# xandercai/JSPSR

Measured on AMD Instinct MI355X. Metric: Mpixels/sec fwd+bwd, JSPSR x8 on 512^2 DEM tiles, higher is better.
Workload: dtype bf16; 1 GPU; jspsr_r8_img_msk (image+mask guided, 43.87M params), 8 x 512x512 tiles per GPU, train step (fwd + L1/L2/Sobel loss + bwd + grad all-reduce + AdamW); storage policy: bf16 activations / gradients / MFMA operands, fp32 accumulation, BatchNorm statistics, master weights and optimizer, and the generator head (affinity logits + offsets) kept as fp32 planes; tiles_per_gpu=8, tile=512, global_tiles=8, parallelism=dp1, step_mode=eager

## Files before the change

### include/jspsr_hip.h

```cpp
#ifndef JSPSR_HIP_H
#define JSPSR_HIP_H

#include <stddef.h>
#include <stdint.h>

#ifdef __cplusplus
extern "C" {
#endif

#define JSPSR_OK 0
#define JSPSR_EINVAL (-1)
#define JSPSR_EALIGN (-2)

typedef void* jspsr_stream_t;

int jspsr_abi_version(void);
long long jspsr_launch_count(const char* what);
int jspsr_conv_dynamic_queue(int on);
const char* jspsr_last_error(void);

int jspsr_prop_forward_f32(const float* dem, const float* weight, const float* offset,
                           int offset_channels, const float* wk, const float* b0, float scale,
                           float* out, int B, int H, int W, jspsr_stream_t stream);

// ... 71 lines not shown
typedef struct jspsr_pack_desc {
  const float* w;
  void* out;
  long long start;
  long long total;
  int O, I, KH, KW;
  int mode;
  int c_pad;
  int dtype;
  int reserved;
} jspsr_pack_desc;
int jspsr_pack_chunk(void);
int jspsr_pack_weights_multi(const jspsr_pack_desc* descs, int n, long long total_blocks, jspsr_stream_t stream);

int jspsr_conv2d_stats_rows(int B, int OH, int OW);
int jspsr_conv2d_in_affine_ok(int dtype, int Cin, int KH, int KW, int stride);
int jspsr_conv2d_forward(int dtype, const void* in, const void* wpack, const float* bias, void* out,
                         int B, int IH, int IW, int Cin, int in_cstride, int in_coff, int Cout,
                         int out_cstride, int out_coff, int KH, int KW, int stride, int pad, int relu,
                         float* stats, const float* scale, const void* addend, int add_cstride,
                         const float* in_affine, int in_relu, jspsr_stream_t stream);
int jspsr_conv2d_forward_scaled(int dtype, const void* in, const void* wpack, const float* bias, void* out,
                                int B, int IH, int IW, int Cin, int in_cstride, int in_coff, int Cout,
                                int out_cstride, int out_coff, int KH, int KW, int stride, int pad, int relu,
                                float* stats, const float* scale, const void* addend, int add_cstride,
                                const float* in_scale, int in_scale_bstride, jspsr_stream_t stream);

int jspsr_conv2d_dgrad_reduce_ok(int dtype, int B, int IH, int IW, int Cg, int Cin, int KH, int KW, int stride, int pad);
int jspsr_conv2d_dgrad(int dtype, const void* gout, const void* wpack_t, const float* bias, void* gin,
                       int B, int OH, int OW, int Cg, int g_cstride, int g_coff, int IH, int IW,
                       int Cin, int in_cstride, int in_coff, int KH, int KW, int stride, int pad,
                       int relu, const void* addend, int add_cstride, const float* scale,
                       const void* red_x, int red_cstride, const float* red_par, float* red_out, jspsr_stream_t stream);

size_t jspsr_conv2d_wgrad_workspace_bytes(int dtype, int B, int OH, int OW, int Cg, int Cx, int KH, int KW);
int jspsr_conv2d_wgrad_x_affine_ok(int dtype, int B, int OH, int OW, int Cg, int Cx, int KH, int KW, int stride, int pad);
int jspsr_conv2d_wgrad(int dtype, const void* G, int Cg, int g_cstride, int g_coff, const void* X, int Cx,
                       int x_cstride, int x_coff, float* dW, int R, int C, int B, int OH, int OW,
                       int IH, int IW, int KH, int KW, int stride, int pad, int accumulate,
                       const float* x_affine, int x_relu, void* workspace, jspsr_stream_t stream);
int jspsr_conv2d_wgrad_scaled(int dtype, const void* G, int Cg, int g_cstride, int g_coff, const void* X, int Cx,
                              int x_cstride, int x_coff, float* dW, int R, int C, int B, int OH, int OW,
                              int IH, int IW, int KH, int KW, int stride, int pad, int accumulate,
                              const float* x_scale, int x_scale_bstride, void* workspace, jspsr_stream_t stream);

size_t jspsr_reduce_workspace_bytes(int dtype, int C, int nseg);

size_t jspsr_bn_mask_bytes(int dtype, long long npix, int C);
int jspsr_bn_forward(int dtype, const void* x, int x_cs, int x_coff, const void* res, int r_cs, int r_coff,
                     void* y, int y_cs, int y_coff, const float* gamma, const float* beta,
                     float* running_mean, float* running_var, float momentum, float eps, int training,
                     int relu, float res_scale, float* save_mean, float* save_invstd, long long npix, int C,
                     const float* ext_partial, int ext_rows, const float* res_affine, float* affine_out,
                     void* mask_out, void* workspace, jspsr_stream_t stream);

int jspsr_bn_fold(const float* gamma, const float* beta, const float* running_mean, const float* running_var,
                  float eps, float res_scale, int C, float* scale, float* shift, jspsr_stream_t stream);

int jspsr_bn_reduce_params(const float* gamma, const float* beta, const float* save_mean, const float* save_invstd, int C,
                           float* par, jspsr_stream_t stream);
int jspsr_bn_backward(int dtype, const void* dy, int dy_cs, int dy_coff, const void* y, int y_cs, int y_coff,
                      const void* x, int x_cs, int x_coff, const float* gamma, const float* beta, const float* save_mean,
                      const float* save_invstd, int training, int relu, float res_scale, void* dx, void* dres,
                      float* dgamma, float* dbeta, int accumulate, long long npix, int C, void* workspace,
                      const float* ext_partial, int ext_rows, const void* mask, jspsr_stream_t stream);

// ... 128 lines not shown
```

### jspsr_amd/JSPSR.py

```python
from __future__ import annotations

import contextlib
import math
import os

import torch
import torch.nn as nn

from . import engine as E
from . import ops
from .blocks import ConvUnit, HotPathModule, ResUnit, UpUnit
from .spn import Generator, PostProcessor

_AUX_KEYS = ("mask", "canopy", "coord")


class Model(HotPathModule):
    receptive_radius = 97
    plain_receptive_radius = 92
    size_multiple = 8

    def __init__(self, in_channels: dict, out_channels: int = 1, num_feature: int = 32,
                 layers: tuple = (2, 2, 2, 2), res_scale: tuple = (1, 1, 1, 1), spn: bool = True,
                 spn_scale: int = 1):
# ... 93 lines not shown
            elif flag_dem_coord:
                dem, coord = in_tensor
            else:
                raise NotImplementedError
        else:
            raise NotImplementedError
        return dem, img, msk, canopy, coord

    def forward(self, *in_tensor):
        dem, img, msk, canopy, coord = self.parse_input(
            self.flag_dem_img, self.flag_dem_msk, self.flag_dem_canopy, self.flag_dem_coord, *in_tensor)
        aux = msk if msk is not None else (canopy if canopy is not None else coord)
        with E.compute_dtype(self.compute_dtype), E.count_batches():
            return self._forward(dem, img, aux)

    branch_streams = True

    def _side_streams(self, device):
        if not self.branch_streams or os.environ.get("JSPSR_BRANCH_STREAMS", "1") == "0" or device.type != "cuda":
            return None
        cache = self.__dict__.setdefault("_branch_stream_cache", {})
        key = (device.index if device.index is not None else torch.cuda.current_device())
        if key not in cache:
            cache[key] = {br: torch.cuda.Stream(device=device) for br in ("img", "aux")}
        return {br: st for br, st in cache[key].items() if br in self._branches}

    def side_streams(self, device=None):
        device = device if device is not None else next(self.parameters()).device
        side = self._side_streams(torch.device(device))
        return list(side.values()) if side else []

    def _forward(self, dem, img, aux):
        dem_a = E.from_nchw(dem)
        feats = {"dem": self.conv_dem(dem_a)}
        if img is not None:
            feats["img"] = self.conv_img(E.from_nchw(img))
        if aux is not None:
            feats["aux"] = self.conv_aux(E.from_nchw(aux))
        order = [b for b in self._branches if b in feats]
        if len(order) < 2:
            raise NotImplementedError
        B, H, W = dem_a.shape[:3]
        nb, nf2 = len(order), self.conv0.conv[0].out_channels
        bufs, fused, joined = [], [], []
        defer_skip = all(getattr(self, f"layer{s}_dem")[0].fused for s in (2, 3, 4))
        deposit_ok = os.environ.get("JSPSR_GRAD_DEPOSIT", "1") != "0" and torch.is_grad_enabled() and order[0] == "dem"
        for s in range(1, 5):
            planes = nf2 * 2 ** (s - 1)
            if s > 1:
                H, W = (H + 1) // 2, (W + 1) // 2
            lead = planes if s < 4 else 0
            buf = E.SliceBuffer(B, H, W, lead + nb * planes, dem_a.dtype, dem_a.device)
            nxt = {}
            side = self._side_streams(dem_a.device) if len(order) > 1 else None
            if side is not None:
                main = torch.cuda.current_stream()
                forked = main.record_event()
            for i, br in enumerate(order):
                from_fused = br == "dem" and bool(fused)
                src = fused[-1] if from_fused else feats[br]
                units = list(getattr(self, f"layer{s}_{br}"))
                st = side.get(br) if side is not None else None
                if st is not None:
                    st.wait_event(forked)
                    buf.buf.record_stream(st)
                    if s == 1:
                        src.record_stream(st)
                with (torch.cuda.stream(st) if st is not None else contextlib.nullcontext()):
                    for k, u in enumerate(units):
                        kw = {}
                        if k == 0 and from_fused and defer_skip:
                            kw["grad_extra"] = bufs[-1][0]
                        elif k == 0 and s > 1 and defer_skip and br != "dem" and getattr(u, "fused", False) and deposit_ok:
                            holder, w_prev = bufs[-1][0], planes // 2
                            kw["grad_extra"] = (holder, i * w_prev, w_prev)
                            holder.expected_deposits += 1
                        if k == len(units) - 1:
                            kw["dest"] = (buf, lead + i * planes)
                        src = u(src, **kw)
                nxt[br] = src
            if side is not None:
                for st in side.values():
                    main.wait_stream(st)
            feats = nxt
            bufs.append((buf, lead))
            joined.append([feats[b] for b in order])
            fused.append(buf.join(joined[-1], lead))
        x = fused[3]
        for up, s in ((self.layer3d, 2), (self.layer2d, 1), (self.layer1d, 0)):
            buf, lead = bufs[s]
            x = buf.join([up(x, dest=(buf, 0))] + joined[s], 0, defer=nb if defer_skip else 0)
        c0 = self.conv0(x)
        if not self.spn:
            head = self.postprocessor.conv[0]
            return E.conv_head1(c0, head.weight, head.bias)
        dem = dem.detach()
        feature = self.generator.features(dem_a.detach(), c0)
        return self.postprocessor.from_feature(dem.float(), feature, self.generator)
```

### jspsr_amd/_lib.py

```python
from __future__ import annotations

import ctypes
import os
import subprocess
import threading

_HERE = os.path.dirname(os.path.abspath(__file__))
SO_PATH = os.environ.get("JSPSR_LAB_LIB") or os.path.join(_HERE, "lib", "libjspsr_hip.so")
CSRC = os.path.join(_HERE, "csrc")
ABI_VERSION = 25

_lock = threading.Lock()
_lib = None

c_p = ctypes.c_void_p
c_i = ctypes.c_int
c_f = ctypes.c_float
c_ll = ctypes.c_longlong

SIGNATURES = {
    "jspsr_abi_version": (c_i, []),
    "jspsr_launch_count": (c_ll, [ctypes.c_char_p]),
    "jspsr_conv_dynamic_queue": (c_i, [c_i]),
    "jspsr_last_error": (ctypes.c_char_p, []),
    "jspsr_prop_forward_f32": (c_i, [c_p, c_p, c_p, c_i, c_p, c_p, c_f, c_p, c_i, c_i, c_i, c_p]),
    "jspsr_prop_backward_workspace_bytes": (ctypes.c_size_t, [c_i, c_i, c_i]),
    "jspsr_prop_backward_f32": (c_i, [c_p] * 4 + [c_i] + [c_p] * 6 + [c_i, c_i, c_i, c_p]),
    "jspsr_prop_backward_fold_f32": (c_i, [c_p, c_i, c_i, c_i, c_p, c_p, c_p]),
    "jspsr_prop_step_forward_f32": (c_i, [c_p, c_p, c_p, c_i, c_p, c_p, c_f, c_i, c_p, c_i, c_i, c_i, c_p]),
    "jspsr_prop_step_backward_workspace_bytes": (ctypes.c_size_t, [c_i, c_i, c_i]),
    "jspsr_prop_step_backward_f32": (c_i, [c_p] * 4 + [c_i, c_p, c_f, c_i, c_i] + [c_p] * 6 + [c_i, c_i, c_i, c_p]),
    "jspsr_prop_head_forward": (c_i, [c_i, c_p, c_p, c_p, c_p, c_f, c_p, c_i, c_i, c_i, c_p]),
    "jspsr_prop_head_backward_workspace_bytes": (ctypes.c_size_t, [c_i, c_i, c_i]),
    "jspsr_prop_head_backward": (c_i, [c_i] + [c_p] * 8 + [c_i, c_i, c_i, c_p]),
    "jspsr_prop_logits_forward_f32": (c_i, [c_p, c_p, c_p, c_p, c_f, c_p, c_i, c_i, c_i, c_p]),
    "jspsr_prop_logits_backward_f32": (c_i, [c_p] * 8 + [c_i, c_i, c_i, c_p]),
    "jspsr_head_ok": (c_i, [c_i] * 5),
    "jspsr_head_forward": (c_i, [c_i, c_p, c_i, c_i, c_i, c_p, c_p, c_p, c_i, c_i, c_i, c_p]),
    "jspsr_head_backward_workspace_bytes": (ctypes.c_size_t, [c_i, c_i, c_i]),
    "jspsr_head_backward": (c_i, [c_i, c_p, c_p, c_i, c_p, c_i, c_i, c_p, c_p, c_p, c_i, c_i, c_i, c_p]),
    "jspsr_conv_head1_forward": (c_i, [c_i, c_p, c_i, c_i, c_i, c_p, c_p, c_p, c_i, c_i, c_i, c_p]),
    "jspsr_conv_head1_workspace_bytes": (ctypes.c_size_t, [c_i, c_i, c_i, c_i]),
    "jspsr_conv_head1_backward": (c_i, [c_i, c_p, c_p, c_i, c_i, c_i, c_p, c_p, c_i, c_i, c_p, c_p, c_p, c_i, c_i, c_i, c_p]),
    "jspsr_pack_weight": (c_i, [c_i, c_p, c_p] + [c_i] * 6 + [c_p]),
    "jspsr_pack_chunk": (c_i, []),
    "jspsr_pack_weights_multi": (c_i, [c_p, c_i, c_ll, c_p]),
    "jspsr_conv2d_stats_rows": (c_i, [c_i, c_i, c_i]),
    "jspsr_conv2d_in_affine_ok": (c_i, [c_i] * 5),
    "jspsr_conv2d_forward": (c_i, [c_i] + [c_p] * 4 + [c_i] * 14 + [c_p, c_p, c_p, c_i, c_p, c_i, c_p]),
    "jspsr_conv2d_forward_scaled": (c_i, [c_i] + [c_p] * 4 + [c_i] * 14 + [c_p, c_p, c_p, c_i, c_p, c_i, c_p]),
    "jspsr_bn_fold": (c_i, [c_p, c_p, c_p, c_p, c_f, c_f, c_i, c_p, c_p, c_p]),
    "jspsr_conv2d_dgrad_reduce_ok": (c_i, [c_i] * 10),
    "jspsr_conv2d_dgrad": (c_i, [c_i] + [c_p] * 4 + [c_i] * 16 + [c_p, c_i, c_p, c_p, c_i, c_p, c_p, c_p]),
    "jspsr_conv2d_wgrad_workspace_bytes": (ctypes.c_size_t, [c_i] * 8),
    "jspsr_conv2d_wgrad_x_affine_ok": (c_i, [c_i] * 10),
    "jspsr_conv2d_wgrad": (c_i, [c_i, c_p, c_i, c_i, c_i, c_p, c_i, c_i, c_i, c_p] + [c_i] * 12 + [c_p, c_i, c_p, c_p]),
    "jspsr_conv2d_wgrad_scaled": (c_i, [c_i, c_p, c_i, c_i, c_i, c_p, c_i, c_i, c_i, c_p] + [c_i] * 12 + [c_p, c_i, c_p, c_p]),
    "jspsr_reduce_workspace_bytes": (ctypes.c_size_t, [c_i, c_i, c_i]),
    "jspsr_bn_forward": (c_i, [c_i, c_p, c_i, c_i, c_p, c_i, c_i, c_p, c_i, c_i, c_p, c_p, c_p, c_p, c_f, c_f, c_i,
                               c_i, c_f, c_p, c_p, c_ll, c_i, c_p, c_i, c_p, c_p, c_p, c_p, c_p]),
    "jspsr_bn_mask_bytes": (ctypes.c_size_t, [c_i, c_ll, c_i]),
    "jspsr_bn_reduce_params": (c_i, [c_p, c_p, c_p, c_p, c_i, c_p, c_p]),
    "jspsr_bn_backward": (c_i, [c_i, c_p, c_i, c_i, c_p, c_i, c_i, c_p, c_i, c_i, c_p, c_p, c_p, c_p, c_i, c_i, c_f,
                                c_p, c_p, c_p, c_p, c_i, c_ll, c_i, c_p, c_p, c_i, c_p, c_p]),
    "jspsr_act_backward": (c_i, [c_i, c_p, c_i, c_i, c_p, c_i, c_i, c_p, c_i, c_p, c_ll, c_i, c_p, c_p]),
    "jspsr_gate_pool": (c_i, [c_i, c_p, c_i, c_ll, c_i, c_p, c_p, c_p, c_p, c_p]),
    "jspsr_gate_scale": (c_i, [c_i, c_p, c_p, c_p, c_i, c_ll, c_i, c_p]),
    "jspsr_gate_backward_reduce": (c_i, [c_i, c_p, c_p, c_p, c_i, c_ll, c_i, c_p, c_p]),
    "jspsr_gate_backward_apply": (c_i, [c_i, c_p, c_p, c_p, c_p, c_p, c_p, c_i, c_ll, c_i, c_p]),
    "jspsr_loss_workspace_bytes": (ctypes.c_size_t, [c_i, c_i, c_i]),
    "jspsr_loss_forward": (c_i, [c_p, c_p, c_f, c_f, c_f, c_p, c_p, c_i, c_i, c_i, c_p]),
    "jspsr_loss_backward": (c_i, [c_p, c_p, c_p, c_f, c_f, c_f, c_p, c_p, c_i, c_i, c_i, c_p]),
    "jspsr_loss_menu_workspace_bytes": (ctypes.c_size_t, [c_i, c_i, c_i, c_i]),
    "jspsr_loss_menu_forward": (c_i, [c_p, c_p, c_i, c_i, c_i, c_i, c_i, c_p, c_p, c_p, c_p, c_p, c_p]),
    "jspsr_loss_menu_backward": (c_i, [c_p, c_p, c_i, c_i, c_i, c_i, c_p, c_p, c_p, c_p, c_p]),
    "jspsr_ssim_workspace_bytes": (ctypes.c_size_t, [c_i, c_i, c_i, c_i]),
    "jspsr_ssim_forward": (c_i, [c_p, c_p, c_i, c_i, c_i, c_i, c_p, c_p, c_p, c_p]),
    "jspsr_metrics_workspace_bytes": (ctypes.c_size_t, [c_i, c_i]),
    "jspsr_metrics_forward": (c_i, [c_p, c_p, c_i, c_i, c_f, c_f, c_f, c_i, c_p, c_p, c_p]),
    "jspsr_scores_batch_workspace_bytes": (ctypes.c_size_t, [c_i, c_i, c_i]),
    "jspsr_scores_batch_forward": (c_i, [c_p, c_p, c_i, c_i, c_i, c_f, c_f, c_f, c_i, c_p, c_p, c_p]),
    "jspsr_scenes_assemble_f32": (c_i, [c_p] * 5 + [c_ll] + [c_i] * 6 + [ctypes.c_double, ctypes.c_double, c_p]),
    "jspsr_summary_workspace_bytes": (ctypes.c_size_t, [c_i, c_i, c_ll, c_ll]),
    "jspsr_summary_forward": (c_i, [c_p, c_p, c_i, c_p, c_ll, c_p, c_i, c_p, c_i, c_ll, c_ll, ctypes.c_double, c_p, c_p, c_p]),
    "jspsr_summary_valid_workspace_bytes": (ctypes.c_size_t, [c_i, c_i, c_ll, c_ll]),
    "jspsr_summary_valid_forward": (c_i, [c_p, c_p, c_i, c_p, c_ll, c_p, c_ll, c_p, c_i, c_p, c_i, c_ll, c_ll, ctypes.c_double,
# ... 82 lines not shown
```

### jspsr_amd/blocks.py

```python
from __future__ import annotations

import torch
import torch.nn as nn

from . import engine as E
from . import ops


class HotPathModule(nn.Module):

    def zero_grad(self, set_to_none: bool = True):
        red = self.__dict__.get("_grad_reducer")
        if red is not None:
            red.zero_grad()
        else:
            super().zero_grad(set_to_none)

    def train(self, mode: bool = True):
        ops.invalidate_packed_weights()
        return super().train(mode)

    def load_state_dict(self, *args, **kwargs):
        out = super().load_state_dict(*args, **kwargs)
        ops.invalidate_packed_weights()
        return out


class ChannelGate(nn.Module):

    def __init__(self, channels: int, ratio: int = 16):
        super().__init__()
        self.fc = nn.Sequential()
        self.fc.add_module("0", nn.Conv2d(channels, channels // ratio, 1, bias=False))
        self.fc.add_module("2", nn.Conv2d(channels // ratio, channels, 1, bias=False))

    def forward(self, x):
        return E.channel_gate(x, self.fc[0].weight, self.fc[1].weight)


class ConvUnit(nn.Module):

    def __init__(self, cin, cout, kernel_size=3, bn=True, relu=True, gate=False):
        super().__init__()
        if gate:
            self.camb = ChannelGate(cin)
        self.conv = nn.Sequential()
        self.conv.add_module("0", nn.Conv2d(cin, cout, kernel_size, 1, kernel_size // 2, bias=not bn))
        if bn:
            self.conv.add_module("bn", nn.BatchNorm2d(cout))
        self.k = kernel_size
        self.relu = relu

    def forward(self, x, dest=None):
        c = self.conv[0]
        if hasattr(self, "camb") and hasattr(self.conv, "bn"):
            fc = self.camb.fc
            return E.gated_conv_bn(x, fc[0].weight, fc[1].weight, c.weight, self.conv.bn, self.k // 2, relu=self.relu, dest=dest)
        if hasattr(self, "camb"):
            x = self.camb(x)
        if hasattr(self.conv, "bn"):
            return E.conv_bn(x, c.weight, self.conv.bn, 1, self.k // 2, relu=self.relu, dest=dest)
        return E.conv2d(x, c.weight, c.bias, 1, self.k // 2, relu=self.relu, dest=dest)


class UpUnit(nn.Module):

    def __init__(self, cin, cout):
        super().__init__()
        self.dconv = nn.Sequential()
        self.dconv.add_module("0", ConvUnit(cin, cout, 3, bn=True, relu=True, gate=True))
        self.dconv.add_module("1", nn.ConvTranspose2d(cout, cout, 3, 2, 1, 1, bias=False))
        self.dconv.add_module("bn", nn.BatchNorm2d(cout))

    def forward(self, x, dest=None):
        y = self.dconv[0](x)
        bn = self.dconv.bn
        if not torch.is_grad_enabled() and not (bn.training or bn.running_mean is None):
            return ops.conv_transpose_bn_infer(y, self.dconv[1].weight, bn.weight, bn.bias, E._bn_state(bn), True, dest)
        y = E.conv_transpose2d(y, self.dconv[1].weight)
        return E.batch_norm(y, bn, relu=True, dest=dest)


class ResUnit(nn.Module):

    def __init__(self, cin, cout, stride=1, project=False, act=True, scale=1.0):
        super().__init__()
        self.conv1 = nn.Conv2d(cin, cout, 3, stride, 1, bias=False)
        self.bn1 = nn.BatchNorm2d(cout)
        self.conv2 = nn.Conv2d(cout, cout, 3, 1, 1, bias=False)
        self.bn2 = nn.BatchNorm2d(cout)
        self.downsample = None
        if project:
            self.downsample = nn.Sequential(nn.Conv2d(cin, cout, 1, stride, bias=False), nn.BatchNorm2d(cout))
        self.stride, self.act, self.scale = stride, act, scale

    fused = True

    def forward(self, x, dest=None, grad_extra=None):
        if self.fused:
            return E.res_unit(x, self.conv1, self.bn1, self.conv2, self.bn2, self.downsample, self.stride, self.scale,
                              self.act, dest, grad_extra)
        if grad_extra is not None:
            raise RuntimeError("grad_extra needs the fused block")
        y = E.conv_bn(x, self.conv1.weight, self.bn1, self.stride, 1, relu=True)
        if self.downsample is not None:
            r = E.conv_bn(x, self.downsample[0].weight, self.downsample[1], self.stride, 0)
        else:
            r = x
        return E.conv_bn(y, self.conv2.weight, self.bn2, 1, 1, relu=self.act, residual=r, res_scale=self.scale,
                         dest=dest)
```

### jspsr_amd/csrc/conv.hip

```cpp
#include "conv_igemm.h"

#include <cstdlib>
#include <type_traits>

namespace {

using namespace jspsr;

constexpr int NT = 256;
constexpr int NCH = 8;
template <typename T> struct Elem;
template <> struct Elem<float> { static constexpr int EPC = 4; };
template <> struct Elem<__bf16> { static constexpr int EPC = 8; };

template <typename T> struct Mma;
template <> struct Mma<float> {
  static constexpr int BLK = 32, ROWP = 144, NE = 16, SUB = NCH / 2, SUBB = 32;
  using acc_t = f32x16;
  static __device__ __forceinline__ int frag_row(int lane) { return lane & 31; }
  static __device__ __forceinline__ int frag_chunk(int lane) { return lane >> 5; }
  static __device__ __forceinline__ int acc_row(int lane, int e) { return (e & 3) + 8 * (e >> 2) + 4 * (lane >> 5); }
  static __device__ __forceinline__ int acc_col(int lane) { return lane & 31; }
};
template <> struct Mma<__bf16> {
// ... 90 lines not shown
    for (int i = 0; i < 4; ++i) f[i] = __uint_as_float(w[i]);
  } else {
#pragma unroll
    for (int i = 0; i < 4; ++i) {
      f[2 * i] = __uint_as_float(w[i] << 16);
      f[2 * i + 1] = __uint_as_float(w[i] & 0xffff0000u);
    }
  }
}

template <typename T>
__device__ __forceinline__ uint4 add_packed(uint4 a, uint4 b) {
  if constexpr (sizeof(T) == 4) {
    float4 x = __builtin_bit_cast(float4, a), y = __builtin_bit_cast(float4, b);
    x.x += y.x; x.y += y.y; x.z += y.z; x.w += y.w;
    return __builtin_bit_cast(uint4, x);
  } else {
    const unsigned* pa = &a.x;
    const unsigned* pb = &b.x;
    uint4 r;
    unsigned* pr = &r.x;
#pragma unroll
    for (int i = 0; i < 4; ++i) {
      const float lo = __uint_as_float(pa[i] << 16) + __uint_as_float(pb[i] << 16);
      const float hi = __uint_as_float(pa[i] & 0xffff0000u) + __uint_as_float(pb[i] & 0xffff0000u);
      const __bf16 l = (__bf16)lo, h = (__bf16)hi;
      pr[i] = (unsigned)__builtin_bit_cast(unsigned short, l) | ((unsigned)__builtin_bit_cast(unsigned short, h) << 16);
    }
    return r;
  }
}

template <typename T>
__device__ __forceinline__ uint4 relu_packed(uint4 a) {
  if constexpr (sizeof(T) == 4) {
    float4 x = __builtin_bit_cast(float4, a);
    x.x = fmaxf(x.x, 0.f); x.y = fmaxf(x.y, 0.f); x.z = fmaxf(x.z, 0.f); x.w = fmaxf(x.w, 0.f);
    return __builtin_bit_cast(uint4, x);
  } else {
    unsigned* p = &a.x;
#pragma unroll
    for (int i = 0; i < 4; ++i) {
      if (p[i] & 0x00008000u) p[i] &= 0xffff0000u;
      if (p[i] & 0x80000000u) p[i] &= 0x0000ffffu;
    }
    return a;
  }
}

template <typename T, int BM, int BN, int WGM, int WGN, bool UNI, int NBUF>
__global__ __launch_bounds__(NT, NBUF == 1 ? 4 : 2) void conv_igemm_kernel(const T* __restrict__ in,
                                                          const T* __restrict__ wgt,
                                                          const float* __restrict__ bias,
                                                          T* __restrict__ out, float* __restrict__ stats, ConvGeom g) {
  static_assert(WGM * WGN == 4, "4 waves");
  constexpr int EPC = Elem<T>::EPC, BK = NCH * EPC;
  using M = IgemmMma<T, NBUF>;
  constexpr int ROWB = M::ROWP, BLK = M::BLK;
  constexpr int WTM = BM / WGM, WTN = BN / WGN, MI = WTM / BLK, NI = WTN / BLK;
  constexpr int A_IT = BM * NCH / NT, B_IT = (BN * NCH + NT - 1) / NT;
  static_assert(MI >= 1 && NI >= 1 && BM * NCH % NT == 0, "tile");
  using frag_t = typename Frag<T>::type;

  extern __shared__ __attribute__((aligned(16))) char smem[];
  constexpr int AS_BYTES = BM * ROWB, BS_BYTES = BN * ROWB;
  char* As = smem;
  char* Bs = smem + NBUF * AS_BYTES;

  constexpr int TLW = 16, TLH = BM / TLW;
  const int tid = threadIdx.x;
  const int ntn = (g.Cout + BN - 1) / BN;
  const int ttx = (g.MW + TLW - 1) / TLW, tty = (g.MH + TLH - 1) / TLH;
  const int t = g.accumulate ? (int)blockIdx.x : xcd_contiguous(blockIdx.x, gridDim.x);
  const int n0 = (t % ntn) * BN;
  const int mt = t / ntn;
  const int txi = mt % ttx, tyi = (mt / ttx) % tty, bimg = mt / (ttx * tty);
  const int ty0 = tyi * TLH, tx0 = txi * TLW;

  const int ch = tid & (NCH - 1);
  const int r0 = tid >> 3;
  constexpr unsigned OOB = 0xFFFFFFF0u;
  const int pix_bytes = g.in_cstride * (int)sizeof(T);
  const int iy_ref = ty0 * g.iy_mul + g.iy_add, ix_ref = tx0 * g.ix_mul + g.ix_add;
// ... 193 lines not shown
        areg[j] = make_uint4(0, 0, 0, 0);
        if (opix >= 0 && n0 + c16 * EPC < g.Cout)
          areg[j] = *reinterpret_cast<const uint4*>(static_cast<const char*>(g.addend) +
                                                    (opix * g.add_cstride + n0) * (long long)sizeof(T) + c16 * 16);
      }
    }
#pragma unroll
    for (int mi = 0; mi < MI; ++mi)
#pragma unroll
      for (int e = 0; e < M::NE; ++e) {
        const int row = wm * WTM + mi * BLK + M::acc_row(lane, e);
#pragma unroll
        for (int ni = 0; ni < NI; ++ni) {
          float v = acc[mi][ni][e] * sv[ni] + bv[ni];
          if (relu_first) v = fmaxf(v, 0.f);
          *reinterpret_cast<T*>(Os + row * OPITCH + (wn * WTN + ni * BLK + lc) * (int)sizeof(T)) = (T)v;
        }
      }
    __syncthreads();
    char* const obase = reinterpret_cast<char*>(out + g.out_coff + n0);
#pragma unroll
    for (int j = 0; j < O_IT; ++j) {
      const int i = tid + j * NT, row = i / CPRO, c16 = i % CPRO;
      const long long opix = out_pixel(row);
      if (opix < 0 || n0 + c16 * EPC >= g.Cout) continue;
      uint4 v = *reinterpret_cast<const uint4*>(Os + row * OPITCH + c16 * 16);
      if (CONV_ABLATE == 4 && v.x != 0x12345678u) continue;
      if (add_pre)
        v = add_packed<T>(v, areg[j < A_PRE ? j : 0]);
      else if (g.addend)
        v = add_packed<T>(v, *reinterpret_cast<const uint4*>(static_cast<const char*>(g.addend) +
                                                              (opix * g.add_cstride + n0) * (long long)sizeof(T) + c16 * 16));
      if (relu_last) v = relu_packed<T>(v);
      *reinterpret_cast<uint4*>(obase + opix * g.out_cstride * (long long)sizeof(T) + c16 * 16) = v;
    }
  } else {
#pragma unroll
    for (int mi = 0; mi < MI; ++mi) {
#pragma unroll
      for (int e = 0; e < M::NE; ++e) {
        const int row = wm * WTM + mi * BLK + M::acc_row(lane, e);
        const long long opix = out_pixel(row);
        if (opix < 0) continue;
        T* orow = out + opix * g.out_cstride + g.out_coff;
#pragma unroll
        for (int ni = 0; ni < NI; ++ni) {
          if (ncol[ni] >= g.Cout) continue;
          float v = acc[mi][ni][e] * sv[ni] + bv[ni];
          if (relu_first) v = fmaxf(v, 0.f);
          if (g.addend) v = (float)(T)v + (float)static_cast<const T*>(g.addend)[opix * g.add_cstride + ncol[ni]];
          if (relu_last) v = fmaxf(v, 0.f);
          orow[ncol[ni]] = (T)v;
        }
      }
    }
  }
}

#ifdef CONVLAB_STAMPS
constexpr int CONVLAB_SLOTS = 1 << 17;
__device__ unsigned long long convlab_stamp[CONVLAB_SLOTS * 16];
#define CL_NOW(t) do { __builtin_amdgcn_sched_barrier(0); asm volatile("s_memtime %0\n\ts_waitcnt lgkmcnt(0)" : "=s"(t) :: "memory"); \
    __builtin_amdgcn_sched_barrier(0); } while (0)
#if CONVLAB_STAMPS == 2
#define CL_STAMP(i) do { unsigned long long now_; CL_NOW(now_); cl_stamp[i] += now_ - cl_last; cl_last = now_; } while (0)
#else
#define CL_STAMP(i) do { } while (0)
#endif
#else
#define CL_STAMP(i) do { } while (0)
#endif
#if defined(CONVLAB_STAMPS) && CONVLAB_STAMPS == 3
#define CL_STAMP3(i) do { unsigned long long now_; CL_NOW(now_); cl_stamp[i] += now_ - cl_last; cl_last = now_; } while (0)
#else
#define CL_STAMP3(i) do { } while (0)
#endif

__host__ __device__ constexpr int patch_it(int BM, int NTH) { return ((BM / 16 + 2) * 18 * NCH + NTH - 1) / NTH; }

template <typename T, int BM, int BN, int WGM, int WGN>
__global__ __launch_bounds__(64 * WGM * WGN, WGM * WGN == 8 ? 1 : 2) void conv_patch_kernel(const T* __restrict__ in, const T* __restrict__ wgt,
                                                          const float* __restrict__ bias, T* __restrict__ out,
                                                          float* __restrict__ stats, ConvGeom g) {
  static_assert(WGM * WGN == 4 || WGM * WGN == 8, "4 or 8 waves");
  constexpr int NTH = 64 * WGM * WGN, RPI = NTH / NCH;
  constexpr int TLW = 16, TLH = BM / TLW;
  constexpr int EPC = Elem<T>::EPC, BK = NCH * EPC;
  using M = Mma<T>;
  constexpr int ROWB = M::ROWP, BLK = M::BLK;
  constexpr int WTM = BM / WGM, WTN = BN / WGN, MI = WTM / BLK, NI = WTN / BLK;
  constexpr int B_IT = (BN * NCH + NTH - 1) / NTH;
  constexpr int P_IT = patch_it(BM, NTH);
  constexpr int MAXPIX = P_IT * NTH / NCH;
  constexpr int BS_BYTES = BN * ROWB;
  constexpr unsigned OOB = 0xFFFFFFF0u;
  using frag_t = typename Frag<T>::type;

  extern __shared__ __attribute__((aligned(16))) char smem[];
  char* Ps = smem;
  char* Bs = smem + MAXPIX * ROWB;

#ifdef CONVLAB_STAMPS
  unsigned long long cl_entry, cl_stamp[8] = {0, 0, 0, 0, 0, 0, 0, 0}, cl_last = 0, cl_first = 0;
  CL_NOW(cl_entry);
  cl_last = cl_entry;
#endif
  const int tid = threadIdx.x;
  const int ntn = (g.Cout + BN - 1) / BN;
  const int ttx = (g.MW + TLW - 1) / TLW, tty = (g.MH + TLH - 1) / TLH;
  const int t = xcd_contiguous(blockIdx.x, gridDim.x);
  const int mt = (int)fastdiv((unsigned)t, g.fd_ntn);
  const int n0 = (t - mt * ntn) * BN;
  const int mrow = (int)fastdiv((unsigned)mt, g.fd_ttx), txi = mt - mrow * ttx;
// ... 253 lines not shown
  if (stats) {
    if constexpr (BM == 128) {
      stats_epilogue<M, MI, NI, WGM, WTM, WTN, BN>(acc, stats, smem, mt, g.Cout, n0, wm, wn, lane, out_pixel);
    } else {
      const int tty8 = (g.MH + 7) / 8;
      const int r1 = (bimg * tty8 + 2 * tyi) * ttx + txi;
      const int r2 = (2 * tyi + 1 < tty8) ? r1 + ttx : -1;
      stats_epilogue<M, MI, NI, WGM, WTM, WTN, BN>(acc, stats, smem, r1, g.Cout, n0, wm, wn, lane, out_pixel, r2);
    }
  }
  float bv[NI], sv[NI];
  int ncol[NI];
  const bool relu_first = g.relu && !g.addend, relu_last = g.relu && g.addend;
#pragma unroll
  for (int ni = 0; ni < NI; ++ni) {
    ncol[ni] = n0 + wn * WTN + ni * BLK + lc;
    bv[ni] = (bias && ncol[ni] < g.Cout) ? bias[ncol[ni]] : 0.f;
    sv[ni] = (g.scale && ncol[ni] < g.Cout) ? g.scale[ncol[ni]] : 1.f;
  }
  constexpr int OPITCH = BN * (int)sizeof(T) + 16;
  char* Os = smem;
  const bool vec_ok = (g.Cout % EPC == 0) && ((g.out_cstride * (int)sizeof(T)) % 16 == 0) &&
                      (((g.out_coff + n0) * (int)sizeof(T)) % 16 == 0) &&
                      ((reinterpret_cast<uintptr_t>(out) & 15u) == 0) &&
                      (!g.addend || (((reinterpret_cast<uintptr_t>(g.addend) & 15u) == 0) &&
                                     ((g.add_cstride * (int)sizeof(T)) % 16 == 0) && ((n0 * (int)sizeof(T)) % 16 == 0)));
  if (vec_ok) {
    constexpr int CPRO = BN * (int)sizeof(T) / 16;
    constexpr int O_IT = BM * CPRO / NTH, OB = O_IT <= 8 ? O_IT : 8;
    static_assert(BM * CPRO % NTH == 0 && O_IT % OB == 0, "epilogue rows");
    long long ooff[OB];
    uint4 areg[OB];
    uint4 zreg[OB];
    const int oy_t = ty0 * g.oy_mul + g.oy_add, ox_t = tx0 * g.ox_mul + g.ox_add, ystep = g.oy_mul * g.OW;
    const long long pix_t = ((long long)bimg * g.OH + oy_t) * g.OW + ox_t;
    const unsigned ocs = (unsigned)g.out_cstride * (unsigned)sizeof(T), acs = (unsigned)g.add_cstride * (unsigned)sizeof(T);
    const long long obase_t = pix_t * ocs, abase_t = pix_t * acs + n0 * (long long)sizeof(T);
    const unsigned zcs = (unsigned)g.red_cstride * (unsigned)sizeof(T);
    const long long zbase_t = pix_t * zcs + n0 * (long long)sizeof(T);
    const bool inside = ty0 + TLH <= g.MH && tx0 + TLW <= g.MW && oy_t + (TLH - 1) * g.oy_mul < g.OH &&
                        ox_t + (TLW - 1) * g.ox_mul < g.OW && n0 + BN <= g.Cout;
    auto plan_pieces = [&](int j0) __attribute__((always_inline)) {
#pragma unroll
      for (int j = 0; j < OB; ++j) {
        const int i = tid + (j0 + j) * NTH, row = i / CPRO, c16 = i % CPRO;
        const int dy = row >> 4, dx = (row + rot * dy) & (TLW - 1);
        const unsigned dpix = (unsigned)(dy * ystep + dx * g.ox_mul);
        bool ok = true;
        if (!inside)
          ok = ty0 + dy < g.MH && tx0 + dx < g.MW && oy_t + dy * g.oy_mul < g.OH && ox_t + dx * g.ox_mul < g.OW &&
               n0 + c16 * EPC < g.Cout;
        ooff[j] = ok ? obase_t + (long long)((unsigned long long)dpix * ocs) + c16 * 16 : -1;
        if (g.addend) {
          areg[j] = make_uint4(0, 0, 0, 0);
          if (ok)
            areg[j] = *reinterpret_cast<const uint4*>(static_cast<const char*>(g.addend) + abase_t +
                                                      (long long)((unsigned long long)dpix * acs) + c16 * 16);
        }
        if (g.red_out) {
          zreg[j] = make_uint4(0, 0, 0, 0);
          if (ok)
            zreg[j] = *reinterpret_cast<const uint4*>(static_cast<const char*>(g.red_x) + zbase_t +
                                                      (long long)((unsigned long long)dpix * zcs) + c16 * 16);
        }
      }
    };
    float rs1[EPC], rs2[EPC], rpa[EPC], rpb[EPC], rpi[EPC], rpm[EPC];
    if (g.red_out) {
      static_assert(NTH % CPRO == 0, "a thread's pieces share their channels");
      const int cc = n0 + (tid % CPRO) * EPC;
#pragma unroll
      for (int e2 = 0; e2 < EPC; ++e2) {
        const bool in_c = cc + e2 < g.Cout;
        rs1[e2] = rs2[e2] = 0.f;
        rpa[e2] = in_c ? g.red_par[cc + e2] : 0.f;
        rpb[e2] = in_c ? g.red_par[g.Cout + cc + e2] : 0.f;
        rpi[e2] = in_c ? g.red_par[2 * g.Cout + cc + e2] : 0.f;
        rpm[e2] = in_c ? g.red_par[3 * g.Cout + cc + e2] : 0.f;
      }
    }
    plan_pieces(0);
#pragma unroll
    for (int mi = 0; mi < MI; ++mi)
#pragma unroll
      for (int e = 0; e < M::NE; ++e) {
        const int row = wm * WTM + mi * BLK + M::acc_row(lane, e);
#pragma unroll
        for (int ni = 0; ni < NI; ++ni) {
          float v = acc[mi][ni][e] * sv[ni] + bv[ni];
          if (relu_first) v = fmaxf(v, 0.f);
          *reinterpret_cast<T*>(Os + row * OPITCH + (wn * WTN + ni * BLK + lc) * (int)sizeof(T)) = (T)v;
        }
      }
    CL_STAMP3(0);
    __syncthreads();
    CL_STAMP3(1);
    char* const obase = reinterpret_cast<char*>(out + g.out_coff + n0);
#pragma unroll
    for (int j0 = 0; j0 < O_IT; j0 += OB) {
      if (j0) plan_pieces(j0);
      uint4 ov[OB];
#pragma unroll
      for (int j = 0; j < OB; ++j) {
        const int i = tid + (j0 + j) * NTH, row = i / CPRO, c16 = i % CPRO;
        ov[j] = *reinterpret_cast<const uint4*>(Os + row * OPITCH + c16 * 16);
      }
      CL_STAMP3(2);
#pragma unroll
      for (int j = 0; j < OB; ++j) {
        if (ooff[j] < 0) continue;
        uint4 v = ov[j];
        if (g.addend) v = add_packed<T>(v, areg[j]);
        if (relu_last) v = relu_packed<T>(v);
        *reinterpret_cast<uint4*>(obase + ooff[j]) = v;
        if (g.red_out) {
          float dv[EPC], zv[EPC];
          unpack_chunk<T>(v, dv);
          unpack_chunk<T>(zreg[j], zv);
#pragma unroll
          for (int e2 = 0; e2 < EPC; ++e2) {
            const float dz = rpa[e2] * zv[e2] + rpb[e2] > 0.f ? dv[e2] : 0.f;
            rs1[e2] += dz;
            rs2[e2] += dz * (zv[e2] * rpi[e2] + rpm[e2]);
          }
        }
      }
    }
    if (g.red_out) {
      __syncthreads();
      float* red = reinterpret_cast<float*>(smem);
#pragma unroll
      for (int e2 = 0; e2 < EPC; ++e2) {
        red[tid * 2 * EPC + e2] = rs1[e2];
        red[tid * 2 * EPC + EPC + e2] = rs2[e2];
      }
      __syncthreads();
      int r1 = mt, r2 = -1;
      if constexpr (BM != 128) {
        const int tty8 = (g.MH + 7) / 8;
        r1 = (bimg * tty8 + 2 * tyi) * ttx + txi;
        r2 = (2 * tyi + 1 < tty8) ? r1 + ttx : -1;
      }
      for (int i = tid; i < 2 * BN; i += NTH) {
        const int which = i / BN, col = i % BN;
        if (n0 + col >= g.Cout) continue;
        const int cg_ = col / EPC, e2 = col % EPC;
        float tsum = 0.f;
        for (int k2 = 0; k2 < NTH / CPRO; ++k2) tsum += red[(cg_ + CPRO * k2) * 2 * EPC + which * EPC + e2];
        g.red_out[((size_t)r1 * 2 + which) * g.Cout + n0 + col] = tsum;
        if (r2 >= 0) g.red_out[((size_t)r2 * 2 + which) * g.Cout + n0 + col] = 0.f;
      }
    }
  } else {
#pragma unroll
    for (int mi = 0; mi < MI; ++mi)
#pragma unroll
      for (int e = 0; e < M::NE; ++e) {
        const int row = wm * WTM + mi * BLK + M::acc_row(lane, e);
        const long long opix = out_pixel(row);
        if (opix < 0) continue;
        T* orow = out + opix * g.out_cstride + g.out_coff;
#pragma unroll
        for (int ni = 0; ni < NI; ++ni) {
          if (ncol[ni] >= g.Cout) continue;
          float v = acc[mi][ni][e] * sv[ni] + bv[ni];
          if (relu_first) v = fmaxf(v, 0.f);
          if (g.addend) v = (float)(T)v + (float)static_cast<const T*>(g.addend)[opix * g.add_cstride + ncol[ni]];
          if (relu_last) v = fmaxf(v, 0.f);
          orow[ncol[ni]] = (T)v;
        }
      }
  }
#ifdef CONVLAB_STAMPS
  if ((tid & 63) == 0) {
    unsigned long long end_;
    CL_NOW(end_);
    unsigned long long* o = convlab_stamp + (size_t)((blockIdx.x * (NTH / 64) + (tid >> 6)) % CONVLAB_SLOTS) * 16;
    for (int i = 0; i < 4; ++i) o[i] = cl_stamp[i] + (i == 3 ? cl_stamp[4] : 0);
    o[4] = cl_first - cl_entry;
    o[5] = cl_loop - cl_first;
    o[6] = end_ - cl_loop;
    for (int i = 5; i < 8; ++i) o[3 + i] = cl_stamp[i];
    o[11] = cl_stamp[4];
    o[7] = (unsigned long long)KT;
  }
#endif
}

template <typename T, int BM, int BN, int WGM, int WGN>
int launch_patch(const void* in, const void* wgt, const float* bias, void* out, float* stats, const ConvGeom& g, hipStream_t s) {
  constexpr int NTH = 64 * WGM * WGN, TLW = 16, TLH = BM / TLW, MAXPIX = patch_it(BM, NTH) * NTH / NCH;
  const long long nblk = (long long)g.B * ((g.MH + TLH - 1) / TLH) * ((g.MW + TLW - 1) / TLW) * ((g.Cout + BN - 1) / BN);
  if (nblk > 0x7fffffffLL || (long long)TLH * g.oy_mul * g.OW + (long long)TLW * g.ox_mul > 0x7fffffffLL)
    return fail(JSPSR_EINVAL, "conv: grid too large");
  constexpr int ROWB = Mma<T>::ROWP;
  const size_t lds_stage = (size_t)MAXPIX * ROWB + 2 * BN * ROWB, lds_out = (size_t)BM * (BN * sizeof(T) + 16);
  const size_t lds = lds_stage > lds_out ? lds_stage : lds_out;
  ConvGeom gk = g;
  gk.fd_ntn = make_fastdiv((unsigned)((g.Cout + BN - 1) / BN));
  gk.fd_ttx = make_fastdiv((unsigned)((g.MW + TLW - 1) / TLW));
  gk.fd_tty = make_fastdiv((unsigned)((g.MH + TLH - 1) / TLH));
  auto kern = conv_patch_kernel<T, BM, BN, WGM, WGN>;
  static bool attr_set = false;
  if (!attr_set) {
    (void)hipFuncSetAttribute(reinterpret_cast<const void*>(kern), hipFuncAttributeMaxDynamicSharedMemorySize, (int)lds);
    attr_set = true;
  }
  hipLaunchKernelGGL(kern, dim3((unsigned)nblk), dim3(NTH), lds, s, static_cast<const T*>(in), static_cast<const T*>(wgt),
                     bias, static_cast<T*>(out), stats, gk);
  return check_launch(BM == 256 ? (BN == 64 ? "conv_patch_16x16" : "conv_patch_16x16x128") : "conv_patch");
}

template <typename T, int BM, int BN, int WGM, int WGN, int NBUF>
int launch_cfg(const void* in, const void* wgt, const float* bias, void* out, float* stats, const ConvGeom& g, hipStream_t s) {
  if ((long long)g.B * g.MH * g.MW <= 0) return JSPSR_OK;
  constexpr int TLW = 16, TLH = BM / TLW;
  const long long nblk = (long long)g.B * ((g.MH + TLH - 1) / TLH) * ((g.MW + TLW - 1) / TLW) * ((g.Cout + BN - 1) / BN);
  if (nblk > 0x7fffffffLL) return fail(JSPSR_EINVAL, "conv: grid too large");
  constexpr int ROWB = IgemmMma<T, NBUF>::ROWP;
  const size_t lds_stage = NBUF * (BM + BN) * ROWB, lds_out = (size_t)BM * (BN * sizeof(T) + 16);
  const size_t lds = lds_stage > lds_out ? lds_stage : lds_out;
  constexpr int BK = NCH * Elem<T>::EPC;
  static bool attr_set = false;
  if (!attr_set) {
    (void)hipFuncSetAttribute(reinterpret_cast<const void*>(conv_igemm_kernel<T, BM, BN, WGM, WGN, true, NBUF>),
                              hipFuncAttributeMaxDynamicSharedMemorySize, (int)lds);
    (void)hipFuncSetAttribute(reinterpret_cast<const void*>(conv_igemm_kernel<T, BM, BN, WGM, WGN, false, NBUF>),
                              hipFuncAttributeMaxDynamicSharedMemorySize, (int)lds);
    attr_set = true;
  }
  if (g.Cin % BK == 0)
    hipLaunchKernelGGL((conv_igemm_kernel<T, BM, BN, WGM, WGN, true, NBUF>), dim3((unsigned)nblk), dim3(NT), lds, s,
                       static_cast<const T*>(in), static_cast<const T*>(wgt), bias, static_cast<T*>(out), stats, g);
  else
    hipLaunchKernelGGL((conv_igemm_kernel<T, BM, BN, WGM, WGN, false, NBUF>), dim3((unsigned)nblk), dim3(NT), lds, s,
                       static_cast<const T*>(in), static_cast<const T*>(wgt), bias, static_cast<T*>(out), stats, g);
  return check_launch("conv_igemm");
}

template <typename T>
int launch(const void* in, const void* wgt, const float* bias, void* out, float* stats, const ConvGeom& g, hipStream_t s) {
  static const int no_patch = [] { const char* e = getenv("JSPSR_CONV_NOPATCH"); return e ? atoi(e) : 0; }();
  constexpr int BKT = NCH * Elem<T>::EPC;
  if constexpr (sizeof(T) == 2)
  {
    if (conv64_resident_ok(g, in, wgt, bias, out)) return launch_conv64_resident(in, wgt, bias, out, stats, g, s);
    if (conv128_resident_ok(g, in, wgt, bias, out)) return launch_conv128_resident(in, wgt, bias, out, stats, g, s);
  }
  if ((!no_patch || g.in_affine) && g.iy_mul == 1 && g.ix_mul == 1 && g.nty >= 1 && g.ntx >= 1 && g.nty <= 3 && g.ntx <= 3 &&
      g.nty * g.ntx > 1 && g.Cin % BKT == 0 && (long long)(g.IW + 20) * 12 * g.in_cstride * (long long)sizeof(T) < 0xE0000000LL) {
    static const int tall = [] { const char* e = getenv("JSPSR_CONV_TALL"); return e ? atoi(e) : 1; }();
    const long long tiles16 = (long long)g.B * ((g.MH + 15) / 16) * ((g.MW + 15) / 16);
    if (g.Cout > 64) {
      if (tall == 2 && tiles16 * ((g.Cout + 127) / 128) >= 512) return launch_patch<T, 256, 128, 4, 2>(in, wgt, bias, out, stats, g, s);
      if (tall && tall != 4 && tiles16 * ((g.Cout + 63) / 64) >= 1024) return launch_patch<T, 256, 64, 4, 1>(in, wgt, bias, out, stats, g, s);
      return launch_patch<T, 128, 128, 2, 2>(in, wgt, bias, out, stats, g, s);
    }
    if (g.Cout > 32) {
      if (tall && tiles16 >= 1024) return launch_patch<T, 256, 64, 4, 1>(in, wgt, bias, out, stats, g, s);
      return launch_patch<T, 128, 64, 2, 2>(in, wgt, bias, out, stats, g, s);
    }
    return launch_patch<T, 128, 32, 4, 1>(in, wgt, bias, out, stats, g, s);
  }
  if (g.red_out) return fail(JSPSR_EINVAL, "conv2d_dgrad: the fused BatchNorm-backward reduce needs the patch kernel (jspsr_conv2d_dgrad_reduce_ok)");
  if (g.in_affine) return fail(JSPSR_EINVAL, "conv2d_forward: in_affine needs the patch kernel (stride 1, 2..9 taps, Cin a multiple of %d): ask jspsr_conv2d_in_affine_ok first", BKT);
  static const int nbuf_env = [] { const char* e = getenv("JSPSR_CONV_NBUF"); return e ? atoi(e) : 0; }();
  const int nbuf_narrow = nbuf_env ? nbuf_env : ((long long)g.nty * g.ntx * g.Cin <= 1152 ? 1 : 2);
  if (g.Cout > 64) return launch_cfg<T, 128, 128, 2, 2, 2>(in, wgt, bias, out, stats, g, s);
// ... 136 lines not shown
extern "C" int jspsr_conv2d_forward_scaled(int dtype, const void* in, const void* wpack, const float* bias, void* out,
                                           int B, int IH, int IW, int Cin, int in_cstride, int in_coff, int Cout,
                                           int out_cstride, int out_coff, int KH, int KW, int stride, int pad, int relu,
                                           float* stats, const float* scale, const void* addend, int add_cstride,
                                           const float* in_scale, int in_scale_bstride, jspsr_stream_t stream) {
  if (!in_scale || in_scale_bstride < Cin || in_scale_bstride % 4)
    return fail(JSPSR_EINVAL, "conv2d_forward_scaled: in_scale must be [B][in_scale_bstride >= Cin] floats, the stride a multiple of 4");
  return conv2d_forward_impl(dtype, in, wpack, bias, out, B, IH, IW, Cin, in_cstride, in_coff, Cout, out_cstride, out_coff, KH, KW,
                             stride, pad, relu, stats, scale, addend, add_cstride, in_scale, 0, in_scale_bstride, 1, stream);
}

extern "C" int jspsr_conv2d_in_affine_ok(int dtype, int Cin, int KH, int KW, int stride) {
  const int bk = NCH * (dtype == JSPSR_F32 ? 4 : 8);
  return (dtype == JSPSR_F32 || dtype == JSPSR_BF16) && stride == 1 && KH >= 1 && KW >= 1 && KH <= 3 && KW <= 3 && KH * KW > 1 &&
         Cin > 0 && Cin % bk == 0;
}

extern "C" int jspsr_conv2d_dgrad_reduce_ok(int dtype, int B, int IH, int IW, int Cg, int Cin, int KH, int KW, int stride, int pad) {
  if (dtype != JSPSR_F32 && dtype != JSPSR_BF16) return 0;
  static const int off = [] { const char* e = getenv("JSPSR_BN_REDUCE_FUSE"); return e && atoi(e) == 0; }();
  if (off) return 0;
  const int epc = dtype == JSPSR_F32 ? 4 : 8, bkt = NCH * epc;
  if (KH != 3 || KW != 3 || stride != 1 || pad != 1 || Cg <= 0 || Cg % bkt || Cin <= 0 || Cin % epc || B <= 0 || IH <= 0 || IW <= 0) return 0;
  static const int no_patch = [] { const char* e = getenv("JSPSR_CONV_NOPATCH"); return e ? atoi(e) : 0; }();
  if (no_patch) return 0;
  if (dtype == JSPSR_BF16 && Cg == 64 && Cin == 64) {
    static const int resident = [] { const char* e = getenv("JSPSR_CONV_RESIDENT"); return e ? atoi(e) : 1; }();
    static const int min_tiles = [] { const char* e = getenv("JSPSR_CONV_RESIDENT_MIN"); return e ? atoi(e) : 512; }();
    if (resident && (long long)B * ((IH + 15) / 16) * ((IW + 15) / 16) >= min_tiles) return 0;
  }
  return 1;
}

extern "C" int jspsr_conv2d_dgrad(int dtype, const void* gout, const void* wpack_t, const float* bias, void* gin,
                                  int B, int OH, int OW, int Cg, int g_cstride, int g_coff, int IH, int IW,
                                  int Cin, int in_cstride, int in_coff, int KH, int KW, int stride, int pad,
                                  int relu, const void* addend, int add_cstride, const float* scale,
                                  const void* red_x, int red_cstride, const float* red_par, float* red_out,
                                  jspsr_stream_t stream) {
  if (int e = check_common(dtype, gout, wpack_t, gin, Cg, g_cstride, g_coff, in_cstride, in_coff, Cin, "conv2d_dgrad")) return e;
  if (addend && add_cstride < Cin) return fail(JSPSR_EINVAL, "conv2d_dgrad: addend pitch %d < %d channels", add_cstride, Cin);
  if (red_out) {
    if (!red_x || !red_par || !jspsr_conv2d_dgrad_reduce_ok(dtype, B, IH, IW, Cg, Cin, KH, KW, stride, pad))
      return fail(JSPSR_EINVAL, "conv2d_dgrad: the fused BatchNorm-backward reduce needs jspsr_conv2d_dgrad_reduce_ok(...) != 0");
    const int epc = dtype == JSPSR_F32 ? 4 : 8;
    if (red_cstride < Cin || red_cstride % epc || in_cstride % epc || in_coff % epc || !aligned16(red_x) || !aligned16(gin) ||
        (addend && (!aligned16(addend) || add_cstride % epc)))
      return fail(JSPSR_EALIGN, "conv2d_dgrad: fused reduce needs 16-byte pieces (pitches / offsets multiples of %d, aligned tensors)", epc);
  }
  if (B <= 0 || OH <= 0 || OW <= 0 || IH <= 0 || IW <= 0 || KH <= 0 || KW <= 0 || stride <= 0 || pad < 0)
    return fail(JSPSR_EINVAL, "conv2d_dgrad: bad geometry");
  hipStream_t s = static_cast<hipStream_t>(stream);
  for (int py = 0; py < stride; ++py)
    for (int px = 0; px < stride; ++px) {
      ConvGeom g{};
      g.B = B; g.IH = OH; g.IW = OW; g.Cin = Cg;
      g.OH = IH; g.OW = IW; g.Cout = Cin;
      g.in_cstride = g_cstride; g.in_coff = g_coff; g.out_cstride = in_cstride; g.out_coff = in_coff;
      g.MH = (IH - py + stride - 1) / stride;
      g.MW = (IW - px + stride - 1) / stride;
      if (g.MH <= 0 || g.MW <= 0) continue;
      g.ky0 = (py + pad) % stride; g.kx0 = (px + pad) % stride; g.kstep = stride;
      g.nty = g.ky0 < KH ? (KH - g.ky0 + stride - 1) / stride : 0;
      g.ntx = g.kx0 < KW ? (KW - g.kx0 + stride - 1) / stride : 0;
      if (g.nty == 0 || g.ntx == 0) g.nty = g.ntx = 0;
      g.iy_mul = 1; g.iy_add = (py + pad - g.ky0) / stride; g.ix_mul = 1; g.ix_add = (px + pad - g.kx0) / stride;
      g.sign = -1; g.KH = KH; g.KW = KW;
      g.oy_mul = stride; g.oy_add = py; g.ox_mul = stride; g.ox_add = px; g.relu = relu;
      g.addend = addend; g.add_cstride = add_cstride; g.scale = scale;
      g.red_x = red_x; g.red_cstride = red_cstride; g.red_par = red_par; g.red_out = red_out;
      const int e = dtype == JSPSR_F32 ? launch<float>(gout, wpack_t, bias, gin, nullptr, g, s)
                                       : launch<__bf16>(gout, wpack_t, bias, gin, nullptr, g, s);
      if (e) return e;
    }
  return JSPSR_OK;
}

#ifdef CONVLAB_STAMPS
extern "C" int jspsr_lab_conv_stamps(unsigned long long* out16, int reset) {
  static unsigned long long host[CONVLAB_SLOTS * 16];
  if (hipMemcpyFromSymbol(host, HIP_SYMBOL(convlab_stamp), sizeof(host)) != hipSuccess) return 1;
  for (int i = 0; i < 16; ++i) out16[i] = 0;
  for (int r = 0; r < CONVLAB_SLOTS; ++r)
    if (host[r * 16 + 7]) { for (int i = 0; i < 16; ++i) out16[i] += host[r * 16 + i]; }
  if (reset) { for (size_t i = 0; i < sizeof(host) / 8; ++i) host[i] = 0; if (hipMemcpyToSymbol(HIP_SYMBOL(convlab_stamp), host, sizeof(host)) != hipSuccess) return 1; }
  return 0;
}
#endif
```

### jspsr_amd/csrc/conv128.hip

```cpp
#include "conv_igemm.h"

#include <atomic>

#include <cstdlib>
#include <type_traits>

namespace {

using namespace jspsr;

constexpr int Q_NTH = 256;
constexpr int Q_TH = 8, Q_TW = 16;
constexpr int Q_PH = Q_TH + 2, Q_PW = Q_TW + 2, Q_NPIX = Q_PH * Q_PW;
constexpr int Q_PIXB = 256;
constexpr int Q_PATCHB = Q_NPIX * Q_PIXB;
constexpr int Q_PIECES = Q_PATCHB / 1024;
static_assert(Q_PIECES * 1024 == Q_PATCHB, "whole pieces");
constexpr int Q_NP = (Q_PIECES + 3) / 4;
constexpr int Q_BUF1 = 65536;
constexpr int Q_XCHB = 16384;
constexpr int Q_OFF_RED = Q_PATCHB + Q_XCHB;
static_assert(Q_OFF_RED + 2048 <= Q_BUF1, "the first 64 KiB hold patch 0, inbox 0 and the fold");
constexpr int Q_OFF_RUN = Q_OFF_RED + 2048;
static_assert(Q_OFF_RUN + 16 <= Q_BUF1, "run starts inside the first 64 KiB");
// ... 38 lines not shown
}

template <bool FIRST, bool WA>
__device__ __forceinline__ void mfma4(f32x4& c0, f32x4& c1, f32x4& c2, f32x4& c3, const i32x4& w0, const i32x4& w1, const i32x4& w2,
                                      const i32x4& w3, const i32x4& b) {
#define K2Q_MFMA4(OUT, CC, WC)                                                                                           \
  asm volatile("v_mfma_f32_16x16x32_bf16 %0, %4, %8, " CC "0\n\tv_mfma_f32_16x16x32_bf16 %1, %5, %8, " CC "1\n\t"        \
               "v_mfma_f32_16x16x32_bf16 %2, %6, %8, " CC "2\n\tv_mfma_f32_16x16x32_bf16 %3, %7, %8, " CC "3"             \
               : OUT(c0), OUT(c1), OUT(c2), OUT(c3) : WC(w0), WC(w1), WC(w2), WC(w3), "v"(b))
  if constexpr (FIRST) {
    if constexpr (WA)
      asm volatile("v_mfma_f32_16x16x32_bf16 %0, %4, %8, 0\n\tv_mfma_f32_16x16x32_bf16 %1, %5, %8, 0\n\t"
                   "v_mfma_f32_16x16x32_bf16 %2, %6, %8, 0\n\tv_mfma_f32_16x16x32_bf16 %3, %7, %8, 0"
                   : "=&v"(c0), "=&v"(c1), "=&v"(c2), "=&v"(c3) : "a"(w0), "a"(w1), "a"(w2), "a"(w3), "v"(b));
    else
      asm volatile("v_mfma_f32_16x16x32_bf16 %0, %4, %8, 0\n\tv_mfma_f32_16x16x32_bf16 %1, %5, %8, 0\n\t"
                   "v_mfma_f32_16x16x32_bf16 %2, %6, %8, 0\n\tv_mfma_f32_16x16x32_bf16 %3, %7, %8, 0"
                   : "=&v"(c0), "=&v"(c1), "=&v"(c2), "=&v"(c3) : "v"(w0), "v"(w1), "v"(w2), "v"(w3), "v"(b));
  } else {
    if constexpr (WA) K2Q_MFMA4("+v", "%", "a");
    else K2Q_MFMA4("+v", "%", "v");
  }
#undef K2Q_MFMA4
}

typedef const i32x4 __attribute__((address_space(3)))* lds_frag_t;

struct QTile { int bimg, tyi, txi; };
struct QSrc { i32x4 desc; __amdgpu_buffer_rsrc_t rsrc; int oy0, ox0; bool interior; };

template <int SIGN, int MODE, int KH>
__device__ __forceinline__ void conv128_body(const __bf16* __restrict__ in, const __bf16* __restrict__ wgt, const float* __restrict__ bias,
                                             __bf16* __restrict__ out, float* __restrict__ stats, const ConvGeom& g, int ntiles, unsigned* __restrict__ ticket, char* smem) {
  constexpr bool STATS = MODE == 1, AFFINE = MODE == 2;
  const int tid = threadIdx.x, wave = __builtin_amdgcn_readfirstlane(tid >> 6), lane = tid & 63;
  const int cg = wave & 1;
  const int n = lane & 15, q = lane >> 4;
  const int ttx = (g.MW + Q_TW - 1) / Q_TW, tty = (g.MH + Q_TH - 1) / Q_TH;
  const int G = gridDim.x;
  const unsigned lds0 = (unsigned)(size_t)(lptr_t)smem;
  if (lds0 != 0) __builtin_trap();
  const int v = xcd_contiguous(blockIdx.x, G);

  i32x4 breg[9][2][4];
#pragma unroll
  for (int cb = 0; cb < 4; ++cb) {
    const int ch = 64 * cg + 32 * (cb >> 1) + 8 * (n >> 2) + 4 * (cb & 1) + (n & 3);
    const char* wrow = reinterpret_cast<const char*>(wgt) + (size_t)ch * (9 * 128 * 2) + (64 * KH + 8 * q) * 2;
#pragma unroll
    for (int t = 0; t < 9; ++t)
#pragma unroll
      for (int s = 0; s < 2; ++s) breg[t][s][cb] = *reinterpret_cast<const i32x4*>(wrow + t * 256 + s * 64);
  }

  const int dGx = G % ttx, dGy = (G / ttx) % tty, dGb = G / (ttx * tty);
  auto advance = [&](QTile c) {
    c.txi += dGx;
    int carry = c.txi >= ttx;
    c.txi -= carry ? ttx : 0;
    c.tyi += dGy + carry;
    carry = c.tyi >= tty;
    c.tyi -= carry ? tty : 0;
    c.bimg += dGb + carry;
    return c;
  };

  const int pix_bytes = g.in_cstride * 2;
// ... 42 lines not shown
  };
  auto piece_dst = [&](unsigned bufoff, int i) __attribute__((always_inline)) {
#ifdef K2Q_LAB_TODUMP
    return (unsigned)Q_OFF_DUMP;
#endif
    return (wave + 4 * i < Q_PIECES) ? bufoff + (unsigned)(wave + 4 * i) * 1024u : (unsigned)Q_OFF_DUMP;
  };
  auto issue_piece = [&](const QSrc& p, unsigned bufoff, int i) __attribute__((always_inline)) {
    unsigned src = dsrc[i];
    if (!p.interior) src = piece_src(p, piece_xy(i));
    const unsigned dst = lds0 + piece_dst(bufoff, i);
#if defined(K2Q_LAB_NOISSUE)
    asm volatile("" : : "s"(dst), "v"(src), "s"(p.desc));
#elif defined(K2Q_LAB_OOB)
    asm volatile("s_mov_b32 m0, %0\n\ts_nop 4\n\tbuffer_load_dwordx4 %1, %2, 0 offen lds" : : "s"(dst), "v"(src | 0xF0000000u), "s"(p.desc));
#else
    asm volatile("s_mov_b32 m0, %0\n\ts_nop 4\n\tbuffer_load_dwordx4 %1, %2, 0 offen lds" : : "s"(dst), "v"(src), "s"(p.desc));
#endif
  };

  unsigned abase[4][3];
#pragma unroll
  for (int b = 0; b < 4; ++b)
#pragma unroll
    for (int tx = 0; tx < 3; ++tx)
      abase[b][tx] = (unsigned)((Q_PW * b + tx + n) * Q_PIXB + (((8 * KH + q) ^ (2 * ((2 * b + tx + n) & 7))) << 4));

  auto prefetch_addend = [&](QTile tc) __attribute__((always_inline)) {
    const int y = tc.tyi * Q_TH + 4 * KH + q, x = tc.txi * Q_TW + n;
    const unsigned off = (y < g.MH && x < g.MW) ? (unsigned)(y * g.OW + x) * (unsigned)(g.add_cstride * 2) : 0xFFFFFFF0u;
    const unsigned long long b64 = reinterpret_cast<unsigned long long>(g.addend) + ((long long)tc.bimg * g.OH * g.OW * g.add_cstride + 64 * cg) * 2;
    const i32x4 d = {(int)(unsigned)b64, (int)((unsigned)(b64 >> 32) & 0xffffu), g.addend ? (int)0xFFFFFF00u : 0, 0x00020000};
    asm volatile("s_mov_b32 m0, %0\n\ts_nop 4\n\tbuffer_load_dwordx4 %1, %2, 0 offen lds" : : "s"(lds0 + (unsigned)Q_OFF_DUMP), "v"(off), "s"(d));
  };

  char* const give = smem + inbox_off(wave ^ 2) + lane * 16;
  const char* const take = smem + inbox_off(wave) + lane * 16;
  f32x4 acc[8][4];
  auto meet = [&]() __attribute__((always_inline)) {
    asm volatile("s_nop 15\n\ts_nop 15" ::: "memory");
#pragma unroll
    for (int i = 0; i < 4; ++i)
#pragma unroll
      for (int cb = 0; cb < 4; ++cb) *reinterpret_cast<f32x4*>(give + (i * 4 + cb) * 1024) = acc[4 * (1 - KH) + i][cb];
    asm volatile("s_waitcnt lgkmcnt(0)" ::: "memory");
    __builtin_amdgcn_s_barrier();
    asm volatile("" ::: "memory");
#pragma unroll
    for (int i = 0; i < 4; ++i)
#pragma unroll
      for (int cb = 0; cb < 4; ++cb) acc[4 * KH + i][cb] = *reinterpret_cast<const f32x4*>(take + (i * 4 + cb) * 1024);
  };

  auto mfma_tile = [&](const QSrc& nxt, unsigned nbufoff, QTile tc) __attribute__((always_inline)) {
    i32x4 a[Q_LAH];
    constexpr int NSTG = (K2Q_LD_DIST + K2Q_LD_EVERY - 1) / K2Q_LD_EVERY;
    u32x4 stg[NSTG];
    static_for<0, Q_NK + Q_LAH>([&](auto K) __attribute__((always_inline)) {
      constexpr int k = decltype(K)::value;
      if constexpr (k >= Q_LAH) {
        constexpr int kk = k - Q_LAH, half = kk / 72, st = (kk % 72) >> 2, tap = st >> 1, s = st & 1;
        constexpr int r = (half == 0 ? 4 * (1 - KH) : 4 * KH) + (kk & 3);
        if constexpr (kk == 72) meet();
        mfma4<(half == 0 && st == 0), (tap < 8)>(acc[r][0], acc[r][1], acc[r][2], acc[r][3], breg[tap][s][0], breg[tap][s][1], breg[tap][s][2],
                                                 breg[tap][s][3], a[kk % Q_LAH]);
      }
      if constexpr (k < Q_NK) {
        constexpr int half = k / 72, st = (k % 72) >> 2, tap = st >> 1, s = st & 1;
        constexpr int r = (half == 0 ? 4 * (1 - KH) : 4 * KH) + (k & 3);
        constexpr int ty = SIGN > 0 ? tap / 3 : 2 - tap / 3, tx = SIGN > 0 ? tap % 3 : 2 - tap % 3;
        constexpr int R = r + ty;
        a[k % Q_LAH] = *reinterpret_cast<lds_frag_t>((abase[R & 3][tx] ^ (unsigned)(s * 64)) + (unsigned)((R >> 2) * Q_ROWS4));
        if constexpr (K2Q_DMA_MODE == 1 && k % K2Q_DMA_EVERY == 2 && k / K2Q_DMA_EVERY < Q_NP) issue_piece(nxt, nbufoff, k / K2Q_DMA_EVERY);
        if constexpr (!STATS && k == 1) prefetch_addend(tc);
        if constexpr (K2Q_DMA_MODE == 3) {
          constexpr int LD = K2Q_LD_EVERY, WD = K2Q_LD_DIST;
          static_assert(2 + LD * (Q_NP - 1) + WD < Q_NK, "the last piece is written inside the loop");
          if constexpr (k >= 2 + WD && (k - 2 - WD) % LD == 0 && (k - 2 - WD) / LD < Q_NP) {
            constexpr int j = (k - 2 - WD) / LD;
            *reinterpret_cast<u32x4*>(smem + piece_dst(nbufoff, j) + lane * 16) = stg[j % NSTG];
          }
          if constexpr (k >= 2 && (k - 2) % LD == 0 && (k - 2) / LD < Q_NP) {
            constexpr int j = (k - 2) / LD;
            stg[j % NSTG] = __builtin_amdgcn_raw_buffer_load_b128(nxt.rsrc, piece_src(nxt, piece_xy(j)), 0, 0);
          }
        }
      }
    });
    asm volatile("s_nop 15\n\ts_nop 15" ::: "memory");
  };

  const bool relu_first = g.relu && !g.addend, relu_last = g.relu && g.addend;
  float* const red = reinterpret_cast<float*>(smem + Q_OFF_RED);
  auto out_desc = [&](int bimg) {
    const unsigned long long b64 = reinterpret_cast<unsigned long long>(out) + ((long long)bimg * g.OH * g.OW * g.out_cstride + g.out_coff + 64 * cg) * 2;
    return __builtin_amdgcn_make_buffer_rsrc(reinterpret_cast<char*>(b64), 0, 0xFFFFFF00u, 0x00020000);
  };
  auto add_desc = [&](int bimg) {
    const unsigned long long b64 = reinterpret_cast<unsigned long long>(g.addend) + ((long long)bimg * g.OH * g.OW * g.add_cstride + 64 * cg) * 2;
    return __builtin_amdgcn_make_buffer_rsrc(reinterpret_cast<char*>(b64), 0, g.addend ? 0xFFFFFF00u : 0u, 0x00020000);
  };

  auto epilogue = [&](QTile tc) __attribute__((always_inline)) {
    const int ty0 = tc.tyi * Q_TH + 4 * KH, x = tc.txi * Q_TW + n;
    const __amdgpu_buffer_rsrc_t orsrc = out_desc(tc.bimg), adrsrc = add_desc(tc.bimg);
    unsigned ooff[4], aoff[4];
    bool inside[4];
// ... 33 lines not shown
                s2[c] = __builtin_fmaf(a0, a0, s2[c]);
              }
            }
          }
          row_sum<8>(s1); row_sum<8>(s2);
          row_sum<4>(s1); row_sum<4>(s2);
          row_sum<2>(s1); row_sum<2>(s2);
          row_sum<1>(s1); row_sum<1>(s2);
          if (n == 0) {
            float* r1 = red + (KH * 2 + 0) * 128 + 64 * cg + 32 * h + 8 * q;
            float* r2 = red + (KH * 2 + 1) * 128 + 64 * cg + 32 * h + 8 * q;
            *reinterpret_cast<f32x4*>(r1) = f32x4{s1[0], s1[1], s1[2], s1[3]};
            *reinterpret_cast<f32x4*>(r1 + 4) = f32x4{s1[4], s1[5], s1[6], s1[7]};
            *reinterpret_cast<f32x4*>(r2) = f32x4{s2[0], s2[1], s2[2], s2[3]};
            *reinterpret_cast<f32x4*>(r2 + 4) = f32x4{s2[4], s2[5], s2[6], s2[7]};
          }
        }
      }
    }
    if constexpr (AFFINE) {
#pragma unroll
      for (int h = 0; h < 2; ++h) {
        const float* tab = reinterpret_cast<const float*>(smem + Q_OFF_PAR) + 64 * cg + 32 * h + 8 * q;
#pragma unroll
        for (int u = 0; u < 2; ++u) {
          const f32x4 s4 = *reinterpret_cast<const f32x4*>(tab + 4 * u), b4 = *reinterpret_cast<const f32x4*>(tab + 128 + 4 * u);
#pragma unroll
          for (int i = 0; i < 4; ++i)
#pragma unroll
            for (int j = 0; j < 4; ++j) acc[4 * KH + i][2 * h + u][j] = acc[4 * KH + i][2 * h + u][j] * s4[j] + b4[j];
        }
      }
    }
    if (!STATS && g.addend) {
      u32x4 av[4][2];
#pragma unroll
      for (int i = 0; i < 4; ++i)
#pragma unroll
        for (int h = 0; h < 2; ++h) av[i][h] = __builtin_amdgcn_raw_buffer_load_b128(adrsrc, aoff[i], h * 64, 0);
#pragma unroll
      for (int i = 0; i < 4; ++i)
#pragma unroll
        for (int h = 0; h < 2; ++h) {
          const f32x4 lo = acc[4 * KH + i][2 * h], hi = acc[4 * KH + i][2 * h + 1];
          const u32x4 o = {pack_bf16(lo[0], lo[1]), pack_bf16(lo[2], lo[3]), pack_bf16(hi[0], hi[1]), pack_bf16(hi[2], hi[3])};
          __builtin_amdgcn_raw_buffer_store_b128(add_bf16x8(o, av[i][h], relu_last), orsrc, ooff[i], h * 64, 0);
        }
    } else {
      if (!STATS && relu_first) {
#pragma unroll
        for (int i = 0; i < 4; ++i)
#pragma unroll
          for (int cb = 0; cb < 4; ++cb)
#pragma unroll
            for (int j = 0; j < 4; ++j) acc[4 * KH + i][cb][j] = relu_bits(acc[4 * KH + i][cb][j]);
      }
#pragma unroll
      for (int i = 0; i < 4; ++i)
#pragma unroll
        for (int h = 0; h < 2; ++h) {
          const f32x4 lo = acc[4 * KH + i][2 * h], hi = acc[4 * KH + i][2 * h + 1];
          const u32x4 o = {pack_bf16(lo[0], lo[1]), pack_bf16(lo[2], lo[3]), pack_bf16(hi[0], hi[1]), pack_bf16(hi[2], hi[3])};
          __builtin_amdgcn_raw_buffer_store_b128(o, orsrc, ooff[i], h * 64, 0);
        }
    }
  };
  auto flush_stats = [&](QTile tc) __attribute__((always_inline)) {
// ... 124 lines not shown
  static std::atomic<unsigned> n{0};
  return base ? base + 2 * (n.fetch_add(1, std::memory_order_relaxed) % 1024u) : nullptr;
}

template <int SIGN, int MODE>
void launch_k2q(const void* in, const void* wgt, const float* bias, void* out, float* stats, const ConvGeom& g, int ntiles, int grid, hipStream_t s) {
  static bool attr_set = false;
  if (!attr_set) {
    (void)hipFuncSetAttribute(reinterpret_cast<const void*>(conv128_resident_kernel<SIGN, MODE>), hipFuncAttributeMaxDynamicSharedMemorySize, Q_LDS);
    attr_set = true;
  }
  static const int dynq = [] { const char* e = getenv("JSPSR_CONV_DYNQ128"); return e ? atoi(e) : 0; }();
  const int forced = conv_dynq_override();
  unsigned* ticket = ((forced >= 0 ? forced : dynq) && (long long)ntiles >= 4LL * Q_RUN * grid) ? next_ticket() : nullptr;
  hipLaunchKernelGGL((conv128_resident_kernel<SIGN, MODE>), dim3(grid), dim3(Q_NTH), Q_LDS, s, static_cast<const __bf16*>(in),
                     static_cast<const __bf16*>(wgt), bias, static_cast<__bf16*>(out), stats, g, ntiles, ticket);
}

}

namespace jspsr {

bool conv128_resident_ok(const ConvGeom& g, const void* in, const void* wgt, const float* bias, const void* out) {
  static const int enabled = [] { const char* e = getenv("JSPSR_CONV_RESIDENT128"); return e ? atoi(e) : 1; }();
  if (!enabled) return false;
  if (g.Cin != 128 || g.Cout != 128 || g.nty != 3 || g.ntx != 3 || g.KH != 3 || g.KW != 3) return false;
  if (g.iy_mul != 1 || g.ix_mul != 1 || g.oy_mul != 1 || g.ox_mul != 1 || g.oy_add != 0 || g.ox_add != 0) return false;
  if (g.ky0 != 0 || g.kx0 != 0 || g.kstep != 1 || g.in_affine || g.red_out) return false;
  if (bias && !aligned4(bias)) return false;
  if (g.sign < 0 && (bias || g.scale)) return false;
  if (g.in_cstride % 8 || g.in_coff % 8 || g.out_cstride % 8 || g.out_coff % 8) return false;
  if (!aligned16(in) || !aligned16(wgt) || !aligned16(out)) return false;
  if (g.addend && (!aligned16(g.addend) || g.add_cstride % 8)) return false;
  if ((long long)(g.IW + 20) * 12 * g.in_cstride * 2 >= 0x7fffffffLL || g.IW >= (1 << 20) || g.in_cstride >= (1 << 20)) return false;
  if ((long long)g.OH * g.OW * g.out_cstride * 2 >= 0xF0000000LL || (long long)g.OH * g.OW * g.add_cstride * 2 >= 0xF0000000LL)
    return false;
  const long long tiles = (long long)g.B * ((g.MH + Q_TH - 1) / Q_TH) * ((g.MW + Q_TW - 1) / Q_TW);
  static const int min_tiles = [] { const char* e = getenv("JSPSR_CONV_RESIDENT128_MIN"); return e ? atoi(e) : 2048; }();
  return tiles >= min_tiles && tiles < 0x7fffffffLL;
}

int launch_conv128_resident(const void* in, const void* wgt, const float* bias, void* out, float* stats, const ConvGeom& g, hipStream_t s) {
  const int ntiles = g.B * ((g.MH + Q_TH - 1) / Q_TH) * ((g.MW + Q_TW - 1) / Q_TW);
  static int ncu = 0;
  if (!ncu) {
    int dev = 0;
    hipDeviceProp_t p;
    if (hipGetDevice(&dev) != hipSuccess || hipGetDeviceProperties(&p, dev) != hipSuccess) return fail((int)hipErrorInvalidDevice, "conv: device query failed");
    ncu = p.multiProcessorCount > 0 ? p.multiProcessorCount : 256;
  }
  const int grid = ntiles < ncu ? ntiles : ncu;
  static const int trace = [] { const char* e = getenv("JSPSR_CONV_TRACE128"); return e ? atoi(e) : 0; }();
  if (trace)
    fprintf(stderr, "K2q sign %d B %d %dx%d in pitch %d off %d out pitch %d off %d addend %d (pitch %d) relu %d stats %d in %p out %p\n", g.sign, g.B,
            g.MH, g.MW, g.in_cstride, g.in_coff, g.out_cstride, g.out_coff, g.addend != nullptr, g.add_cstride, g.relu, stats != nullptr, in, out);
  const int mode = stats ? 1 : ((bias || g.scale) ? 2 : 0);
  if (g.sign > 0) {
    if (mode == 0) launch_k2q<1, 0>(in, wgt, bias, out, stats, g, ntiles, grid, s);
    else if (mode == 1) launch_k2q<1, 1>(in, wgt, bias, out, stats, g, ntiles, grid, s);
    else launch_k2q<1, 2>(in, wgt, bias, out, stats, g, ntiles, grid, s);
  } else {
    if (mode != 0) return fail(JSPSR_EINVAL, "conv128_resident: the reversed walk has no statistics / affine form");
    launch_k2q<-1, 0>(in, wgt, bias, out, stats, g, ntiles, grid, s);
  }
  return check_launch("conv128_resident");
}

}
```

### jspsr_amd/csrc/conv64.hip

```cpp
#include "conv_igemm.h"

#include <atomic>

#include <cstdlib>
#include <type_traits>

namespace {

using namespace jspsr;

constexpr int R_NTH = 512;
constexpr int R_PW = 18, R_NPIX = R_PW * R_PW;
constexpr int R_PITCH = 144;
constexpr int R_PPP = 7;
constexpr int R_PIECEB = R_PPP * R_PITCH;
constexpr int R_PIECES = (R_NPIX + R_PPP - 1) / R_PPP;
#ifdef K2R_ORDER
constexpr int order_of(bool) { return K2R_ORDER; }
#else
constexpr int order_of(bool stats) { return stats ? 0 : 2; }
#endif
#ifdef K2R_EARLY
constexpr int early_pieces(bool) { return K2R_EARLY; }
#else
constexpr int early_pieces(bool stats) { return stats ? 8 : 6; }
#endif
constexpr int R_PATCHB = R_PIECES * R_PIECEB + 16;
constexpr int R_SCRP = 80;
constexpr int R_SCRB = 64 * R_SCRP;
constexpr int R_OFF_SCR = 2 * R_PATCHB;
constexpr int R_OFF_RED = R_OFF_SCR + 8 * R_SCRB;
constexpr int R_RUNB = 16;
constexpr int R_LDS_STATS = R_OFF_RED + 3 * 4 * 2 * 64 * 4 + R_RUNB;
constexpr int R_LDS_PLAIN = 2 * R_PATCHB + R_RUNB;
constexpr int R_OFF_PAR = 2 * R_PATCHB;
constexpr int R_LDS_AFFINE = R_OFF_PAR + 2 * 64 * 4 + R_RUNB;
constexpr int R_RUN = 4;
#ifndef K2R_LA
#define K2R_LA 4
#endif
constexpr int R_ROT = 14;
constexpr int NK = 72, LA = K2R_LA;

struct Tile { int bimg, tyi, txi; };
struct PatchSrc { i32x4 desc; int oy0, ox0; bool interior; };

template <int SIGN, int MODE>
__global__ __launch_bounds__(R_NTH) void conv64_resident_kernel(const __bf16* __restrict__ in, const __bf16* __restrict__ wgt,
                                                                  const float* __restrict__ bias, __bf16* __restrict__ out,
                                                                  float* __restrict__ stats, ConvGeom g, int ntiles,
                                                                  unsigned* __restrict__ ticket) {
  constexpr bool STATS = MODE == 1, AFFINE = MODE == 2;
  constexpr int LDSB = MODE == 1 ? R_LDS_STATS : (MODE == 2 ? R_LDS_AFFINE : R_LDS_PLAIN);
  extern __shared__ __attribute__((aligned(128))) char smem[];
  const int tid = threadIdx.x, wave = __builtin_amdgcn_readfirstlane(tid >> 6), lane = tid & 63;
  const int wm = (wave >> 1) & 3, wn = wave & 1;
  const int lr = lane & 31, lh = lane >> 5;
  const int ttx = (g.MW + 15) >> 4, tty = (g.MH + 15) >> 4;
  const int G = gridDim.x;
  const unsigned lds0 = (unsigned)(size_t)(lptr_t)smem;
  const int v = xcd_contiguous(blockIdx.x, G);
  const bool late = wave >= 4;
  constexpr int ORDER = order_of(STATS), R_PE = early_pieces(STATS), R_PL = (R_PIECES - 4 * R_PE + 3) / 4;
  constexpr int R_PIT = R_PE > R_PL ? R_PE : R_PL;

  bf16x8 breg[9][4];
  {
    const char* wrow = reinterpret_cast<const char*>(wgt) + (size_t)(wn * 32 + lr) * (9 * 64 * 2) + lh * 16;
#pragma unroll
    for (int t = 0; t < 9; ++t)
#pragma unroll
      for (int s = 0; s < 4; ++s) breg[t][s] = *reinterpret_cast<const bf16x8*>(wrow + t * 128 + s * 32);
  }

  const int dGx = G % ttx, dGy = (G / ttx) % tty, dGb = G / (ttx * tty);
  auto advance = [&](Tile c) {
    c.txi += dGx;
    int carry = c.txi >= ttx;
    c.txi -= carry ? ttx : 0;
    c.tyi += dGy + carry;
    carry = c.tyi >= tty;
    c.tyi -= carry ? tty : 0;
    c.bimg += dGb + carry;
    return c;
  };
// ... 70 lines not shown
    __builtin_amdgcn_sched_group_barrier(0x100, LA, 0);
#pragma unroll
    for (int k = 0; k < NK; ++k) {
      __builtin_amdgcn_sched_group_barrier(0x008, 1, 0);
      if (k + LA < NK) __builtin_amdgcn_sched_group_barrier(0x100, 1, 0);
    }
  };

  const bool relu_first = g.relu && !g.addend, relu_last = g.relu && g.addend;
  char* const scr = smem + R_OFF_SCR + wave * R_SCRB;
  float* const red = reinterpret_cast<float*>(smem + R_OFF_RED);
  const int ncol = wn * 32 + lr;
  const int tty8 = (g.MH + 7) >> 3;

  auto flush_stats = [&](Tile tc, int par) __attribute__((always_inline)) {
    if (tid < 256) {
      const int half = tid >> 7, which = (tid >> 6) & 1, col = tid & 63;
      const int row = 2 * tc.tyi + half;
      if (row < tty8) {
        const float* r0 = red + ((par * 4 + 2 * half) * 2 + which) * 64 + col;
        stats[((size_t)((tc.bimg * tty8 + row) * ttx + tc.txi) * 2 + which) * 64 + col] = r0[0] + r0[2 * 64];
      }
    }
  };

  auto out_desc = [&](int bimg) {
    const unsigned long long b64 = reinterpret_cast<unsigned long long>(out) + ((long long)bimg * g.OH * g.OW * g.out_cstride + g.out_coff + wn * 32) * 2;
    return __builtin_amdgcn_make_buffer_rsrc(reinterpret_cast<char*>(b64), 0, 0xFFFFFF00u, 0x00020000);
  };
  auto add_desc = [&](int bimg) {
    const unsigned long long b64 = reinterpret_cast<unsigned long long>(g.addend) + ((long long)bimg * g.OH * g.OW * g.add_cstride + wn * 32) * 2;
    return __builtin_amdgcn_make_buffer_rsrc(reinterpret_cast<char*>(b64), 0, g.addend ? 0xFFFFFF00u : 0u, 0x00020000);
  };

  auto epilogue_stats = [&](Tile tc, int par) __attribute__((always_inline)) {
    const int ty0 = tc.tyi * 16, tx0 = tc.txi * 16;
    const bool whole = ty0 + 16 <= g.MH && tx0 + 16 <= g.MW;
    if (stats) {
      float s = 0.f, q = 0.f;
      if (whole) {
        f32x2 s2 = {0.f, 0.f}, q2 = {0.f, 0.f};
#pragma unroll
        for (int mi = 0; mi < 2; ++mi)
#pragma unroll
          for (int e = 0; e < 16; e += 2) {
            const f32x2 a2 = {acc[mi][e], acc[mi][e + 1]};
            s2 += a2;
            q2 = __builtin_elementwise_fma(a2, a2, q2);
          }
        s = s2[0] + s2[1];
        q = q2[0] + q2[1];
      } else {
        int lh4 = 4 * lh;
        asm volatile("" : "+v"(lh4));
#pragma unroll
        for (int mi = 0; mi < 2; ++mi)
#pragma unroll
          for (int e = 0; e < 16; ++e) {
            const int R = wm * 64 + mi * 32 + (e & 3) + 8 * (e >> 2) + lh4, dy = R >> 4;
            const int y = ty0 + dy, x = tx0 + ((R + R_ROT * dy) & 15);
            if (y < g.MH && x < g.MW) {
              const float a0 = acc[mi][e];
              s += a0;
              q += a0 * a0;
            }
          }
// ... 18 lines not shown
    const __amdgpu_buffer_rsrc_t orsrc = out_desc(tc.bimg), adrsrc = add_desc(tc.bimg);
    unsigned ooff[4], aoff[4];
#pragma unroll
    for (int j = 0; j < 4; ++j) {
      const int dy = wm * 4 + j;
      const int y = ty0 + dy, x = tx0 + ((prow + R_ROT * dy) & 15);
      const bool inside = whole || (y < g.MH && x < g.MW);
      const unsigned pix = (unsigned)(y * g.OW + x);
      ooff[j] = inside ? pix * (unsigned)(g.out_cstride * 2) + c16 * 16u : 0xFFFFFFF0u;
      aoff[j] = inside ? pix * (unsigned)(g.add_cstride * 2) + c16 * 16u : 0xFFFFFFF0u;
    }
    if (g.addend) {
      u32x4 av[4];
#pragma unroll
      for (int j = 0; j < 4; ++j) av[j] = __builtin_amdgcn_raw_buffer_load_b128(adrsrc, aoff[j], 0, 0);
#pragma unroll
      for (int j = 0; j < 4; ++j) {
        const u32x4 o = *reinterpret_cast<const u32x4*>(scr + (j * 16 + prow) * R_SCRP + c16 * 16);
        __builtin_amdgcn_raw_buffer_store_b128(add_bf16x8(o, av[j], relu_last), orsrc, ooff[j], 0, 0);
      }
    } else {
#pragma unroll
      for (int j = 0; j < 4; ++j) {
        const u32x4 o = *reinterpret_cast<const u32x4*>(scr + (j * 16 + prow) * R_SCRP + c16 * 16);
        __builtin_amdgcn_raw_buffer_store_b128(o, orsrc, ooff[j], 0, 0);
      }
    }
  };

  auto epilogue_regs = [&](Tile tc) __attribute__((always_inline)) {
    const int ty0 = tc.tyi * 16, tx0 = tc.txi * 16;
    const bool whole = ty0 + 16 <= g.MH && tx0 + 16 <= g.MW;
    const __amdgpu_buffer_rsrc_t orsrc = out_desc(tc.bimg), adrsrc = add_desc(tc.bimg);
    unsigned ooff[2], aoff[2];
#pragma unroll
    for (int mi = 0; mi < 2; ++mi) {
      const int R = wm * 64 + mi * 32 + lr, dy = R >> 4;
      const int y = ty0 + dy, x = tx0 + ((R + R_ROT * dy) & 15);
      const bool inside = whole || (y < g.MH && x < g.MW);
      const unsigned pix = (unsigned)(y * g.OW + x);
      ooff[mi] = inside ? pix * (unsigned)(g.out_cstride * 2) + lh * 16u : 0xFFFFFFF0u;
      aoff[mi] = inside ? pix * (unsigned)(g.add_cstride * 2) + lh * 16u : 0xFFFFFFF0u;
    }
    u32x4 av[2][2];
    if (g.addend) {
#pragma unroll
      for (int mi = 0; mi < 2; ++mi)
#pragma unroll
        for (int h = 0; h < 2; ++h) av[mi][h] = __builtin_amdgcn_raw_buffer_load_b128(adrsrc, aoff[mi], h * 32, 0);
    }
    if constexpr (AFFINE) {
      const float* tab = reinterpret_cast<const float*>(smem + R_OFF_PAR) + wn * 32 + 4 * lh;
#pragma unroll
      for (int q = 0; q < 4; ++q) {
        const f32x4v s4 = *reinterpret_cast<const f32x4v*>(tab + 8 * q), b4 = *reinterpret_cast<const f32x4v*>(tab + 64 + 8 * q);
#pragma unroll
        for (int mi = 0; mi < 2; ++mi)
#pragma unroll
          for (int i = 0; i < 4; ++i) acc[mi][4 * q + i] = acc[mi][4 * q + i] * s4[i] + b4[i];
      }
    }
    if (relu_first) {
#pragma unroll
      for (int mi = 0; mi < 2; ++mi)
#pragma unroll
        for (int e = 0; e < 16; ++e) acc[mi][e] = relu_bits(acc[mi][e]);
    }
    unsigned d[2][8];
#pragma unroll
    for (int mi = 0; mi < 2; ++mi)
#pragma unroll
      for (int e = 0; e < 16; e += 2) d[mi][e >> 1] = pack_bf16(acc[mi][e], acc[mi][e + 1]);
#pragma unroll
    for (int mi = 0; mi < 2; ++mi) {
#pragma unroll
      for (int q = 0; q < 4; q += 2)
#pragma unroll
        for (int w = 0; w < 2; ++w) {
          const auto r = __builtin_amdgcn_permlane32_swap(d[mi][2 * q + w], d[mi][2 * q + 2 + w], false, false);
          d[mi][2 * q + w] = r[0];
          d[mi][2 * q + 2 + w] = r[1];
        }
#pragma unroll
      for (int h = 0; h < 2; ++h) {
        u32x4 o = {d[mi][4 * h], d[mi][4 * h + 1], d[mi][4 * h + 2], d[mi][4 * h + 3]};
        if (g.addend) o = add_bf16x8(o, av[mi][h], relu_last);
        __builtin_amdgcn_raw_buffer_store_b128(o, orsrc, ooff[mi], h * 32, 0);
      }
    }
  };
  auto epilogue = [&](Tile tc, int par) __attribute__((always_inline)) {
    if constexpr (STATS) epilogue_stats(tc, par); else epilogue_regs(tc);
  };

  if constexpr (AFFINE) {
    if (tid < 128) reinterpret_cast<float*>(smem + R_OFF_PAR)[tid] = tid < 64 ? (g.scale ? g.scale[tid] : 1.f) : (bias ? bias[tid - 64] : 0.f);
  }
  const bool dyn = ticket != nullptr;
  int* const s_run = reinterpret_cast<int*>(smem + LDSB - R_RUNB);
  if (dyn) {
    if (tid == 0) {
      s_run[0] = (int)__hip_atomic_fetch_add(ticket, (unsigned)R_RUN, __ATOMIC_RELAXED, __HIP_MEMORY_SCOPE_AGENT);
      s_run[1] = (int)__hip_atomic_fetch_add(ticket, (unsigned)R_RUN, __ATOMIC_RELAXED, __HIP_MEMORY_SCOPE_AGENT);
    }
    __syncthreads();
  }
  auto tile_of = [&](int t_) { return Tile{(t_ / ttx) / tty, (t_ / ttx) % tty, t_ % ttx}; };
  int t = dyn ? s_run[0] : v, it = 0;
  int krun = 0, nrun = 0;
  int tn, kn, nn;
  unsigned pend = 0;
  int pend_slot = -1;
  auto step_walk = [&](int t_, int k_, int n_, Tile c_, int& t2, int& k2, int& n2, Tile& c2) {
    if (!dyn) {
      t2 = t_ + G; k2 = 0; n2 = 0; c2 = advance(c_);
    } else if (k_ + 1 < R_RUN && t_ + 1 < ntiles) {
      t2 = t_ + 1; k2 = k_ + 1; n2 = n_;
      c2 = c_;
      if (++c2.txi == ttx) { c2.txi = 0; if (++c2.tyi == tty) { c2.tyi = 0; ++c2.bimg; } }
// ... 98 lines not shown
  static std::atomic<unsigned> n{0};
  return base ? base + 2 * (n.fetch_add(1, std::memory_order_relaxed) % 1024u) : nullptr;
}

template <int SIGN, int MODE>
void launch_k2r(const void* in, const void* wgt, const float* bias, void* out, float* stats, const ConvGeom& g, int ntiles, int grid,
                hipStream_t s) {
  static const int dynq = [] { const char* e = getenv("JSPSR_CONV_DYNQ"); return e ? atoi(e) : 0; }();
  const int forced = conv_dynq_override();
  unsigned* ticket = ((forced >= 0 ? forced : dynq) && (long long)ntiles >= 4LL * R_RUN * grid) ? next_ticket() : nullptr;
  constexpr int lds = MODE == 1 ? R_LDS_STATS : (MODE == 2 ? R_LDS_AFFINE : R_LDS_PLAIN);
  static bool attr_set = false;
  if (!attr_set) {
    (void)hipFuncSetAttribute(reinterpret_cast<const void*>(conv64_resident_kernel<SIGN, MODE>), hipFuncAttributeMaxDynamicSharedMemorySize, lds);
    attr_set = true;
  }
  hipLaunchKernelGGL((conv64_resident_kernel<SIGN, MODE>), dim3(grid), dim3(R_NTH), lds, s, static_cast<const __bf16*>(in),
                     static_cast<const __bf16*>(wgt), bias, static_cast<__bf16*>(out), stats, g, ntiles, ticket);
}

}

namespace jspsr {

bool conv64_resident_ok(const ConvGeom& g, const void* in, const void* wgt, const float* bias, const void* out) {
  static const int enabled = [] { const char* e = getenv("JSPSR_CONV_RESIDENT"); return e ? atoi(e) : 1; }();
  if (!enabled) return false;
  if (g.Cin != 64 || g.Cout != 64 || g.nty != 3 || g.ntx != 3 || g.KH != 3 || g.KW != 3) return false;
  if (g.iy_mul != 1 || g.ix_mul != 1 || g.oy_mul != 1 || g.ox_mul != 1 || g.oy_add != 0 || g.ox_add != 0) return false;
  if (g.ky0 != 0 || g.kx0 != 0 || g.kstep != 1 || g.in_affine || g.red_out) return false;
  if (g.in_cstride % 8 || g.in_coff % 8 || g.out_cstride % 8 || g.out_coff % 8) return false;
  if (!aligned16(in) || !aligned16(wgt) || !aligned16(out)) return false;
  if (g.addend && (!aligned16(g.addend) || g.add_cstride % 8)) return false;
  if ((long long)(g.IW + 20) * 20 * g.in_cstride * 2 >= 0x7fffffffLL) return false;
  if ((long long)g.OH * g.OW * g.out_cstride * 2 >= 0xF0000000LL || (long long)g.OH * g.OW * g.add_cstride * 2 >= 0xF0000000LL)
    return false;
  const long long tiles = (long long)g.B * ((g.MH + 15) / 16) * ((g.MW + 15) / 16);
  static const int min_tiles = [] { const char* e = getenv("JSPSR_CONV_RESIDENT_MIN"); return e ? atoi(e) : 512; }();
  return tiles >= min_tiles && tiles < 0x7fffffffLL;
}

int launch_conv64_resident(const void* in, const void* wgt, const float* bias, void* out, float* stats, const ConvGeom& g,
                           hipStream_t s) {
  const int ntiles = g.B * ((g.MH + 15) / 16) * ((g.MW + 15) / 16);
  static int ncu = 0;
  if (!ncu) {
    int dev = 0;
    hipDeviceProp_t p;
    if (hipGetDevice(&dev) != hipSuccess || hipGetDeviceProperties(&p, dev) != hipSuccess) return fail((int)hipErrorInvalidDevice, "conv: device query failed");
    ncu = p.multiProcessorCount > 0 ? p.multiProcessorCount : 256;
  }
  const int grid = ntiles < ncu ? ntiles : ncu;
  const int mode = stats ? 1 : ((bias || g.scale) ? 2 : 0);
  if (g.sign > 0) {
    if (mode == 0) launch_k2r<1, 0>(in, wgt, bias, out, stats, g, ntiles, grid, s);
    else if (mode == 1) launch_k2r<1, 1>(in, wgt, bias, out, stats, g, ntiles, grid, s);
    else launch_k2r<1, 2>(in, wgt, bias, out, stats, g, ntiles, grid, s);
  } else {
    if (mode == 0) launch_k2r<-1, 0>(in, wgt, bias, out, stats, g, ntiles, grid, s);
    else if (mode == 1) launch_k2r<-1, 1>(in, wgt, bias, out, stats, g, ntiles, grid, s);
    else launch_k2r<-1, 2>(in, wgt, bias, out, stats, g, ntiles, grid, s);
  }
  return check_launch("conv64_resident");
}

}
```

### jspsr_amd/csrc/conv_igemm.h

```cpp
#pragma once
#include "common.h"

namespace jspsr {

using f32x16 = __attribute__((ext_vector_type(16))) float;
using f32x4 = __attribute__((ext_vector_type(4))) float;
using bf16x8 = __attribute__((ext_vector_type(8))) __bf16;
using u16 = unsigned short;

struct ConvGeom {
  int B, IH, IW, Cin;
  int OH, OW, Cout;
  int in_cstride;
  int in_coff;
  int out_cstride;
  int out_coff;
  int MH, MW;
  int iy_mul, iy_add, ix_mul, ix_add, sign;
  int nty, ntx;
  int ky0, kx0, kstep;
  int KH, KW;
  int oy_mul, oy_add, ox_mul, ox_add;
  int relu;
  int accumulate;
  const void* addend;
  int add_cstride;
  const float* scale;
  const float* in_affine;
  int in_relu;
  int in_bstride;
  int in_scale_only;
  FastDiv fd_ntn, fd_ttx, fd_tty;
  const void* red_x;
  int red_cstride;
  const float* red_par;
  float* red_out;
};

typedef __attribute__((address_space(3))) void* lptr_t;
typedef int i32x4 __attribute__((ext_vector_type(4)));
typedef unsigned u32x4 __attribute__((ext_vector_type(4)));
typedef float f32x2 __attribute__((ext_vector_type(2)));
typedef float f32x4v __attribute__((ext_vector_type(4)));

typedef __bf16 bf16x2 __attribute__((ext_vector_type(2)));
__device__ __forceinline__ unsigned pack_bf16(float lo, float hi) {
  const f32x2 v = {lo, hi};
  return __builtin_bit_cast(unsigned, __builtin_convertvector(v, bf16x2));
}
__device__ __forceinline__ float relu_bits(float x) { return __int_as_float(max(__float_as_int(x), 0)); }
__device__ __forceinline__ u32x4 add_bf16x8(u32x4 a, u32x4 b, bool relu) {
  u32x4 r;
#pragma unroll
  for (int i = 0; i < 4; ++i) {
    float lo = __uint_as_float(a[i] << 16) + __uint_as_float(b[i] << 16);
    float hi = __uint_as_float(a[i] & 0xffff0000u) + __uint_as_float(b[i] & 0xffff0000u);
    if (relu) { lo = relu_bits(lo); hi = relu_bits(hi); }
    r[i] = pack_bf16(lo, hi);
  }
  return r;
}


bool conv64_resident_ok(const ConvGeom& g, const void* in, const void* wgt, const float* bias, const void* out);
int launch_conv64_resident(const void* in, const void* wgt, const float* bias, void* out, float* stats, const ConvGeom& g,
                           hipStream_t s);

bool conv128_resident_ok(const ConvGeom& g, const void* in, const void* wgt, const float* bias, const void* out);
int launch_conv128_resident(const void* in, const void* wgt, const float* bias, void* out, float* stats, const ConvGeom& g, hipStream_t s);

}

template <typename T, int N>
__device__ __forceinline__ uint4 affine_relu16(const uint4& v, const float (&sc)[N], const float (&sh)[N], bool relu) {
  static_assert(N * sizeof(T) == 16, "one 16-byte chunk of channels");
  uint4 r;
  if constexpr (sizeof(T) == 4) {
    float f[4] = {__uint_as_float(v.x), __uint_as_float(v.y), __uint_as_float(v.z), __uint_as_float(v.w)};
#pragma unroll
    for (int i = 0; i < 4; ++i) {
      f[i] = __builtin_fmaf(f[i], sc[i], sh[i]);
      if (relu) f[i] = fmaxf(f[i], 0.f);
    }
    r = make_uint4(__float_as_uint(f[0]), __float_as_uint(f[1]), __float_as_uint(f[2]), __float_as_uint(f[3]));
  } else {
    const unsigned w[4] = {v.x, v.y, v.z, v.w};
    unsigned o[4];
#pragma unroll
    for (int i = 0; i < 4; ++i) {
      float lo = __builtin_fmaf(__uint_as_float(w[i] << 16), sc[2 * i], sh[2 * i]);
      float hi = __builtin_fmaf(__uint_as_float(w[i] & 0xffff0000u), sc[2 * i + 1], sh[2 * i + 1]);
      if (relu) { lo = fmaxf(lo, 0.f); hi = fmaxf(hi, 0.f); }
      const __bf16 bl = (__bf16)lo, bh = (__bf16)hi;
      o[i] = (unsigned)__builtin_bit_cast(unsigned short, bl) | ((unsigned)__builtin_bit_cast(unsigned short, bh) << 16);
    }
// ... 28 lines not shown
```

### jspsr_amd/csrc/elementwise.hip

```cpp
#include "common.h"

#include <atomic>
#include <cstdlib>

namespace {

using namespace jspsr;

constexpr int TX = 64, TY = 4;

template <typename T> struct V;
template <> struct V<float> { static constexpr int N = 4; };
template <> struct V<__bf16> { static constexpr int N = 8; };

template <typename T, int N>
struct Pack { T v[N]; };

template <typename T>
__device__ __forceinline__ uint4 load_raw(const T* p) { return *reinterpret_cast<const uint4*>(p); }
template <typename T>
__device__ __forceinline__ void unpack(const uint4& raw, float (&f)[V<T>::N]) {
  if constexpr (sizeof(T) == 4) {
    f[0] = __uint_as_float(raw.x); f[1] = __uint_as_float(raw.y); f[2] = __uint_as_float(raw.z); f[3] = __uint_as_float(raw.w);
  } else {
// ... 807 lines not shown
  else if (mode == 0) { BN_BWD_APPLY(0, dy, dy_cs, dy_coff, dres); }
  else if (mode == 1) { BN_BWD_APPLY(1, dy, dy_cs, dy_coff, dres); }
  else if (mode == 2) { BN_BWD_APPLY(2, dy, dy_cs, dy_coff, dres); }
  else { BN_BWD_APPLY(3, dy, dy_cs, dy_coff, dres); }
#undef BN_BWD_APPLY
  return check_launch("bn_bwd_apply");
}

extern "C" int jspsr_bn_fold(const float* gamma, const float* beta, const float* running_mean, const float* running_var,
                             float eps, float res_scale, int C, float* scale, float* shift, jspsr_stream_t stream) {
  if (!gamma || !beta || !running_mean || !running_var || !scale || !shift || C <= 0)
    return fail(JSPSR_EINVAL, "bn_fold: bad arguments");
  hipLaunchKernelGGL(bn_fold_kernel, dim3((C + 255) / 256), dim3(256), 0, static_cast<hipStream_t>(stream), gamma, beta,
                     running_mean, running_var, eps, res_scale, C, scale, shift);
  return check_launch("bn_fold");
}

extern "C" int jspsr_act_backward(int dtype, const void* dy, int dy_cs, int dy_coff, const void* y, int y_cs, int relu,
                                  void* dz, int dz_cs, float* dbias, long long npix, int C, void* workspace,
                                  jspsr_stream_t stream) {
  if (int e = check_c(dtype, C, "act_backward")) return e;
  if (!dy || (relu && !y) || !workspace || npix <= 0) return fail(JSPSR_EINVAL, "act_backward: null pointer or empty tensor");
  const int vec = dtype == JSPSR_F32 ? 4 : 8;
  if (dy_cs % vec || dy_coff % vec || (dz && dz_cs % vec) || (relu && (y_cs % vec || y_cs < C)))
    return fail(JSPSR_EINVAL, "act_backward: bad pitch");
  hipStream_t s = static_cast<hipStream_t>(stream);
  float* partial = static_cast<float*>(workspace);
  const RedGeom g = make_red(npix, 1, C, vec);
#define ACT_BWD(R) DISPATCH(dtype, hipLaunchKernelGGL((act_bwd_kernel<T, R>), red_grid(g, vec), dim3(TX, TY), 0, s, static_cast<const T*>(dy), \
                                     dy_cs, dy_coff, static_cast<const T*>(y), y_cs, relu, static_cast<T*>(dz), dz_cs, g, partial))
  if (relu) { ACT_BWD(true); } else { ACT_BWD(false); }
#undef ACT_BWD
  if (int e = check_launch("act_backward")) return e;
  if (dbias) {
    hipLaunchKernelGGL(sum_rows_kernel, dim3((C + 3) / 4), dim3(256), 0, s, partial, g.chunks, 1, 0, C, dbias);
    return check_launch("act_backward_bias");
  }
  return JSPSR_OK;
}

extern "C" int jspsr_gate_pool(int dtype, const void* x, int B, long long npix, int C, float* avg, float* mx, int* amax,
                               void* workspace, jspsr_stream_t stream) {
  if (int e = check_c(dtype, C, "gate_pool")) return e;
  if (!x || !avg || !mx || !amax || !workspace || B <= 0 || npix <= 0 || npix > 0x7fffffffLL)
    return fail(JSPSR_EINVAL, "gate_pool: bad arguments");
  const int vec = dtype == JSPSR_F32 ? 4 : 8;
  hipStream_t s = static_cast<hipStream_t>(stream);
  const RedGeom g = make_red(npix, B, C, vec);
  const size_t rows = (size_t)B * g.chunks;
  float* psum = static_cast<float*>(workspace);
  float* pmax = psum + rows * C;
  int* pidx = reinterpret_cast<int*>(pmax + rows * C);
  DISPATCH(dtype, hipLaunchKernelGGL(gate_pool_kernel<T>, red_grid(g, vec), dim3(TX, TY), 0, s, static_cast<const T*>(x), g,
                                     psum, pmax, pidx));
  if (int e = check_launch("gate_pool")) return e;
  hipLaunchKernelGGL(gate_pool_finalize_kernel, dim3((C + 255) / 256, B), dim3(256), 0, s, psum, pmax, pidx, g.chunks, C,
                     npix, avg, mx, amax);
  return check_launch("gate_pool_finalize");
}

extern "C" int jspsr_gate_scale(int dtype, const void* x, const float* s_, void* y, int B, long long npix, int C,
                                jspsr_stream_t stream) {
  if (int e = check_c(dtype, C, "gate_scale")) return e;
  if (!x || !s_ || !y || B <= 0 || npix <= 0) return fail(JSPSR_EINVAL, "gate_scale: bad arguments");
  const int vec = dtype == JSPSR_F32 ? 4 : 8;
  hipStream_t s = static_cast<hipStream_t>(stream);
// ... 370 lines not shown
```

### jspsr_amd/engine.py

```python
from __future__ import annotations

import os

import torch

from . import kernels as K
from . import ops

_compute_dtype = torch.float32
_gate_sync = None
_offset_probe = None


class compute_dtype:

    def __init__(self, dtype):
        if dtype not in (torch.float32, torch.bfloat16):
            raise ValueError("compute dtype must be torch.float32 or torch.bfloat16")
        self.dtype = dtype

    def __enter__(self):
        global _compute_dtype
        self.prev, _compute_dtype = _compute_dtype, self.dtype

    def __exit__(self, *a):
        global _compute_dtype
        _compute_dtype = self.prev


def _gpu(x: torch.Tensor) -> torch.Tensor:
    if not x.is_cuda:
        raise RuntimeError("jspsr_amd runs on the GPU only: move the module and its inputs to cuda "
                           "(there is no CPU fallback; the CPU restatement lives in oracle/ for tests)")
    return x


def from_nchw(x: torch.Tensor) -> torch.Tensor:
    _gpu(x)
    B, C, H, W = x.shape
    e = K.epc(_compute_dtype)
    if x.dtype == torch.float32 and x.is_contiguous() and not (x.requires_grad and torch.is_grad_enabled()):
        return K.nchw_to_nhwc(x, _compute_dtype, (C + e - 1) // e * e)
    x = x.reshape(B, H, W, 1) if C == 1 else x.permute(0, 2, 3, 1)
    return ops.pad_channels(x.to(_compute_dtype), e).contiguous()


def to_nchw_f32(x: torch.Tensor) -> torch.Tensor:
    B, H, W, C = x.shape
    if C == 1:
        return x.float().reshape(B, 1, H, W)
    return x.permute(0, 3, 1, 2).float().contiguous()


SliceBuffer = ops.SliceBuffer


def conv2d(x, weight, bias=None, stride=1, padding=0, relu=False, dest=None):
    return ops.conv2d(x, weight, bias, stride, padding, relu, dest)


def conv_transpose2d(x, weight):
    return ops.conv_transpose2d(x, weight)


_nbt_pending = None


class count_batches:

    def __enter__(self):
        global _nbt_pending
        self.prev, _nbt_pending = _nbt_pending, []
        return self

    def __exit__(self, *a):
        global _nbt_pending
        todo, _nbt_pending = _nbt_pending, self.prev
        if todo and a[0] is None:
            seen = {}
            for t in todo:
                seen[id(t)] = (t, seen.get(id(t), (t, 0))[1] + 1)
            once = [t for t, k in seen.values() if k == 1]
            if once:
                torch._foreach_add_(once, 1)
            for t, k in seen.values():
                if k > 1:
                    t += k
        return False


def _count_batch(bn):
    if bn.training and bn.track_running_stats and bn.num_batches_tracked is not None:
        if _nbt_pending is not None:
            _nbt_pending.append(bn.num_batches_tracked)
        else:
            bn.num_batches_tracked += 1


def batch_norm(x, bn: torch.nn.BatchNorm2d, relu=False, residual=None, res_scale=1.0, partial=None, dest=None):
    training = bn.training or bn.running_mean is None
    _count_batch(bn)
    return ops.batch_norm(x, bn.weight, bn.bias, bn.running_mean, bn.running_var, bn.momentum, bn.eps, training,
                          relu, residual, res_scale, partial, dest)


def conv_bn(x, weight, bn: torch.nn.BatchNorm2d, stride=1, padding=0, relu=False, residual=None, res_scale=1.0, dest=None):
    if bn.training or bn.running_mean is None:
        y, st = ops.conv2d_with_stats(x, weight, stride, padding)
        return batch_norm(y, bn, relu, residual, res_scale, partial=st, dest=dest)
    if not torch.is_grad_enabled():
        return ops.conv_bn_infer(x, weight, bn.weight, bn.bias, _bn_state(bn), stride, padding, relu, residual,
                                 res_scale, dest)
    return batch_norm(ops.conv2d(x, weight, None, stride, padding), bn, relu, residual, res_scale, dest=dest)


def _bn_state(bn: torch.nn.BatchNorm2d):
    training = bn.training or bn.running_mean is None
    _count_batch(bn)
    return (bn.running_mean, bn.running_var, bn.momentum, bn.eps, training)


def res_unit(x, conv1, bn1, conv2, bn2, downsample, stride, scale, act, dest=None, grad_extra=None):
    bns = [_bn_state(bn1), _bn_state(bn2)]
    wd = gd = bd = None
    if downsample is not None:
        wd, gd, bd = downsample[0].weight, downsample[1].weight, downsample[1].bias
        bns.append(_bn_state(downsample[1]))
    return ops.res_unit(x, conv1.weight, bn1.weight, bn1.bias, conv2.weight, bn2.weight, bn2.bias, wd, gd, bd,
                        stride, scale, act, tuple(bns), dest, grad_extra)


def channel_gate(x, w1, w2):
    if _gate_sync is not None:
        avg, mx = _gate_sync.pool(x.contiguous())
        s = ops._gate_mlp(avg, mx, w1.detach().float(), w2.detach().float()).contiguous()
        return K.gate_scale(x.contiguous(), s)
    return ops.channel_gate(x, w1, w2)


def gated_conv_bn(x, gw1, gw2, weight, bn: torch.nn.BatchNorm2d, padding=1, relu=False, dest=None):
    training = bn.training or bn.running_mean is None
    if _gate_sync is None and training and torch.is_grad_enabled() and ops.gated_conv_ok(x, weight, padding):
        return ops.gated_conv_bn(x, gw1, gw2, weight, bn.weight, bn.bias, _bn_state(bn), padding, relu, dest)
    return conv_bn(channel_gate(x, gw1, gw2), weight, bn, 1, padding, relu=relu, dest=dest)


def propagate_head(dem, head, w, b, scale=1.0):
    return ops.propagate_head(dem.contiguous(), head, w, b, scale)


planar_heads = os.environ.get("JSPSR_HEAD_PLANES", "1") != "0"


def heads_propagate(dem, feature, conv_weight, conv_offset, w, b, scale=1.0):
    dem = dem.contiguous()
    if planar_heads and ops.head_planes_ok(feature):
        planes = ops.head_planes(feature, conv_weight.weight, conv_weight.bias, conv_offset.weight, conv_offset.bias)
        if _offset_probe is not None:
            _offset_probe.append(planes[:, 9:].permute(0, 2, 3, 1))
        return ops.propagate_logits(dem, planes, w, b, scale)
    w_all, b_all = ops.merge_heads(conv_weight.weight, conv_weight.bias, conv_offset.weight, conv_offset.bias)
    head = conv2d(feature, w_all, b_all)
# ... 20 lines not shown
```

### jspsr_amd/kernels.py

```python
from __future__ import annotations

import torch

from . import _lib

F32, BF16 = 0, 1


def _dt(t: torch.Tensor) -> int:
    if t.dtype == torch.float32:
        return F32
    if t.dtype == torch.bfloat16:
        return BF16
    raise TypeError(f"unsupported dtype {t.dtype}")


def epc(dtype: torch.dtype) -> int:
    return 4 if dtype == torch.float32 else 8


def _stream() -> int:
    return torch.cuda.current_stream().cuda_stream


# ... 80 lines not shown
    if addend is not None:
        _chk_s(addend, "conv2d_forward addend")
        if tuple(addend.shape) != (B, OH, OW, Cout) or addend.dtype != x.dtype:
            raise ValueError(f"conv2d_forward: addend {tuple(addend.shape)} {addend.dtype} does not match the result")
    head = (_dt(x), x.data_ptr(), wpack.data_ptr(), bias.data_ptr() if bias is not None else None, out.data_ptr(),
            B, IH, IW, Cin, Cs, in_coff, Cout, pitch(out), out_coff, KH, KW, stride, pad, int(relu),
            st.data_ptr() if st is not None else None, scale.data_ptr() if scale is not None else None,
            addend.data_ptr() if addend is not None else None, pitch(addend) if addend is not None else 0)
    if in_scale is not None:
        if in_affine is not None:
            raise ValueError("conv2d_forward: in_scale and in_affine exclude each other")
        _chk_scale(in_scale, B, Cin, "conv2d_forward in_scale")
        _lib.check(lib.jspsr_conv2d_forward_scaled(*head, in_scale.data_ptr(), in_scale.shape[1], _stream()),
                   "jspsr_conv2d_forward_scaled")
    else:
        _lib.check(lib.jspsr_conv2d_forward(*head, in_affine.data_ptr() if in_affine is not None else None, int(in_relu),
                                            _stream()), "jspsr_conv2d_forward")
    return (out, st) if stats else out


def dgrad_reduce_ok(dtype, B, IH, IW, Cg, Cin, KH, KW, stride, pad) -> bool:
    dt = F32 if dtype == torch.float32 else BF16
    return bool(_lib.load().jspsr_conv2d_dgrad_reduce_ok(dt, B, IH, IW, Cg, Cin, KH, KW, stride, pad))


def bn_reduce_params(gamma, beta, mean, invstd):
    C = gamma.numel()
    par = torch.empty((4, C), dtype=torch.float32, device=gamma.device)
    _lib.check(_lib.load().jspsr_bn_reduce_params(gamma.data_ptr(), beta.data_ptr(), mean.data_ptr(), invstd.data_ptr(), C,
                                                  par.data_ptr(), _stream()), "jspsr_bn_reduce_params")
    return par


def conv2d_dgrad(g, wpack_t, in_hw, stride, pad, bias=None, relu=False, out=None, out_coff=0, g_coff=0, addend=None,
                 scale=None, red=None):
    _chk_s(g, "conv2d_dgrad")
    B, OH, OW, _ = g.shape
    Cgs = pitch(g)
    Cin, KH, KW, Cg = wpack_t.shape
    IH, IW = in_hw
    if out is None:
        out = torch.empty((B, IH, IW, Cin), dtype=g.dtype, device=g.device)
    else:
        _chk_s(out, "conv2d_dgrad out")
        if tuple(out.shape[:3]) != (B, IH, IW) or out.shape[3] < out_coff + Cin or out.dtype != g.dtype:
            raise ValueError(f"conv2d_dgrad: out {tuple(out.shape)} {out.dtype} cannot take a ({B},{IH},{IW},{Cin}) {g.dtype} result at channel {out_coff}")
    if addend is not None:
        _chk_s(addend, "conv2d_dgrad addend")
        if tuple(addend.shape) != (B, IH, IW, Cin) or addend.dtype != g.dtype:
            raise ValueError(f"conv2d_dgrad: addend {tuple(addend.shape)} {addend.dtype} does not match the result")
    lib = _lib.load()
    red_x = red_par = red_out = None
    if red is not None:
        red_x, red_par = red
        _chk_s(red_x, "conv2d_dgrad red_x")
        if tuple(red_x.shape) != (B, IH, IW, Cin) or red_x.dtype != g.dtype:
            raise ValueError(f"conv2d_dgrad: red_x {tuple(red_x.shape)} {red_x.dtype} does not match the result")
        rows = lib.jspsr_conv2d_stats_rows(B, IH, IW)
        red_out = torch.empty((rows, 2, Cin), dtype=torch.float32, device=g.device)
    _lib.check(lib.jspsr_conv2d_dgrad(_dt(g), g.data_ptr(), wpack_t.data_ptr(),
                                      bias.data_ptr() if bias is not None else None, out.data_ptr(),
                                      B, OH, OW, Cg, Cgs, g_coff, IH, IW, Cin, pitch(out), out_coff,
                                      KH, KW, stride, pad, int(relu),
                                      addend.data_ptr() if addend is not None else None,
                                      pitch(addend) if addend is not None else 0,
                                      scale.data_ptr() if scale is not None else None,
                                      red_x.data_ptr() if red is not None else None, pitch(red_x) if red is not None else 0,
                                      red_par.data_ptr() if red is not None else None,
                                      red_out.data_ptr() if red is not None else None, _stream()), "jspsr_conv2d_dgrad")
    return (out, red_out) if red is not None else out


def conv2d_wgrad(G, X, R, C, KH, KW, stride, pad, out=None, accumulate=False, g_coff=0, cg=None, x_coff=0, cx=None,
                 x_affine=None, x_relu=False, x_scale=None):
    _chk_s(G, "conv2d_wgrad")
    _chk_s(X, "conv2d_wgrad")
    B, OH, OW, Cg_ = G.shape
    _, IH, IW, Cx_ = X.shape
    Cgs, Cxs = pitch(G), pitch(X)
    cg = Cg_ if cg is None else cg
    cx = Cx_ if cx is None else cx
    if out is None:
        out = torch.empty((R, C, KH, KW), dtype=torch.float32, device=G.device)
    lib = _lib.load()
    dt = _dt(G)
    nbytes = lib.jspsr_conv2d_wgrad_workspace_bytes(dt, B, OH, OW, cg, cx, KH, KW)
    ws = torch.empty(max(nbytes, 16), dtype=torch.uint8, device=G.device)
    head = (dt, G.data_ptr(), cg, Cgs, g_coff, X.data_ptr(), cx, Cxs, x_coff, out.data_ptr(), R, C, B, OH, OW, IH, IW, KH, KW,
            stride, pad, int(accumulate))
    if x_scale is not None:
        if x_affine is not None:
            raise ValueError("conv2d_wgrad: x_scale and x_affine exclude each other")
        _chk_scale(x_scale, B, cx, "conv2d_wgrad x_scale")
        _lib.check(lib.jspsr_conv2d_wgrad_scaled(*head, x_scale.data_ptr(), x_scale.shape[1], ws.data_ptr(), _stream()),
                   "jspsr_conv2d_wgrad_scaled")
    else:
        _lib.check(lib.jspsr_conv2d_wgrad(*head, x_affine.data_ptr() if x_affine is not None else None, int(x_relu),
                                          ws.data_ptr(), _stream()), "jspsr_conv2d_wgrad")
    return out



# ... 194 lines not shown
```

### jspsr_amd/ops.py

```python
from __future__ import annotations

import collections
import os
import weakref

import torch

from . import _lib
from . import kernels as K


def _stream() -> int:
    return torch.cuda.current_stream().cuda_stream


def _need_gpu(*ts):
    for t in ts:
        if not t.is_cuda:
            raise RuntimeError("jspsr_amd ops run on the GPU only (got a CPU tensor); there is no CPU fallback")
        if t.dtype != torch.float32:
            raise TypeError(f"expected float32, got {t.dtype}")


def prop_forward_raw(dem, weight, offset, w, b, scale, out):
# ... 577 lines not shown
            raise ValueError("SliceBuffer: slice start / buffer width must be a multiple of 16 bytes")
        return v

    def join(self, parts, lo=0, defer=0):
        return _Join.apply(self, lo, defer, *parts)


class _Join(torch.autograd.Function):
    @staticmethod
    def forward(ctx, holder, lo, defer, *parts):
        ctx.holder, ctx.defer = holder, int(defer)
        ctx.widths = [p.shape[3] for p in parts]
        n = sum(ctx.widths)
        for p, w in zip(parts, ctx.widths):
            if p.untyped_storage().data_ptr() != holder.buf.untyped_storage().data_ptr():
                raise RuntimeError("SliceBuffer.join: a part does not live in this buffer")
        return holder.buf.narrow(3, lo, n).detach()

    @staticmethod
    def backward(ctx, g):
        outs, off = [], 0
        keep = len(ctx.widths) - ctx.defer
        for i, w in enumerate(ctx.widths):
            outs.append(g.narrow(3, off, w) if i < keep else None)
            if i == keep:
                ctx.holder.deferred = g.narrow(3, off, sum(ctx.widths[keep:]))
                ctx.holder.deferred_event = torch.cuda.current_stream().record_event()
                ctx.holder.deposit_events = []
                ctx.holder.pending_deposits = ctx.holder.expected_deposits
            off += w
        return (None, None, None) + tuple(outs)


class _Conv(torch.autograd.Function):

    @staticmethod
    def forward(ctx, x, weight, bias, stride, pad, relu, transposed, want_stats=False, dest=None):
        x = K.nhwc(x)
        cdt = x.dtype
        e = K.epc(cdt)
        B, H, W, Cp = x.shape
        if Cp % e:
            raise ValueError(f"conv: input channels {Cp} must be padded to a multiple of {e} (ops.pad_channels)")
        w = weight.detach().contiguous()
        ctx.wparam = weight if isinstance(weight, torch.nn.Parameter) else None
        bias_d = bias.detach().contiguous() if bias is not None else None
        if not transposed:
            O, I, KH, KW = w.shape
            if Cp < I:
                raise ValueError("conv: input has fewer channels than the weight")
            out = None
            if dest is not None:
                out = dest[0].slice(dest[1], O, (B, (H + 2 * pad - KH) // stride + 1, (W + 2 * pad - KW) // stride + 1))
            y = K.conv2d_forward(x, _packed(weight, w, 0, Cp, cdt), bias_d, stride, pad, relu, stats=want_stats, out=out)
            if want_stats:
                y, st = y
                ctx.cfg = (stride, pad, relu, transposed, bias is not None)
                ctx.save_for_backward(x, w, None)
                ctx.mark_non_differentiable(st)
                return y, st
        else:
            I, O, KH, KW = w.shape
            if Cp != I or stride != 2 or pad != 1 or KH != 3:
                raise ValueError("conv_transpose: only k3 s2 p1 op1 without channel padding is built")
            if dest is not None:
                raise ValueError("conv_transpose: dest is not supported")
            y = K.conv2d_dgrad(x, _packed(weight, w, 1, Cp, cdt), (2 * H, 2 * W), 2, 1, bias=bias_d, relu=relu)
        ctx.cfg = (stride, pad, relu, transposed, bias is not None)
        ctx.save_for_backward(x, w, y if relu else None)
        return y

    @staticmethod
    def backward(ctx, dy, *unused):
        stride, pad, relu, transposed, has_bias = ctx.cfg
        x, w, y = ctx.saved_tensors
        cdt = x.dtype
        e = K.epc(cdt)
        dy = K.nhwc(dy)
        Co = dy.shape[3]
        Cg = (Co + e - 1) // e * e
        dbias = None
        if Co % e == 0 and (relu or has_bias):
            dz, dbias = K.act_backward(dy, y, relu, want_dz=relu, want_dbias=has_bias)
            if dz is None:
                dz = dy
        else:
            dz = pad_channels(dy * (y > 0) if relu else dy, e).contiguous()
            if has_bias:
                dbias = K.act_backward(dz, None, False, want_dz=False, want_dbias=True)[1][:Co]
        B, H, W, Cp = x.shape
        dx = dW = None
        if not transposed:
            O, I, KH, KW = w.shape
            if ctx.needs_input_grad[0]:
                if Cp != I:
                    raise RuntimeError("conv backward: gradient w.r.t. a channel-padded input is not supported")
                dx = K.conv2d_dgrad(dz, _packed(ctx.wparam, w, 1, Cg, cdt), (H, W), stride, pad)
            if ctx.needs_input_grad[1]:
                dW = _wgrad_async(ctx.wparam, dz, x, O, I, KH, KW, stride, pad)
        else:
            I, O, KH, KW = w.shape
            if ctx.needs_input_grad[0]:
                dx = K.conv2d_forward(dz, _packed(ctx.wparam, w, 0, Cg, cdt), None, 2, 1, False)
            if ctx.needs_input_grad[1]:
                dW = _wgrad_async(ctx.wparam, x, dz, I, O, KH, KW, 2, 1)
        return dx, dW, dbias, None, None, None, None, None, None


def conv2d(x, weight, bias=None, stride=1, pad=0, relu=False, dest=None):
    return _Conv.apply(x, weight, bias, stride, pad, relu, False, False, dest)


def conv2d_with_stats(x, weight, stride=1, pad=0):
    return _Conv.apply(x, weight, None, stride, pad, False, False, True)


def conv_transpose2d(x, weight):
    return _Conv.apply(x, weight, None, 2, 1, False, True)


class _BatchNorm(torch.autograd.Function):

    @staticmethod
    def forward(ctx, x, gamma, beta, running_mean, running_var, momentum, eps, training, relu, res, res_scale,
                partial=None, dest=None):
        x = K.nhwc(x)
        res_c = K.nhwc(res) if res is not None else None
        rs = float(res_scale) if res is not None else 1.0
        out = dest[0].slice(dest[1], x.shape[3], x.shape[:3]) if dest is not None else None
        mode = 0 if not relu else (1 if res is not None else 2)
        masked = mode == 1 and bn_relu_mask
        y, mean, invstd, *mk = K.bn_forward(x, gamma.detach(), beta.detach(), running_mean, running_var, momentum, eps,
                                            training, relu, res_c, rs, partial=partial if training else None, out=out,
                                            want_mask=masked)
        ctx.gb = tuple(p if isinstance(p, torch.nn.Parameter) else None for p in (gamma, beta))
        ctx.cfg = (training, mode, rs, res is not None)
        ctx.save_for_backward(x, y if mode == 1 and not masked else None, gamma.detach(), beta.detach(), mean, invstd,
                              mk[0] if masked else None)
        return y

    @staticmethod
    def backward(ctx, dy):
        training, relu, rs, has_res = ctx.cfg
        x, y, gamma, beta, mean, invstd, mask = ctx.saved_tensors
        sink = _bn_sink(*ctx.gb)
        dx, dres, dgamma, dbeta = K.bn_backward(K.nhwc(dy), y, x, gamma, mean, invstd, training, relu, rs,
                                                want_dres=has_res and ctx.needs_input_grad[9], beta=beta, grads_into=sink,
                                                mask=mask)
        if sink is not None:
            _bn_ready(*ctx.gb)
        if has_res and ctx.needs_input_grad[9] and dres is None:
            dres = dy
        return dx, dgamma, dbeta, None, None, None, None, None, None, dres, None, None, None


def batch_norm(x, gamma, beta, running_mean, running_var, momentum, eps, training, relu=False, res=None, res_scale=1.0,
               partial=None, dest=None):
    return _BatchNorm.apply(x, gamma, beta, running_mean, running_var, momentum, eps, training, relu, res, res_scale,
                            partial, dest)


fold_shortcut_bn = os.environ.get("JSPSR_BN_FOLD_SHORTCUT", "1") != "0"
fuse_bn1_input = os.environ.get("JSPSR_FUSE_BN1", "1") != "0"


class _ResUnit(torch.autograd.Function):

    @staticmethod
    def forward(ctx, x, w1, g1, b1, w2, g2, b2, wd, gd, bd, stride, scale, act, bns, dest, grad_extra=None):
        ctx.grad_extra = grad_extra
        x = K.nhwc(x)
        cdt, e = x.dtype, K.epc(x.dtype)
        B, H, W, Cp = x.shape
        O, I = w1.shape[:2]
        if Cp != I or Cp % e or O % e:
            raise ValueError(f"res_unit: {Cp} input channels against weight {tuple(w1.shape)} (multiples of {e} needed)")
        has_d = wd is not None
        (rm1, rv1, mom1, eps1, tr1), (rm2, rv2, mom2, eps2, tr2) = bns[0], bns[1]
        w1d, w2d = w1.detach().contiguous(), w2.detach().contiguous()
        g1d, b1d, g2d, b2d = g1.detach(), b1.detach(), g2.detach(), b2.detach()

        def conv_bn(inp, wt, k, st, pad, gam, bet, rm, rv, mom, eps, tr, relu, res=None, rs=1.0, out=None, par=None,
                    res_affine=None, stats_only=False, in_affine=None, want_mask=False):
            z = K.conv2d_forward(inp, _packed(par, wt, 0, inp.shape[3], cdt), None, st, pad, False, stats=tr,
                                 in_affine=in_affine, in_relu=in_affine is not None)
            z, part = z if tr else (z, None)
            y, mean, invstd, *mk = K.bn_forward(z, gam, bet, rm, rv, mom, eps, tr, relu, res, rs, partial=part, out=out,
                                                res_affine=res_affine, stats_only=stats_only, want_mask=want_mask)
            return (z, y, mean, invstd, mk[0]) if want_mask else (z, y, mean, invstd)

        OH1, OW1 = (H + 2 - 3) // stride + 1, (W + 2 - 3) // stride + 1
        fuse1 = fuse_bn1_input and K.fused_input_ok(cdt, B, OH1, OW1, O, O, 3, 3, 1, 1)
        if fuse1:
            z1, aff1, m1, i1 = conv_bn(x, w1d, 3, stride, 1, g1d, b1d, rm1, rv1, mom1, eps1, tr1, True, par=w1, stats_only=True)
            y1 = None
        else:
            z1, y1, m1, i1 = conv_bn(x, w1d, 3, stride, 1, g1d, b1d, rm1, rv1, mom1, eps1, tr1, True, par=w1)
            aff1 = None
        if has_d:
            rmd, rvd, momd, epsd, trd = bns[2]
            wdd, gdd, bdd = wd.detach().contiguous(), gd.detach(), bd.detach()
            if fold_shortcut_bn:
                zd, r_aff, md, idd = conv_bn(x, wdd, 1, stride, 0, gdd, bdd, rmd, rvd, momd, epsd, trd, False, par=wd, stats_only=True)
# ... 63 lines not shown
        dWd = dgd = dbd = None
        side = dres
        deposit = None
        if isinstance(ctx.grad_extra, tuple):
            holder, off, n = ctx.grad_extra
            if holder.deferred is not None and has_d and need_x:
                cur = torch.cuda.current_stream()
                cur.wait_event(holder.deferred_event)
                deposit = holder.deferred.narrow(3, off, n)
                if tuple(deposit.shape) != tuple(x.shape):
                    raise RuntimeError(f"res_unit: parked gradient slice {tuple(deposit.shape)} does not match the input {tuple(x.shape)}")
                if deposit.dtype != x.dtype or not (deposit.is_contiguous() or K.is_slice(deposit)):
                    holder.pending_deposits -= 1
                    deposit = None
                else:
                    deposit.record_stream(cur)
            elif holder.deferred is not None:
                holder.pending_deposits -= 1
        extra = ctx.grad_extra.take_deferred() if (ctx.grad_extra is not None and not isinstance(ctx.grad_extra, tuple)) else deposit
        if extra is not None:
            extra = K.nhwc(extra)
            if tuple(extra.shape) != tuple(x.shape):
                raise RuntimeError(f"res_unit: deferred gradient {tuple(extra.shape)} does not match the input {tuple(x.shape)}")
            if not (has_d and need_x):
                side, extra = side + extra, None
        if has_d:
            sinkd = _bn_sink(pgd, pbd)
            dzd, _, dgd, dbd = K.bn_backward(dres, None, zd, gd, md, idd, trd, 0, 1.0, beta=bd, grads_into=sinkd)
            if sinkd is not None:
                _bn_ready(pgd, pbd)
            dWd = _wgrad_async(pd, dzd, x, O, Cin, 1, 1, stride, 0)
            side = K.conv2d_dgrad(dzd, _packed(pd, wd, 1, O, cdt), (H, W), stride, 0, addend=extra) if need_x else None
        dx = None
        if need_x and deposit is not None:
            K.conv2d_dgrad(dz1, _packed(p1, w1, 1, O, cdt), (H, W), stride, 1, addend=K.nhwc(side), out=deposit)
            ctx.grad_extra[0].deposit_events.append(torch.cuda.current_stream().record_event())
        elif need_x:
            dx = K.conv2d_dgrad(dz1, _packed(p1, w1, 1, O, cdt), (H, W), stride, 1, addend=K.nhwc(side))
        if wgrad_after_dgrad:
            dW1 = _wgrad_async(p1, dz1, x, O, Cin, 3, 3, stride, 1)
        return (dx, dW1, dg1, db1, dW2, dg2, db2, dWd, dgd, dbd, None, None, None, None, None, None)


def conv_bn_infer(x, weight, gamma, beta, bn, stride, pad, relu=False, res=None, res_scale=1.0, dest=None):
    x = K.nhwc(x)
    rm, rv, _, eps, training = bn
    if training or rm is None:
        raise RuntimeError("conv_bn_infer: BatchNorm must be in eval mode with running statistics")
    sc, sh = K.bn_fold(gamma.detach(), beta.detach(), rm, rv, eps, res_scale if res is not None else 1.0)
    O, I, KH, KW = weight.shape
    B, H, W, Cp = x.shape
    out = None
    if dest is not None:
        out = dest[0].slice(dest[1], O, (B, (H + 2 * pad - KH) // stride + 1, (W + 2 * pad - KW) // stride + 1))
    return K.conv2d_forward(x, _packed(weight, weight.detach().contiguous(), 0, Cp, x.dtype), sh, stride, pad, relu, out=out,
                            scale=sc, addend=K.nhwc(res) if res is not None else None)


def conv_transpose_bn_infer(x, weight, gamma, beta, bn, relu=True, dest=None):
    x = K.nhwc(x)
    rm, rv, _, eps, training = bn
    if training or rm is None:
        raise RuntimeError("conv_transpose_bn_infer: BatchNorm must be in eval mode with running statistics")
    I, O, KH, KW = weight.shape
    B, H, W, Cp = x.shape
    if Cp != I or KH != 3:
        raise ValueError("conv_transpose: only k3 s2 p1 op1 without channel padding is built")
    sc, sh = K.bn_fold(gamma.detach(), beta.detach(), rm, rv, eps, 1.0)
    out = dest[0].slice(dest[1], O, (B, 2 * H, 2 * W)) if dest is not None else None
    return K.conv2d_dgrad(x, _packed(weight, weight.detach().contiguous(), 1, Cp, x.dtype), (2 * H, 2 * W), 2, 1, bias=sh,
                          relu=relu, out=out, scale=sc)


def res_unit_infer(x, w1, g1, b1, w2, g2, b2, wd, gd, bd, stride, scale, act, bns, dest=None):
    y1 = conv_bn_infer(x, w1, g1, b1, bns[0], stride, 1, relu=True)
    r = conv_bn_infer(x, wd, gd, bd, bns[2], stride, 0) if wd is not None else x
    return conv_bn_infer(y1, w2, g2, b2, bns[1], 1, 1, relu=bool(act), res=r, res_scale=scale, dest=dest)


def res_unit(x, w1, g1, b1, w2, g2, b2, wd, gd, bd, stride, scale, act, bns, dest=None, grad_extra=None):
    if not torch.is_grad_enabled() and not any(b[4] for b in bns):
        return res_unit_infer(x, w1, g1, b1, w2, g2, b2, wd, gd, bd, stride, scale, act, bns, dest)
    return _ResUnit.apply(x, w1, g1, b1, w2, g2, b2, wd, gd, bd, stride, scale, act, bns, dest, grad_extra)


def _gate_mlp(avg, mx, w1, w2):
    f = torch.nn.functional
    h = lambda v: f.linear(f.relu(f.linear(v, w1.flatten(1))), w2.flatten(1))
    return torch.sigmoid(h(avg) + h(mx))


class _ChannelGate(torch.autograd.Function):

    @staticmethod
    def forward(ctx, x, w1, w2):
        x = x.contiguous()
        avg, mx, amax = K.gate_pool(x)
        w1f, w2f = w1.detach().float().flatten(1).contiguous(), w2.detach().float().flatten(1).contiguous()
        s, hid = K.gate_mlp_forward(avg, mx, w1f, w2f)
        y = K.gate_scale(x, s)
        ctx.save_for_backward(x, avg, mx, amax, s, hid, w1f, w2f)
        ctx.wshapes = (w1.shape, w2.shape, w1.dtype, w2.dtype)
        return y

    @staticmethod
    def backward(ctx, dy):
        x, avg, mx, amax, s, hid, w1f, w2f = ctx.saved_tensors
        dy = dy.contiguous()
        ds = K.gate_backward_reduce(dy, x)
        davg, dmax, dw1, dw2 = K.gate_mlp_backward(ds, s, hid, avg, mx, w1f, w2f)
        dx = K.gate_backward_apply(dy, s, davg, dmax, amax)
        s1, s2, t1, t2 = ctx.wshapes
        return dx, dw1.reshape(s1).to(t1), dw2.reshape(s2).to(t2)


def channel_gate(x, w1, w2):
# ... 72 lines not shown
```

### jspsr_amd/spn.py

```python
from __future__ import annotations

import torch
import torch.nn as nn

from . import engine as E
from . import ops
from .blocks import ConvUnit, ResUnit


class Generator(nn.Module):

    def __init__(self, in_channels, kernel_size, block=None, bc=16, leaky=False):
        super().__init__()
        if kernel_size != 3 or leaky:
            raise NotImplementedError("only the 3x3, ReLU generator the reference instantiates is built")
        self.kernel_size = kernel_size
        self.num = kernel_size * kernel_size - 1
        self.idx_ref = self.num // 2
        self.convd1 = ConvUnit(1, bc * 2, 3, bn=False)
        self.convd2 = ConvUnit(bc * 2, bc * 2, 3, bn=False)
        self.convf1 = ConvUnit(in_channels, bc * 2, 3, bn=False)
        self.convf2 = ConvUnit(bc * 2, bc * 2, 3, bn=False)
        self.conv = ConvUnit(bc * 4, bc * 4, 3, bn=False)
        self.block = ResUnit(bc * 4, bc * 4)
        self.conv_weight = nn.Sequential(nn.Conv2d(bc * 4, kernel_size**2, 1))
        self.conv_offset = ConvUnit(bc * 4, 2 * self.num, 1, bn=False, relu=False)

    def features(self, dem, context):
        B, H, W = context.shape[:3]
        nd, nc = self.convd2.conv[0].out_channels, self.convf2.conv[0].out_channels
        buf = E.SliceBuffer(B, H, W, nd + nc, context.dtype, context.device)
        d = self.convd2(self.convd1(dem), dest=(buf, 0))
        f = self.convf2(self.convf1(context), dest=(buf, nd))
        return self.block(self.conv(buf.join((d, f))))

    def heads(self, feature):
        cw, co = self.conv_weight[0], self.conv_offset.conv[0]
        nw, no = cw.weight.shape[0], co.weight.shape[0]
        pad = (-(nw + no)) % 8
        w_all = torch.cat((cw.weight, co.weight, cw.weight.new_zeros((pad,) + tuple(cw.weight.shape[1:]))), 0)
        b_all = torch.cat((cw.bias, co.bias, cw.bias.new_zeros(pad)))
        y = E.conv2d(feature, w_all, b_all)
        return E.sigmoid(y[..., :nw]), y[..., nw:nw + no]

    def head(self, feature):
        cw, co = self.conv_weight[0], self.conv_offset.conv[0]
        w_all, b_all = ops.merge_heads(cw.weight, cw.bias, co.weight, co.bias)
        return E.conv2d(feature, w_all, b_all)

    def forward(self, dem, context):
        weight, off16 = self.heads(self.features(E.from_nchw(dem), E.from_nchw(context)))
        weight, off16 = E.to_nchw_f32(weight), E.to_nchw_f32(off16)
        B, _, H, W = off16.shape
        zero = torch.zeros(B, 2, H, W, dtype=off16.dtype, device=off16.device)
        i = 2 * self.idx_ref
        offset = torch.cat((off16[:, :i], zero, off16[:, i:]), 1)
        return weight.contiguous(), offset.contiguous()


class PostProcessor(nn.Module):

    def __init__(self, kernel_size=3, residual=True, scale=1.0):
        super().__init__()
        if kernel_size != 3 or not residual:
            raise NotImplementedError("only kernel_size=3, residual=True (what JSPSR/LRRU/EDSR use) is built")
        self.residual = residual
        self.w = nn.Parameter(torch.ones((1, 1, kernel_size, kernel_size)))
# ... 14 lines not shown
```

Baseline: 35.93 Mpixel/s.

## Fuse ReLU backward mask into consumer conv dgrad epilogue via gated outputs

Adds a GATE template variant to the implicit-GEMM and patch conv kernels that zeroes dgrad outputs where the forward input activation (the producer's ReLU output) is non-positive. A ReluLink object lets the consuming conv or ResUnit tell the producing bias+ReLU conv that its incoming gradient is already masked, so the producer skips its separate act_backward ReLU pass and only reduces dbias. This removes a full read/write of gradient tensors for the stem and generator convs, at the cost of an extra gate read in the dgrad epilogue and more kernel instantiations.

```diff
diff --git a/include/jspsr_hip.h b/include/jspsr_hip.h
--- a/include/jspsr_hip.h
+++ b/include/jspsr_hip.h
@@ -127,6 +127,12 @@
                        int Cin, int in_cstride, int in_coff, int KH, int KW, int stride, int pad,
                        int relu, const void* addend, int add_cstride, const float* scale,
                        const void* red_x, int red_cstride, const float* red_par, float* red_out, jspsr_stream_t stream);
+int jspsr_conv2d_dgrad_gated(int dtype, const void* gout, const void* wpack_t, const float* bias, void* gin,
+                             int B, int OH, int OW, int Cg, int g_cstride, int g_coff, int IH, int IW,
+                             int Cin, int in_cstride, int in_coff, int KH, int KW, int stride, int pad,
+                             int relu, const void* addend, int add_cstride, const float* scale,
+                             const void* red_x, int red_cstride, const float* red_par, float* red_out,
+                             const void* gate, int gate_cstride, jspsr_stream_t stream);
 
 size_t jspsr_conv2d_wgrad_workspace_bytes(int dtype, int B, int OH, int OW, int Cg, int Cx, int KH, int KW);
 int jspsr_conv2d_wgrad_x_affine_ok(int dtype, int B, int OH, int OW, int Cg, int Cx, int KH, int KW, int stride, int pad);
diff --git a/jspsr_amd/JSPSR.py b/jspsr_amd/JSPSR.py
--- a/jspsr_amd/JSPSR.py
+++ b/jspsr_amd/JSPSR.py
@@ -149,11 +149,12 @@
 
     def _forward(self, dem, img, aux):
         dem_a = E.from_nchw(dem)
-        feats = {"dem": self.conv_dem(dem_a)}
+        stem_links = {"dem": ops.ReluLink(), "aux": ops.ReluLink()}
+        feats = {"dem": self.conv_dem(dem_a, relu_link=stem_links["dem"])}
         if img is not None:
             feats["img"] = self.conv_img(E.from_nchw(img))
         if aux is not None:
-            feats["aux"] = self.conv_aux(E.from_nchw(aux))
+            feats["aux"] = self.conv_aux(E.from_nchw(aux), relu_link=stem_links["aux"])
         order = [b for b in self._branches if b in feats]
         if len(order) < 2:
             raise NotImplementedError
@@ -192,6 +193,8 @@
                             holder, w_prev = bufs[-1][0], planes // 2
                             kw["grad_extra"] = (holder, i * w_prev, w_prev)
                             holder.expected_deposits += 1
+                        if k == 0 and s == 1 and br in stem_links:
+                            kw["gate_links"] = (stem_links[br],)
                         if k == len(units) - 1:
                             kw["dest"] = (buf, lead + i * planes)
                         src = u(src, **kw)
diff --git a/jspsr_amd/_lib.py b/jspsr_amd/_lib.py
--- a/jspsr_amd/_lib.py
+++ b/jspsr_amd/_lib.py
@@ -52,6 +52,7 @@
     "jspsr_bn_fold": (c_i, [c_p, c_p, c_p, c_p, c_f, c_f, c_i, c_p, c_p, c_p]),
     "jspsr_conv2d_dgrad_reduce_ok": (c_i, [c_i] * 10),
     "jspsr_conv2d_dgrad": (c_i, [c_i] + [c_p] * 4 + [c_i] * 16 + [c_p, c_i, c_p, c_p, c_i, c_p, c_p, c_p]),
+    "jspsr_conv2d_dgrad_gated": (c_i, [c_i] + [c_p] * 4 + [c_i] * 16 + [c_p, c_i, c_p, c_p, c_i, c_p, c_p, c_p, c_i, c_p]),
     "jspsr_conv2d_wgrad_workspace_bytes": (ctypes.c_size_t, [c_i] * 8),
     "jspsr_conv2d_wgrad_x_affine_ok": (c_i, [c_i] * 10),
     "jspsr_conv2d_wgrad": (c_i, [c_i, c_p, c_i, c_i, c_i, c_p, c_i, c_i, c_i, c_p] + [c_i] * 12 + [c_p, c_i, c_p, c_p]),
diff --git a/jspsr_amd/blocks.py b/jspsr_amd/blocks.py
--- a/jspsr_amd/blocks.py
+++ b/jspsr_amd/blocks.py
@@ -51,8 +51,10 @@
         self.k = kernel_size
         self.relu = relu
 
-    def forward(self, x, dest=None):
+    def forward(self, x, dest=None, relu_link=None, gate_links=None):
         c = self.conv[0]
+        if (relu_link is not None or gate_links) and (hasattr(self, "camb") or hasattr(self.conv, "bn") or not self.relu):
+            raise ValueError("ConvUnit: ReLU links need the bias + ReLU form (bn=False, relu=True, no gate)")
         if hasattr(self, "camb") and hasattr(self.conv, "bn"):
             fc = self.camb.fc
             return E.gated_conv_bn(x, fc[0].weight, fc[1].weight, c.weight, self.conv.bn, self.k // 2, relu=self.relu, dest=dest)
@@ -60,7 +62,8 @@
             x = self.camb(x)
         if hasattr(self.conv, "bn"):
             return E.conv_bn(x, c.weight, self.conv.bn, 1, self.k // 2, relu=self.relu, dest=dest)
-        return E.conv2d(x, c.weight, c.bias, 1, self.k // 2, relu=self.relu, dest=dest)
+        return E.conv2d(x, c.weight, c.bias, 1, self.k // 2, relu=self.relu, dest=dest,
+                        relu_link=relu_link, gate_links=gate_links)
 
 
 class UpUnit(nn.Module):
@@ -96,10 +99,10 @@
 
     fused = True
 
-    def forward(self, x, dest=None, grad_extra=None):
+    def forward(self, x, dest=None, grad_extra=None, gate_links=None):
         if self.fused:
             return E.res_unit(x, self.conv1, self.bn1, self.conv2, self.bn2, self.downsample, self.stride, self.scale,
-                              self.act, dest, grad_extra)
+                              self.act, dest, grad_extra, gate_links)
         if grad_extra is not None:
             raise RuntimeError("grad_extra needs the fused block")
         y = E.conv_bn(x, self.conv1.weight, self.bn1, self.stride, 1, relu=True)
diff --git a/jspsr_amd/csrc/conv.hip b/jspsr_amd/csrc/conv.hip
--- a/jspsr_amd/csrc/conv.hip
+++ b/jspsr_amd/csrc/conv.hip
@@ -146,6 +146,27 @@
 }
 
 template <typename T>
+__device__ __forceinline__ uint4 gate_packed(uint4 v, uint4 gt) {
+  if constexpr (sizeof(T) == 4) {
+    v.x = __uint_as_float(gt.x) > 0.f ? v.x : 0u;
+    v.y = __uint_as_float(gt.y) > 0.f ? v.y : 0u;
+    v.z = __uint_as_float(gt.z) > 0.f ? v.z : 0u;
+    v.w = __uint_as_float(gt.w) > 0.f ? v.w : 0u;
+    return v;
+  } else {
+    unsigned* p = &v.x;
+    const unsigned* pg = &gt.x;
+#pragma unroll
+    for (int i = 0; i < 4; ++i) {
+      const unsigned lo = __uint_as_float(pg[i] << 16) > 0.f ? (p[i] & 0x0000ffffu) : 0u;
+      const unsigned hi = __uint_as_float(pg[i] & 0xffff0000u) > 0.f ? (p[i] & 0xffff0000u) : 0u;
+      p[i] = lo | hi;
+    }
+    return v;
+  }
+}
+
+template <typename T>
 __device__ __forceinline__ uint4 relu_packed(uint4 a) {
   if constexpr (sizeof(T) == 4) {
     float4 x = __builtin_bit_cast(float4, a);
@@ -162,7 +183,7 @@
   }
 }
 
-template <typename T, int BM, int BN, int WGM, int WGN, bool UNI, int NBUF>
+template <typename T, int BM, int BN, int WGM, int WGN, bool UNI, int NBUF, bool GATE = false>
 __global__ __launch_bounds__(NT, NBUF == 1 ? 4 : 2) void conv_igemm_kernel(const T* __restrict__ in,
                                                           const T* __restrict__ wgt,
                                                           const float* __restrict__ bias,
@@ -422,6 +443,9 @@
         v = add_packed<T>(v, *reinterpret_cast<const uint4*>(static_cast<const char*>(g.addend) +
                                                               (opix * g.add_cstride + n0) * (long long)sizeof(T) + c16 * 16));
       if (relu_last) v = relu_packed<T>(v);
+      if constexpr (GATE)
+        v = gate_packed<T>(v, *reinterpret_cast<const uint4*>(static_cast<const char*>(g.gate) +
+                                                               (opix * g.gate_cstride + n0) * (long long)sizeof(T) + c16 * 16));
       *reinterpret_cast<uint4*>(obase + opix * g.out_cstride * (long long)sizeof(T) + c16 * 16) = v;
     }
   } else {
@@ -440,6 +464,9 @@
           if (relu_first) v = fmaxf(v, 0.f);
           if (g.addend) v = (float)(T)v + (float)static_cast<const T*>(g.addend)[opix * g.add_cstride + ncol[ni]];
           if (relu_last) v = fmaxf(v, 0.f);
+          if constexpr (GATE) {
+            if (!((float)static_cast<const T*>(g.gate)[opix * g.gate_cstride + ncol[ni]] > 0.f)) v = 0.f;
+          }
           orow[ncol[ni]] = (T)v;
         }
       }
@@ -468,7 +495,7 @@
 
 __host__ __device__ constexpr int patch_it(int BM, int NTH) { return ((BM / 16 + 2) * 18 * NCH + NTH - 1) / NTH; }
 
-template <typename T, int BM, int BN, int WGM, int WGN>
+template <typename T, int BM, int BN, int WGM, int WGN, bool GATE = false>
 __global__ __launch_bounds__(64 * WGM * WGN, WGM * WGN == 8 ? 1 : 2) void conv_patch_kernel(const T* __restrict__ in, const T* __restrict__ wgt,
                                                           const float* __restrict__ bias, T* __restrict__ out,
                                                           float* __restrict__ stats, ConvGeom g) {
@@ -788,12 +815,15 @@
     long long ooff[OB];
     uint4 areg[OB];
     uint4 zreg[OB];
+    uint4 greg[GATE ? OB : 1];
     const int oy_t = ty0 * g.oy_mul + g.oy_add, ox_t = tx0 * g.ox_mul + g.ox_add, ystep = g.oy_mul * g.OW;
     const long long pix_t = ((long long)bimg * g.OH + oy_t) * g.OW + ox_t;
     const unsigned ocs = (unsigned)g.out_cstride * (unsigned)sizeof(T), acs = (unsigned)g.add_cstride * (unsigned)sizeof(T);
     const long long obase_t = pix_t * ocs, abase_t = pix_t * acs + n0 * (long long)sizeof(T);
     const unsigned zcs = (unsigned)g.red_cstride * (unsigned)sizeof(T);
     const long long zbase_t = pix_t * zcs + n0 * (long long)sizeof(T);
+    const unsigned gcs = (unsigned)g.gate_cstride * (unsigned)sizeof(T);
+    const long long gbase_t = pix_t * gcs + n0 * (long long)sizeof(T);
     const bool inside = ty0 + TLH <= g.MH && tx0 + TLW <= g.MW && oy_t + (TLH - 1) * g.oy_mul < g.OH &&
                         ox_t + (TLW - 1) * g.ox_mul < g.OW && n0 + BN <= g.Cout;
     auto plan_pieces = [&](int j0) __attribute__((always_inline)) {
@@ -813,6 +843,12 @@
             areg[j] = *reinterpret_cast<const uint4*>(static_cast<const char*>(g.addend) + abase_t +
                                                       (long long)((unsigned long long)dpix * acs) + c16 * 16);
         }
+        if constexpr (GATE) {
+          greg[j] = make_uint4(0, 0, 0, 0);
+          if (ok)
+            greg[j] = *reinterpret_cast<const uint4*>(static_cast<const char*>(g.gate) + gbase_t +
+                                                      (long long)((unsigned long long)dpix * gcs) + c16 * 16);
+        }
         if (g.red_out) {
           zreg[j] = make_uint4(0, 0, 0, 0);
           if (ok)
@@ -868,6 +904,7 @@
         uint4 v = ov[j];
         if (g.addend) v = add_packed<T>(v, areg[j]);
         if (relu_last) v = relu_packed<T>(v);
+        if constexpr (GATE) v = gate_packed<T>(v, greg[j]);
         *reinterpret_cast<uint4*>(obase + ooff[j]) = v;
         if (g.red_out) {
           float dv[EPC], zv[EPC];
@@ -923,6 +960,9 @@
           if (relu_first) v = fmaxf(v, 0.f);
           if (g.addend) v = (float)(T)v + (float)static_cast<const T*>(g.addend)[opix * g.add_cstride + ncol[ni]];
           if (relu_last) v = fmaxf(v, 0.f);
+          if constexpr (GATE) {
+            if (!((float)static_cast<const T*>(g.gate)[opix * g.gate_cstride + ncol[ni]] > 0.f)) v = 0.f;
+          }
           orow[ncol[ni]] = (T)v;
         }
       }
@@ -943,12 +983,15 @@
 #endif
 }
 
-template <typename T, int BM, int BN, int WGM, int WGN>
+template <typename T, int BM, int BN, int WGM, int WGN, bool GATE = false>
 int launch_patch(const void* in, const void* wgt, const float* bias, void* out, float* stats, const ConvGeom& g, hipStream_t s) {
   constexpr int NTH = 64 * WGM * WGN, TLW = 16, TLH = BM / TLW, MAXPIX = patch_it(BM, NTH) * NTH / NCH;
   const long long nblk = (long long)g.B * ((g.MH + TLH - 1) / TLH) * ((g.MW + TLW - 1) / TLW) * ((g.Cout + BN - 1) / BN);
   if (nblk > 0x7fffffffLL || (long long)TLH * g.oy_mul * g.OW + (long long)TLW * g.ox_mul > 0x7fffffffLL)
     return fail(JSPSR_EINVAL, "conv: grid too large");
+  if constexpr (!GATE) {
+    if (g.gate) return launch_patch<T, BM, BN, WGM, WGN, true>(in, wgt, bias, out, stats, g, s);
+  }
   constexpr int ROWB = Mma<T>::ROWP;
   const size_t lds_stage = (size_t)MAXPIX * ROWB + 2 * BN * ROWB, lds_out = (size_t)BM * (BN * sizeof(T) + 16);
   const size_t lds = lds_stage > lds_out ? lds_stage : lds_out;
@@ -956,7 +999,7 @@
   gk.fd_ntn = make_fastdiv((unsigned)((g.Cout + BN - 1) / BN));
   gk.fd_ttx = make_fastdiv((unsigned)((g.MW + TLW - 1) / TLW));
   gk.fd_tty = make_fastdiv((unsigned)((g.MH + TLH - 1) / TLH));
-  auto kern = conv_patch_kernel<T, BM, BN, WGM, WGN>;
+  auto kern = conv_patch_kernel<T, BM, BN, WGM, WGN, GATE>;
   static bool attr_set = false;
   if (!attr_set) {
     (void)hipFuncSetAttribute(reinterpret_cast<const void*>(kern), hipFuncAttributeMaxDynamicSharedMemorySize, (int)lds);
@@ -967,29 +1010,32 @@
   return check_launch(BM == 256 ? (BN == 64 ? "conv_patch_16x16" : "conv_patch_16x16x128") : "conv_patch");
 }
 
-template <typename T, int BM, int BN, int WGM, int WGN, int NBUF>
+template <typename T, int BM, int BN, int WGM, int WGN, int NBUF, bool GATE = false>
 int launch_cfg(const void* in, const void* wgt, const float* bias, void* out, float* stats, const ConvGeom& g, hipStream_t s) {
   if ((long long)g.B * g.MH * g.MW <= 0) return JSPSR_OK;
   constexpr int TLW = 16, TLH = BM / TLW;
   const long long nblk = (long long)g.B * ((g.MH + TLH - 1) / TLH) * ((g.MW + TLW - 1) / TLW) * ((g.Cout + BN - 1) / BN);
   if (nblk > 0x7fffffffLL) return fail(JSPSR_EINVAL, "conv: grid too large");
+  if constexpr (!GATE) {
+    if (g.gate) return launch_cfg<T, BM, BN, WGM, WGN, NBUF, true>(in, wgt, bias, out, stats, g, s);
+  }
   constexpr int ROWB = IgemmMma<T, NBUF>::ROWP;
   const size_t lds_stage = NBUF * (BM + BN) * ROWB, lds_out = (size_t)BM * (BN * sizeof(T) + 16);
   const size_t lds = lds_stage > lds_out ? lds_stage : lds_out;
   constexpr int BK = NCH * Elem<T>::EPC;
   static bool attr_set = false;
   if (!attr_set) {
-    (void)hipFuncSetAttribute(reinterpret_cast<const void*>(conv_igemm_kernel<T, BM, BN, WGM, WGN, true, NBUF>),
+    (void)hipFuncSetAttribute(reinterpret_cast<const void*>(conv_igemm_kernel<T, BM, BN, WGM, WGN, true, NBUF, GATE>),
                               hipFuncAttributeMaxDynamicSharedMemorySize, (int)lds);
-    (void)hipFuncSetAttribute(reinterpret_cast<const void*>(conv_igemm_kernel<T, BM, BN, WGM, WGN, false, NBUF>),
+    (void)hipFuncSetAttribute(reinterpret_cast<const void*>(conv_igemm_kernel<T, BM, BN, WGM, WGN, false, NBUF, GATE>),
                               hipFuncAttributeMaxDynamicSharedMemorySize, (int)lds);
     attr_set = true;
   }
   if (g.Cin % BK == 0)
-    hipLaunchKernelGGL((conv_igemm_kernel<T, BM, BN, WGM, WGN, true, NBUF>), dim3((unsigned)nblk), dim3(NT), lds, s,
+    hipLaunchKernelGGL((conv_igemm_kernel<T, BM, BN, WGM, WGN, true, NBUF, GATE>), dim3((unsigned)nblk), dim3(NT), lds, s,
                        static_cast<const T*>(in), static_cast<const T*>(wgt), bias, static_cast<T*>(out), stats, g);
   else
-    hipLaunchKernelGGL((conv_igemm_kernel<T, BM, BN, WGM, WGN, false, NBUF>), dim3((unsigned)nblk), dim3(NT), lds, s,
+    hipLaunchKernelGGL((conv_igemm_kernel<T, BM, BN, WGM, WGN, false, NBUF, GATE>), dim3((unsigned)nblk), dim3(NT), lds, s,
                        static_cast<const T*>(in), static_cast<const T*>(wgt), bias, static_cast<T*>(out), stats, g);
   return check_launch("conv_igemm");
 }
@@ -1192,12 +1238,12 @@
   return 1;
 }
 
-extern "C" int jspsr_conv2d_dgrad(int dtype, const void* gout, const void* wpack_t, const float* bias, void* gin,
-                                  int B, int OH, int OW, int Cg, int g_cstride, int g_coff, int IH, int IW,
-                                  int Cin, int in_cstride, int in_coff, int KH, int KW, int stride, int pad,
-                                  int relu, const void* addend, int add_cstride, const float* scale,
-                                  const void* red_x, int red_cstride, const float* red_par, float* red_out,
-                                  jspsr_stream_t stream) {
+static int conv2d_dgrad_impl(int dtype, const void* gout, const void* wpack_t, const float* bias, void* gin,
+                             int B, int OH, int OW, int Cg, int g_cstride, int g_coff, int IH, int IW,
+                             int Cin, int in_cstride, int in_coff, int KH, int KW, int stride, int pad,
+                             int relu, const void* addend, int add_cstride, const float* scale,
+                             const void* red_x, int red_cstride, const float* red_par, float* red_out,
+                             const void* gate, int gate_cstride, jspsr_stream_t stream) {
   if (int e = check_common(dtype, gout, wpack_t, gin, Cg, g_cstride, g_coff, in_cstride, in_coff, Cin, "conv2d_dgrad")) return e;
   if (addend && add_cstride < Cin) return fail(JSPSR_EINVAL, "conv2d_dgrad: addend pitch %d < %d channels", add_cstride, Cin);
   if (red_out) {
@@ -1229,11 +1275,43 @@
       g.oy_mul = stride; g.oy_add = py; g.ox_mul = stride; g.ox_add = px; g.relu = relu;
       g.addend = addend; g.add_cstride = add_cstride; g.scale = scale;
       g.red_x = red_x; g.red_cstride = red_cstride; g.red_par = red_par; g.red_out = red_out;
+      g.gate = gate; g.gate_cstride = gate_cstride;
       const int e = dtype == JSPSR_F32 ? launch<float>(gout, wpack_t, bias, gin, nullptr, g, s)
                                        : launch<__bf16>(gout, wpack_t, bias, gin, nullptr, g, s);
       if (e) return e;
     }
   return JSPSR_OK;
+}
+
+extern "C" int jspsr_conv2d_dgrad(int dtype, const void* gout, const void* wpack_t, const float* bias, void* gin,
+                                  int B, int OH, int OW, int Cg, int g_cstride, int g_coff, int IH, int IW,
+                                  int Cin, int in_cstride, int in_coff, int KH, int KW, int stride, int pad,
+                                  int relu, const void* addend, int add_cstride, const float* scale,
+                                  const void* red_x, int red_cstride, const float* red_par, float* red_out,
+                                  jspsr_stream_t stream) {
+  return conv2d_dgrad_impl(dtype, gout, wpack_t, bias, gin, B, OH, OW, Cg, g_cstride, g_coff, IH, IW, Cin, in_cstride, in_coff, KH, KW,
+                           stride, pad, relu, addend, add_cstride, scale, red_x, red_cstride, red_par, red_out, nullptr, 0, stream);
+}
+
+extern "C" int jspsr_conv2d_dgrad_gated(int dtype, const void* gout, const void* wpack_t, const float* bias, void* gin,
+                                        int B, int OH, int OW, int Cg, int g_cstride, int g_coff, int IH, int IW,
+                                        int Cin, int in_cstride, int in_coff, int KH, int KW, int stride, int pad,
+                                        int relu, const void* addend, int add_cstride, const float* scale,
+                                        const void* red_x, int red_cstride, const float* red_par, float* red_out,
+                                        const void* gate, int gate_cstride, jspsr_stream_t stream) {
+  if (dtype != JSPSR_F32 && dtype != JSPSR_BF16) return fail(JSPSR_EINVAL, "conv2d_dgrad_gated: dtype must be JSPSR_F32 or JSPSR_BF16");
+  if (!gate) return fail(JSPSR_EINVAL, "conv2d_dgrad_gated: null gate (jspsr_conv2d_dgrad is the gate-less entry)");
+  if (relu || bias || scale)
+    return fail(JSPSR_EINVAL, "conv2d_dgrad_gated: the gate is the ReLU backward of a plain data gradient (no ReLU / bias / scale)");
+  if (red_x || red_par || red_out) return fail(JSPSR_EINVAL, "conv2d_dgrad_gated: not together with the fused BatchNorm-backward reduce");
+  if (stride != 1) return fail(JSPSR_EINVAL, "conv2d_dgrad_gated: stride %d (the phases of a strided / transposed conv are not gated)", stride);
+  const int epc = dtype == JSPSR_F32 ? 4 : 8;
+  if (!aligned16(gate) || gate_cstride < Cin || gate_cstride % epc)
+    return fail(JSPSR_EINVAL, "conv2d_dgrad_gated: the gate must be 16-byte aligned, its pitch %d >= %d channels and a multiple of %d",
+                gate_cstride, Cin, epc);
+  const int e = conv2d_dgrad_impl(dtype, gout, wpack_t, bias, gin, B, OH, OW, Cg, g_cstride, g_coff, IH, IW, Cin, in_cstride, in_coff, KH,
+                                  KW, stride, pad, relu, addend, add_cstride, scale, nullptr, 0, nullptr, nullptr, gate, gate_cstride, stream);
+  return e ? e : check_launch("conv2d_dgrad_gated");
 }
 
 #ifdef CONVLAB_STAMPS
diff --git a/jspsr_amd/csrc/conv128.hip b/jspsr_amd/csrc/conv128.hip
--- a/jspsr_amd/csrc/conv128.hip
+++ b/jspsr_amd/csrc/conv128.hip
@@ -94,7 +94,7 @@
 template <int SIGN, int MODE, int KH>
 __device__ __forceinline__ void conv128_body(const __bf16* __restrict__ in, const __bf16* __restrict__ wgt, const float* __restrict__ bias,
                                              __bf16* __restrict__ out, float* __restrict__ stats, const ConvGeom& g, int ntiles, unsigned* __restrict__ ticket, char* smem) {
-  constexpr bool STATS = MODE == 1, AFFINE = MODE == 2;
+  constexpr bool STATS = MODE == 1, AFFINE = MODE == 2, GATED = MODE == 3;
   const int tid = threadIdx.x, wave = __builtin_amdgcn_readfirstlane(tid >> 6), lane = tid & 63;
   const int cg = wave & 1;
   const int n = lane & 15, q = lane >> 4;
@@ -203,6 +203,20 @@
     const unsigned long long b64 = reinterpret_cast<unsigned long long>(g.addend) + ((long long)tc.bimg * g.OH * g.OW * g.add_cstride + 64 * cg) * 2;
     const i32x4 d = {(int)(unsigned)b64, (int)((unsigned)(b64 >> 32) & 0xffffu), g.addend ? (int)0xFFFFFF00u : 0, 0x00020000};
     asm volatile("s_mov_b32 m0, %0\n\ts_nop 4\n\tbuffer_load_dwordx4 %1, %2, 0 offen lds" : : "s"(lds0 + (unsigned)Q_OFF_DUMP), "v"(off), "s"(d));
+  };
+  u32x4 gv[4][2];
+  auto load_gate = [&](QTile tc) __attribute__((always_inline)) {
+    const int ty0 = tc.tyi * Q_TH + 4 * KH, x = tc.txi * Q_TW + n;
+    const unsigned long long b64 = reinterpret_cast<unsigned long long>(g.gate) + ((long long)tc.bimg * g.OH * g.OW * g.gate_cstride + 64 * cg) * 2;
+    const __amdgpu_buffer_rsrc_t gtrsrc = __builtin_amdgcn_make_buffer_rsrc(reinterpret_cast<char*>(b64), 0, g.gate ? 0xFFFFFF00u : 0u, 0x00020000);
+#pragma unroll
+    for (int i = 0; i < 4; ++i) {
+      const int y = ty0 + i;
+      const unsigned goff = (y < g.MH && x < g.MW) ? (unsigned)(y * g.OW + x) * (unsigned)(g.gate_cstride * 2) + q * 16u : 0xFFFFFFF0u;
+#pragma unroll
+      for (int h = 0; h < 2; ++h) gv[i][h] = __builtin_amdgcn_raw_buffer_load_b128(gtrsrc, goff, h * 64, 0);
+    }
+    __builtin_amdgcn_sched_barrier(0);
   };
 
   char* const give = smem + inbox_off(wave ^ 2) + lane * 16;
@@ -244,6 +258,7 @@
         a[k % Q_LAH] = *reinterpret_cast<lds_frag_t>((abase[R & 3][tx] ^ (unsigned)(s * 64)) + (unsigned)((R >> 2) * Q_ROWS4));
         if constexpr (K2Q_DMA_MODE == 1 && k % K2Q_DMA_EVERY == 2 && k / K2Q_DMA_EVERY < Q_NP) issue_piece(nxt, nbufoff, k / K2Q_DMA_EVERY);
         if constexpr (!STATS && k == 1) prefetch_addend(tc);
+        if constexpr (GATED && k == 5) load_gate(tc);
         if constexpr (K2Q_DMA_MODE == 3) {
           constexpr int LD = K2Q_LD_EVERY, WD = K2Q_LD_DIST;
           static_assert(2 + LD * (Q_NP - 1) + WD < Q_NK, "the last piece is written inside the loop");
@@ -343,7 +358,36 @@
         }
       }
     }
-    if (!STATS && g.addend) {
+    if constexpr (GATED) {
+#pragma unroll
+      for (int i = 0; i < 4; ++i)
+#pragma unroll
+        for (int h = 0; h < 2; ++h) asm volatile("" : "+v"(gv[i][h]));
+      if (g.addend) {
+        u32x4 av[4][2];
+#pragma unroll
+        for (int i = 0; i < 4; ++i)
+#pragma unroll
+          for (int h = 0; h < 2; ++h) av[i][h] = __builtin_amdgcn_raw_buffer_load_b128(adrsrc, aoff[i], h * 64, 0);
+#pragma unroll
+        for (int i = 0; i < 4; ++i)
+#pragma unroll
+          for (int h = 0; h < 2; ++h) {
+            const f32x4 lo = acc[4 * KH + i][2 * h], hi = acc[4 * KH + i][2 * h + 1];
+            const u32x4 o = {pack_bf16(lo[0], lo[1]), pack_bf16(lo[2], lo[3]), pack_bf16(hi[0], hi[1]), pack_bf16(hi[2], hi[3])};
+            __builtin_amdgcn_raw_buffer_store_b128(gate_bf16x8(add_bf16x8(o, av[i][h], false), gv[i][h]), orsrc, ooff[i], h * 64, 0);
+          }
+      } else {
+#pragma unroll
+        for (int i = 0; i < 4; ++i)
+#pragma unroll
+          for (int h = 0; h < 2; ++h) {
+            const f32x4 lo = acc[4 * KH + i][2 * h], hi = acc[4 * KH + i][2 * h + 1];
+            const u32x4 o = {pack_bf16(lo[0], lo[1]), pack_bf16(lo[2], lo[3]), pack_bf16(hi[0], hi[1]), pack_bf16(hi[2], hi[3])};
+            __builtin_amdgcn_raw_buffer_store_b128(gate_bf16x8(o, gv[i][h]), orsrc, ooff[i], h * 64, 0);
+          }
+      }
+    } else if (!STATS && g.addend) {
       u32x4 av[4][2];
 #pragma unroll
       for (int i = 0; i < 4; ++i)
@@ -534,6 +578,9 @@
   if (g.in_cstride % 8 || g.in_coff % 8 || g.out_cstride % 8 || g.out_coff % 8) return false;
   if (!aligned16(in) || !aligned16(wgt) || !aligned16(out)) return false;
   if (g.addend && (!aligned16(g.addend) || g.add_cstride % 8)) return false;
+  if (g.gate && (g.sign > 0 || bias || g.scale || g.relu || !aligned16(g.gate) || g.gate_cstride % 8 ||
+                 (long long)g.OH * g.OW * g.gate_cstride * 2 >= 0xF0000000LL))
+    return false;
   if ((long long)(g.IW + 20) * 12 * g.in_cstride * 2 >= 0x7fffffffLL || g.IW >= (1 << 20) || g.in_cstride >= (1 << 20)) return false;
   if ((long long)g.OH * g.OW * g.out_cstride * 2 >= 0xF0000000LL || (long long)g.OH * g.OW * g.add_cstride * 2 >= 0xF0000000LL)
     return false;
@@ -563,7 +610,8 @@
     else launch_k2q<1, 2>(in, wgt, bias, out, stats, g, ntiles, grid, s);
   } else {
     if (mode != 0) return fail(JSPSR_EINVAL, "conv128_resident: the reversed walk has no statistics / affine form");
-    launch_k2q<-1, 0>(in, wgt, bias, out, stats, g, ntiles, grid, s);
+    if (g.gate) launch_k2q<-1, 3>(in, wgt, bias, out, stats, g, ntiles, grid, s);
+    else launch_k2q<-1, 0>(in, wgt, bias, out, stats, g, ntiles, grid, s);
   }
   return check_launch("conv128_resident");
 }
diff --git a/jspsr_amd/csrc/conv64.hip b/jspsr_amd/csrc/conv64.hip
--- a/jspsr_amd/csrc/conv64.hip
+++ b/jspsr_amd/csrc/conv64.hip
@@ -50,7 +50,7 @@
                                                                   const float* __restrict__ bias, __bf16* __restrict__ out,
                                                                   float* __restrict__ stats, ConvGeom g, int ntiles,
                                                                   unsigned* __restrict__ ticket) {
-  constexpr bool STATS = MODE == 1, AFFINE = MODE == 2;
+  constexpr bool STATS = MODE == 1, AFFINE = MODE == 2, GATED = MODE == 3;
   constexpr int LDSB = MODE == 1 ? R_LDS_STATS : (MODE == 2 ? R_LDS_AFFINE : R_LDS_PLAIN);
   extern __shared__ __attribute__((aligned(128))) char smem[];
   const int tid = threadIdx.x, wave = __builtin_amdgcn_readfirstlane(tid >> 6), lane = tid & 63;
@@ -187,6 +187,10 @@
     const unsigned long long b64 = reinterpret_cast<unsigned long long>(g.addend) + ((long long)bimg * g.OH * g.OW * g.add_cstride + wn * 32) * 2;
     return __builtin_amdgcn_make_buffer_rsrc(reinterpret_cast<char*>(b64), 0, g.addend ? 0xFFFFFF00u : 0u, 0x00020000);
   };
+  auto gate_desc = [&](int bimg) {
+    const unsigned long long b64 = reinterpret_cast<unsigned long long>(g.gate) + ((long long)bimg * g.OH * g.OW * g.gate_cstride + wn * 32) * 2;
+    return __builtin_amdgcn_make_buffer_rsrc(reinterpret_cast<char*>(b64), 0, g.gate ? 0xFFFFFF00u : 0u, 0x00020000);
+  };
 
   auto epilogue_stats = [&](Tile tc, int par) __attribute__((always_inline)) {
     const int ty0 = tc.tyi * 16, tx0 = tc.txi * 16;
@@ -271,7 +275,7 @@
     const int ty0 = tc.tyi * 16, tx0 = tc.txi * 16;
     const bool whole = ty0 + 16 <= g.MH && tx0 + 16 <= g.MW;
     const __amdgpu_buffer_rsrc_t orsrc = out_desc(tc.bimg), adrsrc = add_desc(tc.bimg);
-    unsigned ooff[2], aoff[2];
+    unsigned ooff[2], aoff[2], goff[2];
 #pragma unroll
     for (int mi = 0; mi < 2; ++mi) {
       const int R = wm * 64 + mi * 32 + lr, dy = R >> 4;
@@ -280,6 +284,7 @@
       const unsigned pix = (unsigned)(y * g.OW + x);
       ooff[mi] = inside ? pix * (unsigned)(g.out_cstride * 2) + lh * 16u : 0xFFFFFFF0u;
       aoff[mi] = inside ? pix * (unsigned)(g.add_cstride * 2) + lh * 16u : 0xFFFFFFF0u;
+      if constexpr (GATED) goff[mi] = inside ? pix * (unsigned)(g.gate_cstride * 2) + lh * 16u : 0xFFFFFFF0u;
     }
     u32x4 av[2][2];
     if (g.addend) {
@@ -287,6 +292,14 @@
       for (int mi = 0; mi < 2; ++mi)
 #pragma unroll
         for (int h = 0; h < 2; ++h) av[mi][h] = __builtin_amdgcn_raw_buffer_load_b128(adrsrc, aoff[mi], h * 32, 0);
+    }
+    u32x4 gv[2][2];
+    if constexpr (GATED) {
+      const __amdgpu_buffer_rsrc_t gtrsrc = gate_desc(tc.bimg);
+#pragma unroll
+      for (int mi = 0; mi < 2; ++mi)
+#pragma unroll
+        for (int h = 0; h < 2; ++h) gv[mi][h] = __builtin_amdgcn_raw_buffer_load_b128(gtrsrc, goff[mi], h * 32, 0);
     }
     if constexpr (AFFINE) {
       const float* tab = reinterpret_cast<const float*>(smem + R_OFF_PAR) + wn * 32 + 4 * lh;
@@ -324,6 +337,7 @@
       for (int h = 0; h < 2; ++h) {
         u32x4 o = {d[mi][4 * h], d[mi][4 * h + 1], d[mi][4 * h + 2], d[mi][4 * h + 3]};
         if (g.addend) o = add_bf16x8(o, av[mi][h], relu_last);
+        if constexpr (GATED) o = gate_bf16x8(o, gv[mi][h]);
         __builtin_amdgcn_raw_buffer_store_b128(o, orsrc, ooff[mi], h * 32, 0);
       }
     }
@@ -488,6 +502,9 @@
   if (g.in_cstride % 8 || g.in_coff % 8 || g.out_cstride % 8 || g.out_coff % 8) return false;
   if (!aligned16(in) || !aligned16(wgt) || !aligned16(out)) return false;
   if (g.addend && (!aligned16(g.addend) || g.add_cstride % 8)) return false;
+  if (g.gate && (g.sign > 0 || bias || g.scale || g.relu || !aligned16(g.gate) || g.gate_cstride % 8 ||
+                 (long long)g.OH * g.OW * g.gate_cstride * 2 >= 0xF0000000LL))
+    return false;
   if ((long long)(g.IW + 20) * 20 * g.in_cstride * 2 >= 0x7fffffffLL) return false;
   if ((long long)g.OH * g.OW * g.out_cstride * 2 >= 0xF0000000LL || (long long)g.OH * g.OW * g.add_cstride * 2 >= 0xF0000000LL)
     return false;
@@ -508,7 +525,10 @@
   }
   const int grid = ntiles < ncu ? ntiles : ncu;
   const int mode = stats ? 1 : ((bias || g.scale) ? 2 : 0);
-  if (g.sign > 0) {
+  if (g.gate) {
+    if (g.sign > 0 || mode != 0) return fail(JSPSR_EINVAL, "conv64_resident: the ReLU gate exists for the plain data gradient only");
+    launch_k2r<-1, 3>(in, wgt, bias, out, stats, g, ntiles, grid, s);
+  } else if (g.sign > 0) {
     if (mode == 0) launch_k2r<1, 0>(in, wgt, bias, out, stats, g, ntiles, grid, s);
     else if (mode == 1) launch_k2r<1, 1>(in, wgt, bias, out, stats, g, ntiles, grid, s);
     else launch_k2r<1, 2>(in, wgt, bias, out, stats, g, ntiles, grid, s);
diff --git a/jspsr_amd/csrc/conv_igemm.h b/jspsr_amd/csrc/conv_igemm.h
--- a/jspsr_amd/csrc/conv_igemm.h
+++ b/jspsr_amd/csrc/conv_igemm.h
@@ -35,6 +35,8 @@
   int red_cstride;
   const float* red_par;
   float* red_out;
+  const void* gate;
+  int gate_cstride;
 };
 
 typedef __attribute__((address_space(3))) void* lptr_t;
@@ -60,7 +62,16 @@
   }
   return r;
 }
-
+__device__ __forceinline__ u32x4 gate_bf16x8(u32x4 v, u32x4 gt) {
+  u32x4 r;
+#pragma unroll
+  for (int i = 0; i < 4; ++i) {
+    const unsigned lo = __uint_as_float(gt[i] << 16) > 0.f ? (v[i] & 0x0000ffffu) : 0u;
+    const unsigned hi = __uint_as_float(gt[i] & 0xffff0000u) > 0.f ? (v[i] & 0xffff0000u) : 0u;
+    r[i] = lo | hi;
+  }
+  return r;
+}
 
 bool conv64_resident_ok(const ConvGeom& g, const void* in, const void* wgt, const float* bias, const void* out);
 int launch_conv64_resident(const void* in, const void* wgt, const float* bias, void* out, float* stats, const ConvGeom& g,
diff --git a/jspsr_amd/csrc/elementwise.hip b/jspsr_amd/csrc/elementwise.hip
--- a/jspsr_amd/csrc/elementwise.hip
+++ b/jspsr_amd/csrc/elementwise.hip
@@ -863,6 +863,9 @@
   if (relu) { ACT_BWD(true); } else { ACT_BWD(false); }
 #undef ACT_BWD
   if (int e = check_launch("act_backward")) return e;
+  if (relu) {
+    if (int e = check_launch("act_backward_mask")) return e;
+  }
   if (dbias) {
     hipLaunchKernelGGL(sum_rows_kernel, dim3((C + 3) / 4), dim3(256), 0, s, partial, g.chunks, 1, 0, C, dbias);
     return check_launch("act_backward_bias");
diff --git a/jspsr_amd/engine.py b/jspsr_amd/engine.py
--- a/jspsr_amd/engine.py
+++ b/jspsr_amd/engine.py
@@ -55,8 +55,11 @@
 SliceBuffer = ops.SliceBuffer
 
 
-def conv2d(x, weight, bias=None, stride=1, padding=0, relu=False, dest=None):
-    return ops.conv2d(x, weight, bias, stride, padding, relu, dest)
+ReluLink = ops.ReluLink
+
+
+def conv2d(x, weight, bias=None, stride=1, padding=0, relu=False, dest=None, relu_link=None, gate_links=None):
+    return ops.conv2d(x, weight, bias, stride, padding, relu, dest, relu_link, gate_links)
 
 
 def conv_transpose2d(x, weight):
@@ -120,14 +123,14 @@
     return (bn.running_mean, bn.running_var, bn.momentum, bn.eps, training)
 
 
-def res_unit(x, conv1, bn1, conv2, bn2, downsample, stride, scale, act, dest=None, grad_extra=None):
+def res_unit(x, conv1, bn1, conv2, bn2, downsample, stride, scale, act, dest=None, grad_extra=None, gate_links=None):
     bns = [_bn_state(bn1), _bn_state(bn2)]
     wd = gd = bd = None
     if downsample is not None:
         wd, gd, bd = downsample[0].weight, downsample[1].weight, downsample[1].bias
         bns.append(_bn_state(downsample[1]))
     return ops.res_unit(x, conv1.weight, bn1.weight, bn1.bias, conv2.weight, bn2.weight, bn2.bias, wd, gd, bd,
-                        stride, scale, act, tuple(bns), dest, grad_extra)
+                        stride, scale, act, tuple(bns), dest, grad_extra, gate_links)
 
 
 def channel_gate(x, w1, w2):
diff --git a/jspsr_amd/kernels.py b/jspsr_amd/kernels.py
--- a/jspsr_amd/kernels.py
+++ b/jspsr_amd/kernels.py
@@ -136,8 +136,18 @@
     return par
 
 
+def dgrad_gate_ok(gate, g, in_hw, cin, stride, bias=None, relu=False, scale=None, red=None) -> bool:
+    if gate is None or stride != 1 or relu or bias is not None or scale is not None or red is not None:
+        return False
+    if not gate.is_cuda or gate.dtype != g.dtype or gate.dim() != 4 or not (gate.is_contiguous() or is_slice(gate)):
+        return False
+    if tuple(gate.shape) != (g.shape[0], in_hw[0], in_hw[1], cin):
+        return False
+    return gate.data_ptr() % 16 == 0 and pitch(gate) % epc(gate.dtype) == 0
+
+
 def conv2d_dgrad(g, wpack_t, in_hw, stride, pad, bias=None, relu=False, out=None, out_coff=0, g_coff=0, addend=None,
-                 scale=None, red=None):
+                 scale=None, red=None, gate=None):
     _chk_s(g, "conv2d_dgrad")
     B, OH, OW, _ = g.shape
     Cgs = pitch(g)
@@ -162,16 +172,24 @@
             raise ValueError(f"conv2d_dgrad: red_x {tuple(red_x.shape)} {red_x.dtype} does not match the result")
         rows = lib.jspsr_conv2d_stats_rows(B, IH, IW)
         red_out = torch.empty((rows, 2, Cin), dtype=torch.float32, device=g.device)
-    _lib.check(lib.jspsr_conv2d_dgrad(_dt(g), g.data_ptr(), wpack_t.data_ptr(),
-                                      bias.data_ptr() if bias is not None else None, out.data_ptr(),
-                                      B, OH, OW, Cg, Cgs, g_coff, IH, IW, Cin, pitch(out), out_coff,
-                                      KH, KW, stride, pad, int(relu),
-                                      addend.data_ptr() if addend is not None else None,
-                                      pitch(addend) if addend is not None else 0,
-                                      scale.data_ptr() if scale is not None else None,
-                                      red_x.data_ptr() if red is not None else None, pitch(red_x) if red is not None else 0,
-                                      red_par.data_ptr() if red is not None else None,
-                                      red_out.data_ptr() if red is not None else None, _stream()), "jspsr_conv2d_dgrad")
+    head = (_dt(g), g.data_ptr(), wpack_t.data_ptr(),
+            bias.data_ptr() if bias is not None else None, out.data_ptr(),
+            B, OH, OW, Cg, Cgs, g_coff, IH, IW, Cin, pitch(out), out_coff,
+            KH, KW, stride, pad, int(relu),
+            addend.data_ptr() if addend is not None else None,
+            pitch(addend) if addend is not None else 0,
+            scale.data_ptr() if scale is not None else None,
+            red_x.data_ptr() if red is not None else None, pitch(red_x) if red is not None else 0,
+            red_par.data_ptr() if red is not None else None,
+            red_out.data_ptr() if red is not None else None)
+    if gate is not None:
+        if not gate.is_cuda or gate.dim() != 4 or gate.stride(3) != 1:
+            raise ValueError("conv2d_dgrad gate: expected an NHWC tensor on the GPU")
+        if tuple(gate.shape) != (B, IH, IW, Cin) or gate.dtype != g.dtype:
+            raise ValueError(f"conv2d_dgrad: gate {tuple(gate.shape)} {gate.dtype} does not match the result")
+        _lib.check(lib.jspsr_conv2d_dgrad_gated(*head, gate.data_ptr(), pitch(gate), _stream()), "jspsr_conv2d_dgrad_gated")
+    else:
+        _lib.check(lib.jspsr_conv2d_dgrad(*head, _stream()), "jspsr_conv2d_dgrad")
     return (out, red_out) if red is not None else out
 
 
diff --git a/jspsr_amd/ops.py b/jspsr_amd/ops.py
--- a/jspsr_amd/ops.py
+++ b/jspsr_amd/ops.py
@@ -633,10 +633,35 @@
         return (None, None, None) + tuple(outs)
 
 
+relu_gate = os.environ.get("JSPSR_RELU_GATE", "1") != "0"
+
+
+class ReluLink:
+    __slots__ = ("armed",)
+
+    def __init__(self):
+        self.armed = False
+
+
+def _gate_for(links, x, g, in_hw, cin, stride):
+    if links and relu_gate and K.dgrad_gate_ok(x, g, in_hw, cin, stride):
+        return x
+    return None
+
+
+def _arm(links, carried):
+    for link in links or ():
+        link.armed = bool(carried)
+
+
 class _Conv(torch.autograd.Function):
 
     @staticmethod
-    def forward(ctx, x, weight, bias, stride, pad, relu, transposed, want_stats=False, dest=None):
+    def forward(ctx, x, weight, bias, stride, pad, relu, transposed, want_stats=False, dest=None, relu_link=None,
+                gate_links=None):
+        if relu_link is not None and (not relu or transposed or want_stats):
+            raise ValueError("conv: relu_link belongs to a conv with a ReLU in its epilogue")
+        ctx.relu_link, ctx.gate_links = relu_link, tuple(gate_links) if gate_links else None
         x = K.nhwc(x)
         cdt = x.dtype
         e = K.epc(cdt)
@@ -681,7 +706,15 @@
         Co = dy.shape[3]
         Cg = (Co + e - 1) // e * e
         dbias = None
-        if Co % e == 0 and (relu or has_bias):
+        link = ctx.relu_link
+        masked = link is not None and link.armed
+        if link is not None:
+            link.armed = False
+        if masked:
+            dz = dy
+            if has_bias:
+                dbias = K.act_backward(dz, None, False, want_dz=False, want_dbias=True)[1]
+        elif Co % e == 0 and (relu or has_bias):
             dz, dbias = K.act_backward(dy, y, relu, want_dz=relu, want_dbias=has_bias)
             if dz is None:
                 dz = dy
@@ -696,20 +729,25 @@
             if ctx.needs_input_grad[0]:
                 if Cp != I:
                     raise RuntimeError("conv backward: gradient w.r.t. a channel-padded input is not supported")
-                dx = K.conv2d_dgrad(dz, _packed(ctx.wparam, w, 1, Cg, cdt), (H, W), stride, pad)
+                gate = _gate_for(ctx.gate_links, x, dz, (H, W), I, stride)
+                dx = K.conv2d_dgrad(dz, _packed(ctx.wparam, w, 1, Cg, cdt), (H, W), stride, pad, gate=gate)
+                _arm(ctx.gate_links, gate is not None)
+            else:
+                _arm(ctx.gate_links, False)
             if ctx.needs_input_grad[1]:
                 dW = _wgrad_async(ctx.wparam, dz, x, O, I, KH, KW, stride, pad)
         else:
+            _arm(ctx.gate_links, False)
             I, O, KH, KW = w.shape
             if ctx.needs_input_grad[0]:
                 dx = K.conv2d_forward(dz, _packed(ctx.wparam, w, 0, Cg, cdt), None, 2, 1, False)
             if ctx.needs_input_grad[1]:
                 dW = _wgrad_async(ctx.wparam, x, dz, I, O, KH, KW, 2, 1)
-        return dx, dW, dbias, None, None, None, None, None, None
-
-
-def conv2d(x, weight, bias=None, stride=1, pad=0, relu=False, dest=None):
-    return _Conv.apply(x, weight, bias, stride, pad, relu, False, False, dest)
+        return dx, dW, dbias, None, None, None, None, None, None, None, None
+
+
+def conv2d(x, weight, bias=None, stride=1, pad=0, relu=False, dest=None, relu_link=None, gate_links=None):
+    return _Conv.apply(x, weight, bias, stride, pad, relu, False, False, dest, relu_link, gate_links)
 
 
 def conv2d_with_stats(x, weight, stride=1, pad=0):
@@ -768,8 +806,9 @@
 class _ResUnit(torch.autograd.Function):
 
     @staticmethod
-    def forward(ctx, x, w1, g1, b1, w2, g2, b2, wd, gd, bd, stride, scale, act, bns, dest, grad_extra=None):
+    def forward(ctx, x, w1, g1, b1, w2, g2, b2, wd, gd, bd, stride, scale, act, bns, dest, grad_extra=None, gate_links=None):
         ctx.grad_extra = grad_extra
+        ctx.gate_links = tuple(gate_links) if gate_links else None
         x = K.nhwc(x)
         cdt, e = x.dtype, K.epc(x.dtype)
         B, H, W, Cp = x.shape
@@ -899,14 +938,16 @@
             dWd = _wgrad_async(pd, dzd, x, O, Cin, 1, 1, stride, 0)
             side = K.conv2d_dgrad(dzd, _packed(pd, wd, 1, O, cdt), (H, W), stride, 0, addend=extra) if need_x else None
         dx = None
+        gate = _gate_for(ctx.gate_links, x, dz1, (H, W), Cin, stride) if need_x else None
         if need_x and deposit is not None:
-            K.conv2d_dgrad(dz1, _packed(p1, w1, 1, O, cdt), (H, W), stride, 1, addend=K.nhwc(side), out=deposit)
+            K.conv2d_dgrad(dz1, _packed(p1, w1, 1, O, cdt), (H, W), stride, 1, addend=K.nhwc(side), out=deposit, gate=gate)
             ctx.grad_extra[0].deposit_events.append(torch.cuda.current_stream().record_event())
         elif need_x:
-            dx = K.conv2d_dgrad(dz1, _packed(p1, w1, 1, O, cdt), (H, W), stride, 1, addend=K.nhwc(side))
+            dx = K.conv2d_dgrad(dz1, _packed(p1, w1, 1, O, cdt), (H, W), stride, 1, addend=K.nhwc(side), gate=gate)
+        _arm(ctx.gate_links, gate is not None)
         if wgrad_after_dgrad:
             dW1 = _wgrad_async(p1, dz1, x, O, Cin, 3, 3, stride, 1)
-        return (dx, dW1, dg1, db1, dW2, dg2, db2, dWd, dgd, dbd, None, None, None, None, None, None)
+        return (dx, dW1, dg1, db1, dW2, dg2, db2, dWd, dgd, dbd, None, None, None, None, None, None, None)
 
 
 def conv_bn_infer(x, weight, gamma, beta, bn, stride, pad, relu=False, res=None, res_scale=1.0, dest=None):
@@ -945,10 +986,10 @@
     return conv_bn_infer(y1, w2, g2, b2, bns[1], 1, 1, relu=bool(act), res=r, res_scale=scale, dest=dest)
 
 
-def res_unit(x, w1, g1, b1, w2, g2, b2, wd, gd, bd, stride, scale, act, bns, dest=None, grad_extra=None):
+def res_unit(x, w1, g1, b1, w2, g2, b2, wd, gd, bd, stride, scale, act, bns, dest=None, grad_extra=None, gate_links=None):
     if not torch.is_grad_enabled() and not any(b[4] for b in bns):
         return res_unit_infer(x, w1, g1, b1, w2, g2, b2, wd, gd, bd, stride, scale, act, bns, dest)
-    return _ResUnit.apply(x, w1, g1, b1, w2, g2, b2, wd, gd, bd, stride, scale, act, bns, dest, grad_extra)
+    return _ResUnit.apply(x, w1, g1, b1, w2, g2, b2, wd, gd, bd, stride, scale, act, bns, dest, grad_extra, gate_links)
 
 
 def _gate_mlp(avg, mx, w1, w2):
diff --git a/jspsr_amd/spn.py b/jspsr_amd/spn.py
--- a/jspsr_amd/spn.py
+++ b/jspsr_amd/spn.py
@@ -30,9 +30,10 @@
         B, H, W = context.shape[:3]
         nd, nc = self.convd2.conv[0].out_channels, self.convf2.conv[0].out_channels
         buf = E.SliceBuffer(B, H, W, nd + nc, context.dtype, context.device)
-        d = self.convd2(self.convd1(dem), dest=(buf, 0))
-        f = self.convf2(self.convf1(context), dest=(buf, nd))
-        return self.block(self.conv(buf.join((d, f))))
+        ld1, ld2, lf1, lf2, lc = (ops.ReluLink() for _ in range(5))
+        d = self.convd2(self.convd1(dem, relu_link=ld1), dest=(buf, 0), relu_link=ld2, gate_links=(ld1,))
+        f = self.convf2(self.convf1(context, relu_link=lf1), dest=(buf, nd), relu_link=lf2, gate_links=(lf1,))
+        return self.block(self.conv(buf.join((d, f)), relu_link=lc, gate_links=(ld2, lf2)), gate_links=(lc,))
 
     def heads(self, feature):
         cw, co = self.conv_weight[0], self.conv_offset.conv[0]
```

Measured after the change: 35.96 Mpixel/s (median of 3 runs). No clear change (+0.1%).
